# TheCacophonyProject/classifier-pipeline

Measured on AMD Instinct MI355X. Metric: CPTV frames/s end-to-end (track+classify) at 160x120, higher is better.
Workload: dtype u16/i32 track stage (f32 normalise, f64 gates); f32 crop/tile; f32 CNN (stride-1 3x3 convs of stages 2-4 (+ the stride-2 one): two fp16 planes per operand rounded to nearest (11 + 11 significand bits), power-of-two range scaling, 3 fp16 MFMAs per K step, device-side rerun in the exact split if an ac

## Files before the change

classifier-pipeline_amd/cpx/_lib.py:

```python

import ctypes as C
import os

import numpy as np

_HERE = os.path.dirname(os.path.abspath(__file__))
LIB_PATH = os.environ.get("CPX_LIB") or os.path.join(_HERE, "libcpx_hip.so")

CPX_OK = 0
STATUS = {
    0: "CPX_OK",
    -1: "CPX_ERR_INVALID",
    -2: "CPX_ERR_UNSUPPORTED",
    -3: "CPX_ERR_NO_DEVICE",
    -4: "CPX_ERR_HIP",
    -5: "CPX_ERR_OVERFLOW",
    -6: "CPX_ERR_NOMEM",
}


class CpxError(RuntimeError):
    def __init__(self, code, what=""):
        self.code = code
        super().__init__("%s (%d) %s" % (STATUS.get(code, "CPX_ERR"), code, what))


class Config(C.Structure):
    _fields_ = [
        ("width", C.c_int32),
        ("height", C.c_int32),
        ("edge_pixels", C.c_int32),
        ("window", C.c_int32),
        ("background_thresh", C.c_double),
        ("weight_add", C.c_double),
        ("max_components", C.c_int32),
        ("max_frames", C.c_int32),
        ("denoise", C.c_int32),
        ("reserved", C.c_int32),
    ]


FRAME_META_DTYPE = np.dtype(
    [("time_on_ms", "<i8"), ("last_ffc_ms", "<i8"), ("background_frame", "<i4"), ("has_times", "<i4")]
)
COMPONENT_DTYPE = np.dtype(
    [("x", "<i4"), ("y", "<i4"), ("width", "<i4"), ("height", "<i4"), ("area", "<i4"),
     ("sum_x", "<i4"), ("sum_y", "<i4"), ("pixel_variance", "<f4")]
)
FRAME_INFO_DTYPE = np.dtype(
    [("frame_number", "<i4"), ("n_components", "<i4"), ("status", "<i4"), ("ffc_affected", "<i4"),
     ("avg_change", "<i4"), ("norm_min", "<i4"), ("norm_max", "<i4"), ("threshold", "<f4"),
     ("filt_min", "<i4"), ("filt_max", "<i4"), ("thermal_min", "<i4"), ("thermal_max", "<i4"),
     ("thermal_sum", "<u4"), ("thermal_median", "<f4"), ("filtered_abs_sum", "<u8"),
     ("background_average", "<f8"), ("background_changed", "<i4"), ("reserved", "<i4")]
)
REGION_REF_DTYPE = np.dtype([("frame", "<i4"), ("x", "<i4"), ("y", "<i4"), ("width", "<i4"), ("height", "<i4"),
                             ("in_segment", "<i4")])
TRACK_LIMITS_DTYPE = np.dtype([("filt_min", "<f4"), ("filt_max", "<f4"), ("clip_at_zero", "<i4"), ("flags", "<i4"),
                               ("therm_min", "<f4"), ("therm_max", "<f4"), ("reserved", "<i4", (2,))])
CROP_REQ_DTYPE = np.dtype([("frame", "<i4"), ("x", "<i4"), ("y", "<i4"), ("width", "<i4"), ("height", "<i4"),
                           ("track", "<i4"), ("sample", "<i4"), ("tile", "<i4")])
THUMB_STAT_DTYPE = np.dtype([("contours", "<i4"), ("status", "<i4"), ("median_diff", "<f8")])
CONV_TIMING_DTYPE = np.dtype([("key", "<i4"), ("launches", "<i4"), ("total_ms", "<f8"), ("flops", "<f8")])
CPTV_FILE_DTYPE = np.dtype([("in_offset", "<i8"), ("in_bytes", "<i8"), ("out_offset", "<i8"), ("out_capacity", "<i8"),
                            ("slot_offset", "<i8"), ("slot_capacity", "<i4"), ("reserved", "<i4")])
CPTV_RESULT_DTYPE = np.dtype([("status", "<i4"), ("n_frames", "<i4"), ("out_bytes", "<i8"), ("in_consumed", "<i8"),
                              ("header_bytes", "<i4"), ("width", "<i4"), ("height", "<i4"), ("reserved", "<i4")])
CPTV_SLOT_DTYPE = np.dtype([("offset", "<i8"), ("bit_width", "<i4"), ("time_on_ms", "<u4"), ("last_ffc_ms", "<u4"),
                            ("temp_c", "<f4"), ("last_ffc_temp_c", "<f4"), ("flags", "<u4")])
CPTV_HEADER_BYTES = 1024
CPTV_BACKGROUND_FRAME, CPTV_HAS_TIME_ON, CPTV_HAS_LAST_FFC = 1, 2, 4
CPTV_STATUS = {1: "deflate: reserved block type", 2: "deflate: stored block length", 3: "deflate: block header",
               4: "deflate: code lengths", 5: "deflate: invalid symbol", 6: "deflate: distance too far back",
               7: "inflated data larger than the gzip trailer says", 8: "deflate: input exhausted (truncated file)",
               9: "deflate: no end-of-block code", 10: "not a gzip member", 11: "gzip trailer / further member", 12: "gzip CRC-32 mismatch",
               20: "not a CPTV file", 21: "unsupported CPTV version", 22: "CPTV header section", 23: "expected frame section",
               24: "truncated CPTV frame", 25: "malformed CPTV frame section", 26: "more frames than slots",
               27: "CPTV file has no frames"}
assert CPTV_FILE_DTYPE.itemsize == 48 and CPTV_RESULT_DTYPE.itemsize == 40 and CPTV_SLOT_DTYPE.itemsize == 32
assert REGION_REF_DTYPE.itemsize == 24 and TRACK_LIMITS_DTYPE.itemsize == 32 and CROP_REQ_DTYPE.itemsize == 32
assert FRAME_META_DTYPE.itemsize == 24 and COMPONENT_DTYPE.itemsize == 32 and FRAME_INFO_DTYPE.itemsize == 80

class WRResNetBlock(C.Structure):
    _fields_ = [(k, C.c_void_p) for k in ("in_scale", "in_shift", "wa", "a_scale", "a_shift", "wb", "bb")]


class WRResNetParams(C.Structure):
    _fields_ = [("n_labels", C.c_int32), ("blocks_per_stage", C.c_int32), ("groups", C.c_int32),
                ("in_channels", C.c_int32), ("filters", C.c_int32 * 4),
                ("conv1_w", C.c_void_p), ("conv1_b", C.c_void_p),
                ("block", (WRResNetBlock * 8) * 3),
                ("shortcut_w", C.c_void_p * 3), ("shortcut_b", C.c_void_p * 3),
                ("final_scale", C.c_void_p), ("final_shift", C.c_void_p),
                ("dense_w", C.c_void_p), ("dense_b", C.c_void_p),
                ("n_hidden", C.c_int32), ("activation", C.c_int32), ("hidden_sizes", C.c_int32 * 4),
                ("hidden_w", C.c_void_p * 4), ("hidden_b", C.c_void_p * 4)]


class HeadDesc(C.Structure):
    _fields_ = [("N", C.c_int32), ("HW", C.c_int32), ("C", C.c_int32), ("L", C.c_int32),
                ("n_hidden", C.c_int32), ("activation", C.c_int32), ("hidden_sizes", C.c_int32 * 4),
                ("in_dev", C.c_void_p), ("bn_scale_dev", C.c_void_p), ("bn_shift_dev", C.c_void_p),
                ("hidden_w_dev", C.c_void_p * 4), ("hidden_b_dev", C.c_void_p * 4),
                ("dense_w_dev", C.c_void_p), ("dense_b_dev", C.c_void_p),
                ("logits_dev", C.c_void_p), ("probs_dev", C.c_void_p)]


class GraphTensor(C.Structure):
    _fields_ = [("H", C.c_int32), ("W", C.c_int32), ("C", C.c_int32), ("c_offset", C.c_int32), ("c_stride", C.c_int32),
                ("reserved", C.c_int32), ("arena_offset", C.c_int64)]


class GraphOp(C.Structure):
    _fields_ = [("kind", C.c_int32), ("in0", C.c_int32), ("in1", C.c_int32), ("out", C.c_int32),
                ("kh", C.c_int32), ("kw", C.c_int32), ("stride_h", C.c_int32), ("stride_w", C.c_int32),
                ("pad_top", C.c_int32), ("pad_left", C.c_int32), ("pad_bottom", C.c_int32), ("pad_right", C.c_int32),
                ("activation", C.c_int32), ("out_c_offset", C.c_int32), ("out_c_stride", C.c_int32),
                ("n_map", C.c_int32), ("channel_map", C.c_int32 * 4), ("param", C.c_float),
                ("weights", C.c_void_p), ("scale", C.c_void_p), ("shift", C.c_void_p)]


assert C.sizeof(WRResNetParams) == 1560
assert C.sizeof(GraphTensor) == 32 and C.sizeof(GraphOp) == 112
GRAPH_CONV, GRAPH_MAX_POOL, GRAPH_AVG_POOL, GRAPH_ADD, GRAPH_AFFINE, GRAPH_MEAN, GRAPH_FC, GRAPH_LOGISTIC, GRAPH_SOFTMAX, \
    GRAPH_PAD, GRAPH_CHANNEL_MAP, GRAPH_CONV_Q8, GRAPH_FC_Q8, GRAPH_QUANT_PARAMS, GRAPH_DWCONV, GRAPH_DWCONV_Q8, GRAPH_MUL, \
    GRAPH_INPUT, GRAPH_CONV_PRE, GRAPH_SLICE, GRAPH_DWCONV_PRE = range(1, 22)
GRAPH_ACT_SWISH, GRAPH_ACT_LOGISTIC = 16, 17
GRAPH_MEAN_WIDE_PIXELS = 256
GRAPH_CONV_KC, GRAPH_CONV_CO = 16, 32
GRAPH_CONV_Q8_KC = 32
HEAD_SIGMOID, HEAD_SOFTMAX = 0, 1


EXPORTS = [
    "cpx_abi_version", "cpx_create", "cpx_destroy", "cpx_last_error", "cpx_stream", "cpx_synchronize", "cpx_join_medians", "cpx_release_memory",
    "cpx_track_batch", "cpx_track_workspace_bytes", "cpx_last_kernel_timing", "cpx_associate_batch",
    "cpx_track_limits_batch", "cpx_crop_tile", "cpx_conv2d", "cpx_cnn_head",
    "cpx_finalize_tracks", "cpx_counts_prefix", "cpx_plan_segments", "cpx_aggregate_predictions",
    "cpx_conv_timing_enable", "cpx_conv_timing_report", "cpx_cptv_unpack", "cpx_thumb_stats", "cpx_trackless_thumb",
    "cpx_trackless_thumb_batch", "cpx_thumb_stats_ex",
    "cpx_track_frame", "cpx_associate_frame", "cpx_cnn_create", "cpx_cnn_destroy", "cpx_cnn_forward", "cpx_ir_detect", "cpx_set_cnn_math", "cpx_get_cnn_math",
    "cpx_mog2_create", "cpx_mog2_apply", "cpx_mog2_background", "cpx_mog2_destroy",
    "cpx_track_batch_ex", "cpx_track_frame_ex", "cpx_set_background", "cpx_get_background", "cpx_track_limits_batch_ex",
    "cpx_cnn_head_ex", "cpx_ir_delta_variance", "cpx_cptv_inflate", "cpx_cptv_gather_index", "cpx_format_regions", "cpx_json_indent", "cpx_ir_merge", "cpx_ir_resize_area",
    "cpx_ir_frame_statistics", "cpx_cnn_last_overflow", "cpx_cnn_set_activation_bounds", "cpx_cnn_overflow_forwards", "cpx_cnn_forward_taps",
    "cpx_graph_create", "cpx_graph_forward", "cpx_graph_arena_bytes", "cpx_graph_arena_allocated", "cpx_graph_destroy",
    "cpx_cnn_set_residual_bounds", "cpx_cnn_shortcut_scale",
]

IR_FRAME_STATS_DTYPE = np.dtype([("min", "<i4"), ("max", "<i4"), ("sum", "<i8"), ("median_x2", "<i4"), ("reserved", "<i4"),
                                 ("filtered_sum", "<i8")])
assert IR_FRAME_STATS_DTYPE.itemsize == 32

TRACK_KEEP_BACKGROUND, TRACK_FREEZE_ON_FFC, TRACK_FREEZE_BACKGROUND, TRACK_DEFER_MEDIANS = 1, 2, 4, 8
LIMITS_POST_PROCESS, LIMITS_THERMAL_DIFF_NORM, LIMITS_NO_DIFF_NORM, LIMITS_ALWAYS_CLIP, LIMITS_SWAP_CHANNELS = 1, 2, 4, 8, 16
LIMITS_TF_SCALING = 32

_lib = None


def load():
    global _lib
    if _lib is not None:
        return _lib
    if not os.path.exists(LIB_PATH):
        raise ImportError(
            "libcpx_hip.so not built: run `python __graft_entry__.py` (or make -C classifier-pipeline_amd/csrc)")
    try:
        import torch
    except ImportError:
        pass
    lib = C.CDLL(LIB_PATH)
    vp, i32p = C.c_void_p, C.POINTER(C.c_int32)
    lib.cpx_abi_version.restype = C.c_int
    lib.cpx_create.argtypes = [C.c_int, C.POINTER(Config), C.POINTER(vp)]
    lib.cpx_create.restype = C.c_int
    lib.cpx_destroy.argtypes = [vp]
    lib.cpx_destroy.restype = None
    lib.cpx_last_error.argtypes = [vp]
    lib.cpx_last_error.restype = C.c_char_p
    lib.cpx_stream.argtypes = [vp]
    lib.cpx_stream.restype = vp
    lib.cpx_synchronize.argtypes = [vp]
    lib.cpx_synchronize.restype = C.c_int
    lib.cpx_join_medians.argtypes = [vp]
    lib.cpx_join_medians.restype = C.c_int
    lib.cpx_release_memory.argtypes = [vp]
    lib.cpx_release_memory.restype = C.c_int
    lib.cpx_track_batch.argtypes = [vp, vp, i32p, vp, C.c_int, vp, vp, vp, vp, vp]
    lib.cpx_track_batch.restype = C.c_int
    lib.cpx_associate_batch.argtypes = [vp, vp, i32p, vp, C.c_int, vp, vp, vp, vp, vp, vp, vp, vp]
    lib.cpx_associate_batch.restype = C.c_int
    lib.cpx_track_limits_batch.argtypes = [vp, vp, vp, vp, vp, vp, C.c_int, vp]
    lib.cpx_track_limits_batch.restype = C.c_int
    lib.cpx_crop_tile.argtypes = [vp, vp, vp, vp, vp, C.c_int, vp, C.c_int, C.c_int, vp]
    lib.cpx_crop_tile.restype = C.c_int
    lib.cpx_conv2d.argtypes = [vp, vp]
    lib.cpx_conv2d.restype = C.c_int
    lib.cpx_cnn_head.argtypes = [vp, vp, C.c_int, C.c_int, C.c_int, vp, vp, vp, vp, C.c_int, vp, vp]
    lib.cpx_cnn_head.restype = C.c_int
    lib.cpx_cnn_head_ex.argtypes = [vp, C.POINTER(HeadDesc)]
    lib.cpx_cnn_head_ex.restype = C.c_int
    lib.cpx_finalize_tracks.argtypes = [vp, vp, i32p, vp, C.c_int, vp, vp, vp, vp, vp]
    lib.cpx_finalize_tracks.restype = C.c_int
    lib.cpx_plan_segments.argtypes = [vp, vp, i32p, vp, C.c_int, vp, vp, vp, vp, C.c_int, vp, vp, vp, vp, vp]
    lib.cpx_plan_segments.restype = C.c_int
    lib.cpx_counts_prefix.argtypes = [vp, vp, C.c_int, vp]
    lib.cpx_counts_prefix.restype = C.c_int
    lib.cpx_aggregate_predictions.argtypes = [vp, vp, vp, C.c_int, vp, C.c_int, C.c_int, C.c_int, C.c_int, vp, vp]
    lib.cpx_aggregate_predictions.restype = C.c_int
    lib.cpx_conv_timing_enable.argtypes = [vp, C.c_int]
    lib.cpx_conv_timing_enable.restype = C.c_int
    lib.cpx_conv_timing_report.argtypes = [vp, vp, C.c_int, C.POINTER(C.c_int)]
    lib.cpx_conv_timing_report.restype = C.c_int
    lib.cpx_set_cnn_math.argtypes = [vp, C.c_int]
    lib.cpx_set_cnn_math.restype = C.c_int
    lib.cpx_get_cnn_math.argtypes = [vp]
    lib.cpx_get_cnn_math.restype = C.c_int
    lib.cpx_cnn_last_overflow.argtypes = [vp, C.POINTER(C.c_int)]
    lib.cpx_cnn_last_overflow.restype = C.c_int
    lib.cpx_cnn_overflow_forwards.argtypes = [vp, C.POINTER(C.c_int), C.c_int]
    lib.cpx_cnn_overflow_forwards.restype = C.c_int
    lib.cpx_cnn_set_activation_bounds.argtypes = [vp, C.POINTER(C.c_float), C.c_int]
    lib.cpx_cnn_set_activation_bounds.restype = C.c_int
    lib.cpx_cnn_set_residual_bounds.argtypes = [vp, C.POINTER(C.c_float), C.c_int]
    lib.cpx_cnn_set_residual_bounds.restype = C.c_int
    lib.cpx_cnn_shortcut_scale.argtypes = [C.c_float, C.c_float, C.POINTER(C.c_float)]
    lib.cpx_cnn_shortcut_scale.restype = C.c_int
    lib.cpx_mog2_create.argtypes = [vp, C.c_int, C.c_int, C.c_int, C.c_int, C.c_float, C.POINTER(vp)]
    lib.cpx_mog2_create.restype = C.c_int
    lib.cpx_mog2_apply.argtypes = [vp, vp, C.c_double, vp]
    lib.cpx_mog2_apply.restype = C.c_int
    lib.cpx_mog2_background.argtypes = [vp, vp]
    lib.cpx_mog2_background.restype = C.c_int
    lib.cpx_mog2_destroy.argtypes = [vp]
    lib.cpx_mog2_destroy.restype = None
    lib.cpx_ir_detect.argtypes = [vp, vp, C.c_int, C.c_int, C.c_int, C.c_int, C.c_int, vp, vp, vp, vp]
    lib.cpx_ir_detect.restype = C.c_int
    lib.cpx_ir_delta_variance.argtypes = [vp, vp, vp, C.c_int, C.c_int, vp, C.c_int, vp]
    lib.cpx_ir_delta_variance.restype = C.c_int
    lib.cpx_ir_merge.argtypes = [vp, vp, vp, C.c_int, C.c_int, C.c_int, vp, vp, C.c_int, C.c_int, C.c_int, C.c_int, vp, vp, vp]
    lib.cpx_ir_merge.restype = C.c_int
    lib.cpx_ir_resize_area.argtypes = [vp, vp, C.c_int, C.c_int, C.c_int, C.c_int, vp]
    lib.cpx_ir_resize_area.restype = C.c_int
    lib.cpx_ir_frame_statistics.argtypes = [vp, vp, vp, C.c_int, C.c_int, vp, vp]
    lib.cpx_ir_frame_statistics.restype = C.c_int
    lib.cpx_cnn_create.argtypes = [vp, C.POINTER(WRResNetParams), C.POINTER(vp)]
    lib.cpx_cnn_create.restype = C.c_int
    lib.cpx_cnn_destroy.argtypes = [vp]
    lib.cpx_cnn_destroy.restype = None
    lib.cpx_graph_create.argtypes = [vp, C.POINTER(GraphOp), C.c_int, C.POINTER(GraphTensor), C.c_int, C.c_int, C.c_int,
                                     C.POINTER(vp)]
    lib.cpx_graph_create.restype = C.c_int
    lib.cpx_graph_forward.argtypes = [vp, vp, C.c_int, vp]
    lib.cpx_graph_forward.restype = C.c_int
    lib.cpx_graph_arena_bytes.argtypes = [vp, C.c_int, C.POINTER(C.c_size_t)]
    lib.cpx_graph_arena_bytes.restype = C.c_int
    lib.cpx_graph_arena_allocated.argtypes = [vp, C.POINTER(C.c_size_t)]
    lib.cpx_graph_arena_allocated.restype = C.c_int
    lib.cpx_graph_destroy.argtypes = [vp]
    lib.cpx_graph_destroy.restype = None
    lib.cpx_cnn_forward.argtypes = [vp, vp, C.c_int, C.c_int, C.c_int, vp, vp]
    lib.cpx_cnn_forward.restype = C.c_int
    lib.cpx_cnn_forward_taps.argtypes = [vp, vp, C.c_int, C.c_int, C.c_int, vp, vp, C.POINTER(vp), C.c_int, vp]
    lib.cpx_cnn_forward_taps.restype = C.c_int
    lib.cpx_track_frame.argtypes = [vp, vp, vp, C.c_int, C.c_int, vp, vp, vp, vp, vp]
    lib.cpx_track_frame.restype = C.c_int
    lib.cpx_track_batch_ex.argtypes = [vp, vp, i32p, vp, C.c_int, vp, vp, vp, vp, vp, C.c_int]
    lib.cpx_track_batch_ex.restype = C.c_int
    lib.cpx_track_frame_ex.argtypes = [vp, vp, vp, C.c_int, C.c_int, vp, vp, vp, vp, vp, C.c_int]
    lib.cpx_track_frame_ex.restype = C.c_int
    lib.cpx_set_background.argtypes = [vp, C.c_int, vp, vp, C.c_double]
    lib.cpx_set_background.restype = C.c_int
    lib.cpx_get_background.argtypes = [vp, C.c_int, vp, vp, C.POINTER(C.c_double)]
    lib.cpx_get_background.restype = C.c_int
    lib.cpx_track_limits_batch_ex.argtypes = [vp, vp, vp, vp, vp, vp, C.c_int, vp, C.c_int]
    lib.cpx_track_limits_batch_ex.restype = C.c_int
    lib.cpx_associate_frame.argtypes = [vp, vp, vp, C.c_int, C.c_int, vp, vp, vp, vp, vp, vp, vp, vp]
    lib.cpx_associate_frame.restype = C.c_int
    lib.cpx_thumb_stats.argtypes = [vp, vp, vp, vp, vp, C.c_int, vp]
    lib.cpx_thumb_stats.restype = C.c_int
    lib.cpx_thumb_stats_ex.argtypes = [vp, vp, vp, vp, vp, C.c_int, vp, C.c_int, C.c_int, C.c_int]
    lib.cpx_thumb_stats_ex.restype = C.c_int
    lib.cpx_trackless_thumb.argtypes = [vp, vp, C.c_int, C.c_int, vp]
    lib.cpx_trackless_thumb.restype = C.c_int
    lib.cpx_trackless_thumb_batch.argtypes = [vp, vp, vp, C.c_int, vp]
    lib.cpx_trackless_thumb_batch.restype = C.c_int
    lib.cpx_cptv_unpack.argtypes = [vp, vp, vp, vp, vp, C.c_int, vp]
    lib.cpx_cptv_unpack.restype = C.c_int
    lib.cpx_cptv_inflate.argtypes = [vp, vp, vp, C.c_int, vp, vp, vp, vp]
    lib.cpx_cptv_inflate.restype = C.c_int
    lib.cpx_cptv_gather_index.argtypes = [vp, vp, vp, vp, C.c_int, vp, vp, vp]
    lib.cpx_cptv_gather_index.restype = C.c_int
    lib.cpx_format_regions.argtypes = [vp, C.c_int, C.c_long, C.c_int, C.c_int, C.c_int, vp, C.c_long]
    lib.cpx_format_regions.restype = C.c_long
    lib.cpx_json_indent.argtypes = [C.c_char_p, C.c_long, C.c_int, C.c_int, vp, C.c_long]
    lib.cpx_json_indent.restype = C.c_long
    lib.cpx_track_workspace_bytes.argtypes = [vp, C.c_int, C.c_int]
    lib.cpx_track_workspace_bytes.restype = C.c_size_t
    lib.cpx_last_kernel_timing.argtypes = [vp, C.POINTER(C.c_float), C.POINTER(C.c_int)]
    lib.cpx_last_kernel_timing.restype = C.c_int
    if lib.cpx_abi_version() != 3:
        raise ImportError("libcpx_hip.so ABI version mismatch")
    _lib = lib
    return lib
```

classifier-pipeline_amd/cpx/engine.py:

```python

import ctypes as C

import numpy as np

from . import _lib
from ._lib import (COMPONENT_DTYPE, CROP_REQ_DTYPE, FRAME_INFO_DTYPE, FRAME_META_DTYPE, REGION_REF_DTYPE,
                   THUMB_STAT_DTYPE, TRACK_LIMITS_DTYPE, CpxError)
from .tracking import REGION_DTYPE, TRACK_RECORD_DTYPE, make_track_params, track_regions


def thresholds_for_model(model):
    if model == "lepton3.5":
        return 50.0, 1.0
    return 20.0, 0.1


class TrackBatchResult:

    def __init__(self, engine, total, cap, comps, info, labels, filtered, background):
        self.engine, self.total, self.cap = engine, total, cap
        self.comps_dev, self.info_dev = comps, info
        self.labels_dev, self.filtered_dev, self.background_dev = labels, filtered, background
        self._info = self._comps = None
        engine._retain(self)
# ... 108 lines not shown
        self.filtered = t.zeros((n, H, W), dtype=t.float32, device=dev)
        self.background = t.zeros((1, H, W), dtype=t.float32, device=dev)
        ma, mt = params.max_active_tracks, params.max_tracks
        self.pool = t.zeros(n * ma * 14, dtype=t.int32, device=dev)
        self.tracks = t.zeros(mt * 8, dtype=t.int32, device=dev)
        self.ntracks = t.zeros(1, dtype=t.int32, device=dev)
        self.status = t.zeros(1, dtype=t.int32, device=dev)
        self.regions = t.zeros(n * cap * 14, dtype=t.int32, device=dev)
        self.rcounts = t.zeros(n, dtype=t.int32, device=dev)
        self.meta = np.zeros(n, dtype=FRAME_META_DTYPE)
        self.n = 0
        self.n_tracked = 0
        self.result = TrackBatchResult(engine, n, cap, self.comps, self.info, self.labels, self.filtered,
                                       self.background)

    def _p(self, tensor):
        return C.c_void_p(tensor.data_ptr() if tensor is not None else None)

    def append(self, pix, time_on=None, last_ffc=None, init_only=False, associate=True, flags=0):
        eng, t = self.engine, self.engine.torch
        if self.n >= self.cap_frames:
            raise CpxError(-1, "stream is full (%d frames): open the extractor with a larger max_frames"
                           % self.cap_frames)
        f = self.n
        a = np.ascontiguousarray(pix, dtype=np.uint16)
        self.frames_dev[f].copy_(t.from_numpy(a.view(np.int16)))
        m = self.meta[f]
        m["background_frame"] = 1 if init_only else 0
        if time_on is not None and last_ffc is not None:
            m["time_on_ms"], m["last_ffc_ms"], m["has_times"] = time_on, last_ffc, 1
        self.n = f + 1
        if init_only and f == 0:
            return f
        eng.sync_inputs()
        eng.track_calls = getattr(eng, "track_calls", 0) + 1
        mp = C.c_void_p(self.meta.ctypes.data)
        rc = eng.lib.cpx_track_frame_ex(eng.h, self._p(self.frames_dev), mp, self.n_tracked, self.n,
                                        self._p(self.comps), self._p(self.info), self._p(self.labels),
                                        self._p(self.filtered), self._p(self.background), int(flags))
        if rc != 0:
            raise CpxError(rc, eng._err())
        n_prev = self.n_tracked
        self.n_tracked = self.n
        if associate and not init_only:
            rc = eng.lib.cpx_associate_frame(eng.h, C.byref(self.params), mp, n_prev, self.n, self._p(self.comps),
                                             self._p(self.info), self._p(self.pool), self._p(self.tracks),
                                             self._p(self.ntracks), self._p(self.status), self._p(self.regions),
                                             self._p(self.rcounts))
            if rc != 0:
                raise CpxError(rc, eng._err())
        eng.synchronize()
        return f

    def replay(self, old, flags=0, associate=True):
        eng, n = self.engine, old.n
        if n > self.cap_frames:
            raise CpxError(-1, "replay of %d frames into a stream of %d" % (n, self.cap_frames))
        self.frames_dev[:n].copy_(old.frames_dev[:n])
        self.meta[:n] = old.meta[:n]
        self.n = n
        if n == 0 or (n == 1 and self.meta[0]["background_frame"]):
            return
        eng.torch.cuda.current_stream(eng.device).synchronize()
        eng.track_calls = getattr(eng, "track_calls", 0) + 1
        mp = C.c_void_p(self.meta.ctypes.data)
        rc = eng.lib.cpx_track_frame_ex(eng.h, self._p(self.frames_dev), mp, 0, n, self._p(self.comps), self._p(self.info),
                                        self._p(self.labels), self._p(self.filtered), self._p(self.background), int(flags))
        if rc != 0:
            raise CpxError(rc, eng._err())
        self.n_tracked = n
        if associate:
            rc = eng.lib.cpx_associate_frame(eng.h, C.byref(self.params), mp, 0, n, self._p(self.comps), self._p(self.info),
                                             self._p(self.pool), self._p(self.tracks), self._p(self.ntracks),
                                             self._p(self.status), self._p(self.regions), self._p(self.rcounts))
            if rc != 0:
                raise CpxError(rc, eng._err())
        eng.synchronize()

    def overflow(self):
        info = self.info[: self.n * 20].cpu().numpy().view(FRAME_INFO_DTYPE)
        bad = (info["frame_number"] >= 0) & (info["status"] != 0)
        need = int(info["n_components"][bad].max()) if bad.any() else 0
        return need, int(self.status.item()) != 0

    def frame_info(self, f):
        return self.info[f * 20:(f + 1) * 20].cpu().numpy().view(FRAME_INFO_DTYPE)[0]

    def frame_regions(self, f):
        n = int(self.rcounts[f].item())
        cap = self.engine.cap
        return self.regions[f * cap * 14:(f * cap + n) * 14].cpu().numpy().view(REGION_DTYPE)

    def track_records(self):
        n = int(self.ntracks.item())
        st = int(self.status.item())
        if st != 0:
            raise CpxError(st, "track capacity exceeded")
        return self.tracks[: n * 8].cpu().numpy().view(TRACK_RECORD_DTYPE)

    def pool_row(self, q):
        ma = self.params.max_active_tracks
        return self.pool[q * ma * 14:(q + 1) * ma * 14].cpu().numpy().view(REGION_DTYPE)


class ComponentStream:

    def __init__(self, engine, capacity, params):
        t = engine.torch
        self.engine, self.cap_frames, self.params = engine, int(capacity), params
        if self.cap_frames > engine.cfg.max_frames:
            raise ValueError("stream capacity %d exceeds the engine's max_frames %d" % (capacity, engine.cfg.max_frames))
        dev, cap, n = engine.device, engine.cap, self.cap_frames
        ma, mt = params.max_active_tracks, params.max_tracks
        self.comps = t.zeros(n * cap * 8, dtype=t.int32, device=dev)
        self.info = t.zeros(n * 20, dtype=t.int32, device=dev)
        self.pool = t.zeros(n * ma * 14, dtype=t.int32, device=dev)
        self.tracks = t.zeros(mt * 8, dtype=t.int32, device=dev)
        self.ntracks = t.zeros(1, dtype=t.int32, device=dev)
        self.status = t.zeros(1, dtype=t.int32, device=dev)
        self.regions = t.zeros(n * cap * 14, dtype=t.int32, device=dev)
        self.rcounts = t.zeros(n, dtype=t.int32, device=dev)
        self.meta = np.zeros(n, dtype=FRAME_META_DTYPE)
        self.n = 0

    def append(self, components, ffc_affected=False):
        eng, t = self.engine, self.engine.torch
        if self.n >= self.cap_frames:
            raise CpxError(-1, "stream is full (%d frames)" % self.cap_frames)
        comps = np.ascontiguousarray(components, dtype=COMPONENT_DTYPE)
        if len(comps) > eng.cap:
            raise CpxError(-5, "%d components exceed the engine's max_components %d" % (len(comps), eng.cap))
        f = self.n
        if len(comps):
            self.comps[f * eng.cap * 8:(f * eng.cap + len(comps)) * 8] = t.from_numpy(comps.view(np.int32).reshape(-1).copy()).to(eng.device)
        fi = np.zeros(1, FRAME_INFO_DTYPE)
        fi["frame_number"], fi["n_components"], fi["ffc_affected"] = f, len(comps), 1 if ffc_affected else 0
        self.info[f * 20:(f + 1) * 20] = t.from_numpy(fi.view(np.int32).copy()).to(eng.device)
        if ffc_affected:
            self.meta[f]["time_on_ms"], self.meta[f]["last_ffc_ms"], self.meta[f]["has_times"] = 100, 100, 1
        self.n = f + 1
        eng.sync_inputs()
        p = lambda x: C.c_void_p(x.data_ptr())
        rc = eng.lib.cpx_associate_frame(eng.h, C.byref(self.params), C.c_void_p(self.meta.ctypes.data), f, self.n,
                                         p(self.comps), p(self.info), p(self.pool), p(self.tracks), p(self.ntracks),
                                         p(self.status), p(self.regions), p(self.rcounts))
        if rc != 0:
            raise CpxError(rc, eng._err())
        eng.synchronize()
        return f

    frame_regions = TrackStream.frame_regions
    track_records = TrackStream.track_records
    pool_row = TrackStream.pool_row


class TrackEngine:
    def __init__(self, width=160, height=120, model="lepton3", device=0, edge_pixels=1, window=45,
                 max_components=64, max_frames=4096, background_thresh=None, weight_add=None, denoise=False):
        import torch

        self.torch = torch
        self.lib = _lib.load()
        if not torch.cuda.is_available():
            raise RuntimeError("cpx.TrackEngine needs a HIP device (no CPU fallback)")
        bt, wa = thresholds_for_model(model)
        self.cfg = _lib.Config(width, height, edge_pixels, window,
                               float(bt if background_thresh is None else background_thresh),
                               float(wa if weight_add is None else weight_add),
                               max_components, max_frames, 1 if denoise else 0, 0)
        self.device = torch.device("cuda", device)
        self.h = C.c_void_p()
        rc = self.lib.cpx_create(device, C.byref(self.cfg), C.byref(self.h))
        if rc != 0:
            raise CpxError(rc, "cpx_create")
        self.width, self.height, self.cap = width, height, max_components
        self._ctor = dict(width=width, height=height, model=model, device=device, edge_pixels=edge_pixels,
                          background_thresh=self.cfg.background_thresh, weight_add=self.cfg.weight_add,
                          max_frames=max_frames, denoise=denoise)
        self._grown = {}
        self._live_results = 0
        self._close_deferred = False

    def close(self):
        for eng in getattr(self, "_grown", {}).values():
            eng.close()
        self._grown = {}
        if getattr(self, "_live_results", 0) > 0:
            self._close_deferred = True
            if self.h:
                self.lib.cpx_release_memory(self.h)
            return
        self._destroy()

    def _destroy(self):
        if self.h:
            self.lib.cpx_destroy(self.h)
            self.h = C.c_void_p()
        self._torch_stream = None

    def _retain(self, result):
        import weakref

        self._live_results += 1
        weakref.finalize(result, self._release).atexit = False

    def _release(self):
        self._live_results -= 1
        if self.h:
            self.lib.cpx_join_medians(self.h)
        if self._live_results == 0 and self._close_deferred:
            self._close_deferred = False
            try:
                self._destroy()
            except Exception:
                pass

    def _own_stream(self):
        self.sync_inputs()
        return self.torch.cuda.stream(self.torch_stream())

    def MAX_COMPONENTS_EVER(self):
        return ((self.height + 1) // 2) * ((self.width + 1) // 2)

    def grown(self, max_components, max_frames=None):
        cap = self.grown_capacity(max_components)
        eng = self._grown.get(cap)
        if eng is None or (max_frames and eng.cfg.max_frames < max_frames):
            if eng is not None:
                eng.close()
            eng = self.sibling(cap, max_frames)
            self._grown[cap] = eng
        return eng

    def grown_capacity(self, max_components):
        cap = 128
        while cap < max_components:
            cap *= 2
        return max(min(cap, self.MAX_COMPONENTS_EVER()), int(max_components))

    def sibling(self, max_components, max_frames=None):
        args = dict(self._ctor)
        if max_frames:
            args["max_frames"] = max(int(max_frames), args["max_frames"])
        return TrackEngine(max_components=int(max_components), **args)

    def track_clip_grown(self, frames_dev, meta, params=None, need_components=0, want_labels=False, want_filtered=True,
                         want_background=False, flags=0, want_regions=True, associate=True):
        from .tracking import TrackParams

        n = int(frames_dev.shape[0])
        offs = np.array([0, n], np.int32)
        need = max(int(need_components), self.cap)
        params = params or make_track_params(self.width, self.height, self.cfg.edge_pixels)
        while True:
            eng = self if need <= self.cap else self.grown(need, max_frames=n)
            res = eng.track_batch(frames_dev, offs, meta, want_labels=want_labels, want_filtered=want_filtered,
                                  want_background=want_background, flags=flags)
            over = res.overflowed(offs)
            if over:
                if over[0] <= eng.cap:
                    raise CpxError(-5, "a frame reports %d components and still does not fit %d" % (over[0], eng.cap))
                need = over[0]
                continue
            if not associate:
                return eng, res, None, params
            while True:
                assoc = eng.associate_batch(res, offs, meta, params=params, want_regions=want_regions)
                if not assoc.overflowed():
                    return eng, res, assoc, params
                if params.max_active_tracks >= 65536:
                    raise CpxError(-5, "track capacity exceeded at 65536 simultaneous tracks")
                grown = TrackParams.from_buffer_copy(params)
                grown.max_active_tracks = params.max_active_tracks * 2
                grown.max_tracks = params.max_tracks * 2
                params = grown

    def __del__(self):
        try:
            self.close()
        except Exception:
            pass

    def _err(self):
        return (self.lib.cpx_last_error(self.h) or b"").decode()

    def torch_stream(self):
        if getattr(self, "_torch_stream", None) is None:
            self._torch_stream = self.torch.cuda.ExternalStream(int(self.lib.cpx_stream(self.h)), device=self.device)
        return self._torch_stream

    def synchronize(self):
        rc = self.lib.cpx_synchronize(self.h)
        if rc != 0:
            raise CpxError(rc, self._err())

    def sync_inputs(self):
        cur = self.torch.cuda.current_stream(self.device)
        if int(cur.cuda_stream) != int(self.lib.cpx_stream(self.h) or 0):
            cur.synchronize()

    def upload_frames(self, frames):
        t = self.torch
        a = np.ascontiguousarray(frames, dtype=np.uint16)
        return t.from_numpy(a.view(np.int16)).to(self.device)

    def cptv_unpack(self, payload, frame_offsets, bit_widths, clip_offsets):
# ... 60 lines not shown
            res = sub_out.cpu().numpy().view(THUMB_STAT_DTYPE)
            got[take] = res
            done = take[res["status"] == 0] if side is not None else take
            pending = np.setdiff1d(pending, done, assume_unique=True)
        bad = np.nonzero(got["status"] != 0)[0]
        if bad.size:
            raise CpxError(int(got["status"][bad[0]]), "region %d: contour longer than the kernel's chain capacity"
                           % int(bad[0]))
        return got

    THUMB_TIERS = ((46, 2304), (80, 4608))

    CNN_MATH = {"f32": 0, "bf16x3": 1, "bf16x2": 2, "fp16x2": 3}
    DEFAULT_CNN_MATH = "fp16x2"

    def set_cnn_math(self, mode):
        rc = self.lib.cpx_set_cnn_math(self.h, self.CNN_MATH[mode])
        if rc != 0:
            raise CpxError(rc, self._err())

    def cnn_last_overflow(self):
        out = C.c_int(0)
        rc = self.lib.cpx_cnn_last_overflow(self.h, C.byref(out))
        if rc != 0:
            raise CpxError(rc, self._err())
        return bool(out.value)

    def cnn_overflow_forwards(self, reset=False):
        out = C.c_int(0)
        rc = self.lib.cpx_cnn_overflow_forwards(self.h, C.byref(out), 1 if reset else 0)
        if rc != 0:
            raise CpxError(rc, self._err())
        return int(out.value)

    def get_cnn_math(self):
        return {v: k for k, v in self.CNN_MATH.items()}[self.lib.cpx_get_cnn_math(self.h)]

    def ir_detect(self, images_dev, threshold=0, max_components=1024, want_labels=False):
        t = self.torch
        if images_dev.dtype != t.uint8 or images_dev.dim() != 3 or not images_dev.is_contiguous():
            raise ValueError("ir_detect wants a contiguous uint8 [n, H, W] device tensor")
        n, H, W = (int(v) for v in images_dev.shape)
        with self._own_stream():
            comps = t.empty((n, max_components, COMPONENT_DTYPE.itemsize // 4), dtype=t.int32, device=self.device)
            counts = t.zeros(n, dtype=t.int32, device=self.device)
            status = t.zeros(n, dtype=t.int32, device=self.device)
            labels = t.empty((n, H, W), dtype=t.int32, device=self.device) if want_labels else None
        rc = self.lib.cpx_ir_detect(self.h, C.c_void_p(images_dev.data_ptr()), n, W, H, int(threshold),
                                    int(max_components), C.c_void_p(comps.data_ptr()), C.c_void_p(counts.data_ptr()),
                                    C.c_void_p(status.data_ptr()),
                                    C.c_void_p(labels.data_ptr()) if want_labels else None)
        if rc != 0:
            raise CpxError(rc, self._err())
        self.synchronize()
        st = status.cpu().numpy()
        cnt = counts.cpu().numpy()
        bad = np.nonzero(st != 0)[0]
        if bad.size:
            raise CpxError(int(st[bad[0]]), "frame %d has %d components, max_components is %d"
                           % (int(bad[0]), int(cnt[bad[0]]), max_components))
        used = max(1, int(cnt.max()))
        host = comps[:, :used].contiguous().cpu().numpy().view(COMPONENT_DTYPE).reshape(n, used)
        return cnt, host, labels

    def ir_resize_area(self, images_dev, factor, pad_width_to=1):
        t = self.torch
        single = images_dev.dim() == 2
        src = (images_dev[None] if single else images_dev).contiguous()
        n, H, W = (int(v) for v in src.shape)
        with self._own_stream():
            out = t.empty((n, H // factor, W // factor), dtype=t.uint8, device=self.device)
        rc = self.lib.cpx_ir_resize_area(self.h, C.c_void_p(src.data_ptr()), n, W, H, int(factor), C.c_void_p(out.data_ptr()))
        if rc != 0:
            raise CpxError(rc, self._err())
        wo = W // factor
        if pad_width_to > 1 and wo % pad_width_to:
            with t.cuda.stream(self.torch_stream()):
                wide = t.zeros((n, H // factor, (wo + pad_width_to - 1) // pad_width_to * pad_width_to), dtype=t.uint8,
                               device=self.device)
                wide[:, :, :wo] = out
            out = wide
        return out[0] if single else out

    def ir_delta_variance(self, cur_dev, prev_dev, rects):
        t = self.torch
        rects = np.ascontiguousarray(rects, dtype=np.int32).reshape(-1, 4)
        n = len(rects)
        if n == 0:
            return np.zeros(0, np.float64)
        H, W = (int(v) for v in cur_dev.shape)
        r_dev = t.from_numpy(rects).to(self.device)
        out = t.empty(n, dtype=t.float64, device=self.device)
        self.sync_inputs()
        rc = self.lib.cpx_ir_delta_variance(self.h, C.c_void_p(cur_dev.data_ptr()), C.c_void_p(prev_dev.data_ptr()), W, H,
                                            C.c_void_p(r_dev.data_ptr()), n, C.c_void_p(out.data_ptr()))
        if rc != 0:
            raise CpxError(rc, self._err())
        self.synchronize()
        return out.cpu().numpy()

    def trackless_thumb(self, frames_dev, frame, background):
        t = self.torch
        out = t.zeros(2, dtype=t.int32, device=self.device)
        self.sync_inputs()
        rc = self.lib.cpx_trackless_thumb(self.h, C.c_void_p(frames_dev.data_ptr()), int(frame), int(background),
                                          C.c_void_p(out.data_ptr()))
        if rc != 0:
            raise CpxError(rc, self._err())
        self.synchronize()
        x, y = out.cpu().numpy()
        return int(x), int(y)

    @staticmethod
    def make_meta(n, time_on=None, last_ffc=None, background=None):
        m = np.zeros(n, dtype=FRAME_META_DTYPE)
        if time_on is not None:
            for i in range(n):
                if time_on[i] is not None and last_ffc[i] is not None:
                    m["time_on_ms"][i] = time_on[i]
                    m["last_ffc_ms"][i] = last_ffc[i]
                    m["has_times"][i] = 1
        if background is not None:
            m["background_frame"] = np.asarray(background, dtype=np.int32)
        return m

    def set_background(self, clip, background, weights=None, average=None):
        bg = np.ascontiguousarray(background, dtype=np.float32)
        if bg.shape != (self.height, self.width):
            raise ValueError("background must be [%d, %d]" % (self.height, self.width))
        e = self.cfg.edge_pixels
        w = None
        if weights is not None:
            w = np.ascontiguousarray(weights, dtype=np.float64)
            if w.shape != (self.height - 2 * e, self.width - 2 * e):
                raise ValueError("weights must cover the cropped interior")
        if average is None:
            average = float(np.average(bg[e:self.height - e, e:self.width - e]))
        rc = self.lib.cpx_set_background(self.h, int(clip), C.c_void_p(bg.ctypes.data),
                                         C.c_void_p(w.ctypes.data if w is not None else None), float(average))
        if rc != 0:
            raise CpxError(rc, self._err())

    def get_background(self, clip=0):
        e = self.cfg.edge_pixels
        bg = np.empty((self.height, self.width), np.float32)
        w = np.empty((self.height - 2 * e, self.width - 2 * e), np.float64)
        avg = C.c_double()
        rc = self.lib.cpx_get_background(self.h, int(clip), C.c_void_p(bg.ctypes.data), C.c_void_p(w.ctypes.data),
                                         C.byref(avg))
        if rc != 0:
            raise CpxError(rc, self._err())
        return bg, w, float(avg.value)

    def track_batch(self, frames_dev, clip_offsets, meta, want_labels=False, want_filtered=False,
                    want_background=False, outputs=None, flags=0):
        t = self.torch
        offs = np.ascontiguousarray(clip_offsets, dtype=np.int32)
        B = offs.size - 1
        total = int(offs[-1])
        meta = np.ascontiguousarray(meta, dtype=FRAME_META_DTYPE)
        assert meta.size == total and frames_dev.shape[0] >= total
        if outputs is None:
            with self._own_stream():
                comps = t.empty(total * self.cap * 8, dtype=t.int32, device=self.device)
                info = t.empty(total * 20, dtype=t.int32, device=self.device)
                labels = t.empty((total, self.height, self.width), dtype=t.int32, device=self.device) if want_labels else None
                filt = t.empty((total, self.height, self.width), dtype=t.float32, device=self.device) if want_filtered else None
                bgo = t.empty((B, self.height, self.width), dtype=t.float32, device=self.device) if want_background else None
        else:
            comps, info, labels, filt, bgo = outputs
            self.sync_inputs()
        self.track_calls = getattr(self, "track_calls", 0) + 1
        rc = self.lib.cpx_track_batch_ex(
            self.h, C.c_void_p(frames_dev.data_ptr()), offs.ctypes.data_as(C.POINTER(C.c_int32)),
            C.c_void_p(meta.ctypes.data), B, C.c_void_p(comps.data_ptr()), C.c_void_p(info.data_ptr()),
            C.c_void_p(labels.data_ptr() if labels is not None else None),
            C.c_void_p(filt.data_ptr() if filt is not None else None),
            C.c_void_p(bgo.data_ptr() if bgo is not None else None), int(flags))
        if rc != 0:
            raise CpxError(rc, self._err())
        return TrackBatchResult(self, total, self.cap, comps, info, labels, filt, bgo)

    def associate_batch(self, track_result, clip_offsets, meta, params=None, want_regions=True):
        t = self.torch
        offs = np.ascontiguousarray(clip_offsets, dtype=np.int32)
        B = offs.size - 1
        total = int(offs[-1])
        meta = np.ascontiguousarray(meta, dtype=FRAME_META_DTYPE)
        params = params or make_track_params(self.width, self.height, self.cfg.edge_pixels)
        ma, mt = params.max_active_tracks, params.max_tracks
        with self._own_stream():
            pool = t.zeros(total * ma * 14, dtype=t.int32, device=self.device)
            tracks = t.zeros(B * mt * 8, dtype=t.int32, device=self.device)
            ntr = t.zeros(B, dtype=t.int32, device=self.device)
            status = t.zeros(B, dtype=t.int32, device=self.device)
            regions = t.zeros(total * self.cap * 14, dtype=t.int32, device=self.device) if want_regions else None
            rcounts = t.zeros(total, dtype=t.int32, device=self.device) if want_regions else None
        rc = self.lib.cpx_associate_batch(
            self.h, C.byref(params), offs.ctypes.data_as(C.POINTER(C.c_int32)), C.c_void_p(meta.ctypes.data), B,
            C.c_void_p(track_result.comps_dev.data_ptr()), C.c_void_p(track_result.info_dev.data_ptr()),
            C.c_void_p(pool.data_ptr()), C.c_void_p(tracks.data_ptr()), C.c_void_p(ntr.data_ptr()),
            C.c_void_p(status.data_ptr()),
            C.c_void_p(regions.data_ptr() if regions is not None else None),
            C.c_void_p(rcounts.data_ptr() if rcounts is not None else None))
        if rc != 0:
            raise CpxError(rc, self._err())
        return AssocBatchResult(self, offs, params, pool, tracks, ntr, status, regions, rcounts)

    def _to_dev(self, arr):
        a = np.ascontiguousarray(arr)
        return self.torch.from_numpy(a.view(np.int32).reshape(-1).copy()).to(self.device)

    def preprocess_segments(self, frames_dev, track_result, refs, track_offsets, reqs, n_samples, frame_size=32,
                            square_width=5, out=None, limits_flags=0):
        t = self.torch
        if track_result.filtered_dev is None:
            raise ValueError("preprocess_segments needs the filtered frames (track_batch(want_filtered=True))")
        refs = np.ascontiguousarray(refs, dtype=REGION_REF_DTYPE)
        reqs = np.ascontiguousarray(reqs, dtype=CROP_REQ_DTYPE)
        offs = np.ascontiguousarray(track_offsets, dtype=np.int32)
        n_tracks = offs.size - 1
        n_frames, H, W = (int(v) for v in frames_dev.shape[-3:])
        n_frames = min(n_frames, int(track_result.filtered_dev.shape[0]))
        if n_tracks < 0 or offs[0] != 0 or np.any(np.diff(offs) < 0) or offs[-1] > refs.size:
            raise ValueError("preprocess_segments: track_offsets must rise from 0 to at most len(refs)")
        for name, a in (("refs", refs), ("reqs", reqs)):
            empty = (a["width"] <= 0) | (a["height"] <= 0)
            bad = ((a["frame"] < 0) | (a["frame"] >= n_frames) | (a["x"] < 0) | (a["y"] < 0)
                   | (a["x"].astype(np.int64) + a["width"] > W) | (a["y"].astype(np.int64) + a["height"] > H))
            if name == "refs":
                bad &= ~empty
            else:
                bad |= (empty | (a["track"] < 0) | (a["track"] >= n_tracks) | (a["sample"] < 0)
                        | (a["sample"] >= n_samples) | (a["tile"] < 0) | (a["tile"] >= square_width ** 2))
            if np.any(bad):
                raise ValueError("preprocess_segments: %s[%d] = %s lies outside %d frames of %d x %d, %d tracks, "
                                 "%d samples of %d tiles" % (name, int(np.flatnonzero(bad)[0]), a[bad][0], n_frames,
                                                             W, H, n_tracks, n_samples, square_width ** 2))
        refs_dev = self._to_dev(refs) if refs.size else t.zeros(6, dtype=t.int32, device=self.device)
        offs_dev = t.from_numpy(offs).to(self.device)
        reqs_dev = self._to_dev(reqs) if reqs.size else t.zeros(8, dtype=t.int32, device=self.device)
        limits_dev = t.zeros(max(n_tracks, 1) * 8, dtype=t.int32, device=self.device)
        side = square_width * frame_size
        if out is None:
            out = t.empty((n_samples, side, side, 2), dtype=t.float32, device=self.device)
        self.sync_inputs()
        rc = self.lib.cpx_track_limits_batch_ex(
            self.h, C.c_void_p(frames_dev.data_ptr()), C.c_void_p(track_result.filtered_dev.data_ptr()),
            C.c_void_p(track_result.info_dev.data_ptr()), C.c_void_p(refs_dev.data_ptr()),
            C.c_void_p(offs_dev.data_ptr()), n_tracks, C.c_void_p(limits_dev.data_ptr()), int(limits_flags))
        if rc != 0:
            raise CpxError(rc, self._err())
        if reqs.size:
            rc = self.lib.cpx_crop_tile(
                self.h, C.c_void_p(frames_dev.data_ptr()), C.c_void_p(track_result.filtered_dev.data_ptr()),
                C.c_void_p(track_result.info_dev.data_ptr()), C.c_void_p(reqs_dev.data_ptr()), int(reqs.size),
                C.c_void_p(limits_dev.data_ptr()), frame_size, square_width, C.c_void_p(out.data_ptr()))
            if rc != 0:
                raise CpxError(rc, self._err())
        self.synchronize()
        limits = limits_dev.cpu().numpy().view(TRACK_LIMITS_DTYPE).reshape(-1)[:n_tracks]
        return out, limits

    def conv_timing(self, enable=None):
        from ._lib import CONV_TIMING_DTYPE

        if enable is not None:
            rc = self.lib.cpx_conv_timing_enable(self.h, 1 if enable else 0)
            if rc != 0:
                raise CpxError(rc, self._err())
            return None
        out = np.zeros(32, CONV_TIMING_DTYPE)
        n = C.c_int(0)
        rc = self.lib.cpx_conv_timing_report(self.h, C.c_void_p(out.ctypes.data), 32, C.byref(n))
        if rc != 0:
            raise CpxError(rc, self._err())
        return {int(r["key"]): (int(r["launches"]), float(r["total_ms"]), float(r["flops"])) for r in out[: n.value]}

    def last_kernel_timing(self):
        ms = C.c_float()
        n = C.c_int()
        rc = self.lib.cpx_last_kernel_timing(self.h, C.byref(ms), C.byref(n))
        if rc != 0:
            raise CpxError(rc, self._err())
        return float(ms.value), int(n.value)
```

classifier-pipeline_amd/cpx/pipeline.py:

```python

import ctypes as C
import os

import numpy as np

from ._lib import CROP_REQ_DTYPE, REGION_REF_DTYPE, TRACK_DEFER_MEDIANS, CpxError
from .tracking import TRACK_SUMMARY_DTYPE, make_filter_params, make_track_params


class BatchResult:
    def __init__(self):
        self.track = None
        self.assoc = None
        self.summaries_dev = None
        self.counts = None
        self.n_tracks = 0
        self.n_samples = 0
        self.track_clip = None
        self.scores = None
        self.best = None
        self.samples_dev = None
        self.reqs_dev = None
        self.sample_track_dev = None
        self.limits_dev = None
        self.probs = None
        self.parts = None
        self.overflowed = []
        self.regrown = []
        self.clip0 = 0
        self.track_timing = (0.0, 0)

    def summaries(self, max_tracks):
        return self.summaries_dev.cpu().numpy().view(TRACK_SUMMARY_DTYPE).reshape(-1, max_tracks)


class BatchPipeline:
    def __init__(self, engine, network=None, n_labels=17, fp_index=-1, frame_size=32, square_width=5,
                 track_params=None, filter_params=None, cnn_chunk=512, want_regions=False, limits_flags=0,
                 network_bytes=None):
        self.want_regions = want_regions
        self.limits_flags = limits_flags
        self.eng = engine
        self.net = network
        self.n_labels = n_labels
        self.fp_index = fp_index
        self.fs, self.sq = frame_size, square_width
        self.tp = track_params or make_track_params(engine.width, engine.height, engine.cfg.edge_pixels)
        self.fp = filter_params or make_filter_params(max_active_tracks=self.tp.max_active_tracks,
                                                      max_tracks_per_clip=self.tp.max_tracks)
        self.cnn_chunk = cnn_chunk
        self.network_bytes = network_bytes
        self._sample_buf = None

    def _check(self, rc):
        if rc != 0:
            raise CpxError(rc, self.eng._err())

    def sample_chunk(self):
        chunk = max(1, int(self.cnn_chunk))
        per = getattr(self.net, "arena_bytes_per_sample", 0)
        if self.network_bytes is not None and per:
            chunk = max(1, min(chunk, int(self.network_bytes) // int(per)))
        return chunk

    def run(self, frames_dev, clip_offsets, meta, outputs=None, classify=True, keep_samples=False, sub_batches=1):
        if sub_batches > 1 and classify and self.net is not None and not keep_samples:
            if not getattr(self.net, "has_logits", True):
                raise NotImplementedError("sub_batches > 1 (BatchPipeline._run_overlapped) takes the WR-ResNet network only: "
                                          "a TFLite graph network runs through run(sub_batches=1) / classify_front")
            return self._run_overlapped(frames_dev, clip_offsets, meta, outputs, sub_batches)
        eng, t = self.eng, self.eng.torch
        t.cuda.current_stream(eng.device).synchronize()
        with t.cuda.stream(eng.torch_stream()):
            return self._run_on_stream(frames_dev, clip_offsets, meta, outputs, classify, keep_samples)

    def _run_on_stream(self, frames_dev, clip_offsets, meta, outputs, classify, keep_samples):
        eng, t = self.eng, self.eng.torch
        out = self._front(frames_dev, clip_offsets, meta, outputs, classify)
        if not classify or out.n_tracks == 0 or out.n_samples == 0:
            eng.synchronize()
        else:
            out = self.classify_front(out, frames_dev, keep_samples)
        if out.overflowed:
            out = self._regrow(out, frames_dev, clip_offsets, meta, classify, keep_samples)
        return out

    def _regrow(self, out, frames_dev, clip_offsets, meta, classify, keep_samples):
        from .tracking import FilterParams

        eng, t = self.eng, self.eng.torch
        offs = np.ascontiguousarray(clip_offsets, dtype=np.int32)
        meta = np.ascontiguousarray(meta)
        parts = [out]
        for b in out.overflowed:
            f0, f1 = int(offs[b]), int(offs[b + 1])
            fr = frames_dev[f0:f1]
            eng_k, res_k, assoc_k, tp_k = eng.track_clip_grown(fr, meta[f0:f1], params=self.tp, want_filtered=True,
                                                               want_regions=self.want_regions)
            fp_k = FilterParams.from_buffer_copy(self.fp)
            fp_k.max_active_tracks, fp_k.max_tracks_per_clip = tp_k.max_active_tracks, tp_k.max_tracks
            sub = BatchPipeline(eng_k, self.net, n_labels=self.n_labels, fp_index=self.fp_index, frame_size=self.fs,
                                square_width=self.sq, track_params=tp_k, filter_params=fp_k, cnn_chunk=self.cnn_chunk,
                                want_regions=self.want_regions, limits_flags=self.limits_flags,
                                network_bytes=self.network_bytes)
            with t.cuda.stream(eng_k.torch_stream()):
                part = sub._front(fr, np.array([0, f1 - f0], np.int32), meta[f0:f1], None, classify, pre=(res_k, assoc_k))
                if classify and part.n_tracks and part.n_samples:
                    part = sub.classify_front(part, fr, keep_samples)
                else:
                    eng_k.synchronize()
            part.clip0 = b
            out.regrown.append((b, eng_k.cap, tp_k.max_active_tracks, tp_k.max_tracks))
            parts.append(part)
        live = [p for p in parts if p.n_tracks and p.track_clip is not None]
        out.parts = parts
        out.n_tracks = sum(p.n_tracks for p in parts)
        out.n_samples = sum(p.n_samples for p in parts)
        if live:
            tcs = []
            for p in live:
                tc = p.track_clip.clone()
                tc[:, 0] += p.clip0
                tcs.append(tc)
            out.track_clip = t.cat(tcs)
            for name in ("scores", "best", "probs", "logits"):
                vals = [getattr(p, name, None) for p in live]
                if all(v is not None for v in vals):
                    setattr(out, name, t.cat(vals))
        return out

    def classify_front(self, out, frames_dev, keep_samples=False):
        eng, t = self.eng, self.eng.torch
        lib, h = eng.lib, eng.h
        dev = eng.device
        n_tracks, n_samples = out.n_tracks, out.n_samples
        reqs, limits, per = out.reqs_dev, out.limits_dev, self.sq * self.sq
        side = self.sq * self.fs
        probs = t.empty((n_samples, self.n_labels), dtype=t.float32, device=dev)
        has_logits = getattr(self.net, "has_logits", True)
        logits = t.empty((n_samples, self.n_labels), dtype=t.float32, device=dev) if has_logits else None
        n_chunks = -(-n_samples // self.sample_chunk())
        chunk = -(-n_samples // n_chunks)
        if keep_samples:
            out.samples_dev = t.empty((n_samples, side, side, 2), dtype=t.float32, device=dev)
        elif self._sample_buf is None or self._sample_buf.shape[0] < chunk or self._sample_buf.shape[1] != side:
            self._sample_buf = t.empty((chunk, side, side, 2), dtype=t.float32, device=dev)
        sample_bytes = side * side * 2 * 4
        two_streams = self.net is not None and self.net.eng is not eng
        s_eng = eng.torch_stream()
        s_net = self.net.eng.torch_stream() if two_streams else None
        for s0 in range(0, n_samples, chunk):
            s1 = min(s0 + chunk, n_samples)
            buf = out.samples_dev[s0:s1] if keep_samples else self._sample_buf[: s1 - s0]
            self._check(lib.cpx_crop_tile(
                h, C.c_void_p(frames_dev.data_ptr()), C.c_void_p(out.track.filtered_dev.data_ptr()),
                C.c_void_p(out.track.info_dev.data_ptr()), C.c_void_p(reqs.data_ptr() + s0 * per * 32), (s1 - s0) * per,
                C.c_void_p(limits.data_ptr()), self.fs, self.sq, C.c_void_p(buf.data_ptr() - s0 * sample_bytes)))
            if self.net is not None:
                if two_streams:
                    ev = t.cuda.Event()
                    ev.record(s_eng)
                    s_net.wait_event(ev)
                self.net.forward_async(buf, logits[s0:s1] if has_logits else None, probs[s0:s1])
                if has_logits and os.environ.get("CPX_CNN_DEBUG_OVF") and self.net.eng.cnn_last_overflow():
                    per = buf.reshape(buf.shape[0], -1)
                    mx = per.abs().amax(dim=1)
                    print("overflow forward: samples %d..%d, input max %.1f min %.1f nan %d; per-sample max: top %s; "
                          "logits max %.2f" % (s0, s1, float(mx.max()), float(per.min()), int(t.isnan(per).sum()),
                                               [round(float(v), 1) for v in mx.topk(min(5, mx.numel())).values],
                                               float(logits[s0:s1].abs().max())), flush=True)
                if two_streams:
                    ev = t.cuda.Event()
                    ev.record(s_net)
                    s_eng.wait_event(ev)
        if self.net is None:
            eng.synchronize()
            return out
        out.scores = t.empty((n_tracks, self.n_labels), dtype=t.float32, device=dev)
        out.best = t.empty(n_tracks, dtype=t.int32, device=dev)
        self._check(lib.cpx_aggregate_predictions(
            h, C.c_void_p(probs.data_ptr()), C.c_void_p(out.sample_track_dev.data_ptr()), n_samples,
            C.c_void_p(reqs.data_ptr()), n_tracks, self.n_labels, self.fp_index, self.sq,
            C.c_void_p(out.scores.data_ptr()), C.c_void_p(out.best.data_ptr())))
        out.probs = probs
        out.logits = logits
        eng.synchronize()
        if two_streams:
            self.net.eng.synchronize()
        return out

    def _front(self, frames_dev, clip_offsets, meta, outputs, classify=True, pre=None):
        eng, t = self.eng, self.eng.torch
        lib, h = eng.lib, eng.h
        dev = eng.device
        offs = np.ascontiguousarray(clip_offsets, dtype=np.int32)
        meta = np.ascontiguousarray(meta)
        B = offs.size - 1
        out = BatchResult()
        if pre is not None:
            out.track, out.assoc = pre
        else:
            out.track = eng.track_batch(frames_dev, offs, meta, want_filtered=True, outputs=outputs,
                                        flags=TRACK_DEFER_MEDIANS)
            out.assoc = eng.associate_batch(out.track, offs, meta, params=self.tp, want_regions=self.want_regions)
        mt = self.tp.max_tracks
        summ = t.zeros(B * mt * 30, dtype=t.int32, device=dev)
        counts = t.zeros((B, 4), dtype=t.int32, device=dev)
        offs_p = offs.ctypes.data_as(C.POINTER(C.c_int32))
        eng.sync_inputs()
        self._check(lib.cpx_finalize_tracks(
            h, C.byref(self.fp), offs_p, C.c_void_p(meta.ctypes.data), B, C.c_void_p(out.assoc.pool_dev.data_ptr()),
            C.c_void_p(out.assoc.tracks_dev.data_ptr()), C.c_void_p(out.assoc.ntracks_dev.data_ptr()),
            C.c_void_p(summ.data_ptr()), C.c_void_p(counts.data_ptr())))
        out.summaries_dev = summ
        on_stream = int(t.cuda.current_stream(dev).cuda_stream) == int(lib.cpx_stream(h) or 0)
        if not on_stream:
            eng.synchronize()
        prefix = t.empty((B + 1, 4), dtype=t.int32, device=dev)
        self._check(lib.cpx_counts_prefix(h, C.c_void_p(counts.data_ptr()), B, C.c_void_p(prefix.data_ptr())))
        if not on_stream:
            eng.synchronize()
        out.counts = counts.cpu().numpy()
        out.overflowed = [int(b) for b in np.nonzero(out.assoc.status_dev.cpu().numpy())[0]]
        totals = out.counts.sum(axis=0)
        out.track_timing = eng.last_kernel_timing()
        n_tracks, n_refs, n_samples = int(totals[0]), int(totals[1]), int(totals[2])
        out.n_tracks, out.n_samples = n_tracks, n_samples
        if not classify or n_tracks == 0 or n_samples == 0:
            return out
        per = self.sq * self.sq
        refs = t.empty(max(n_refs, 1) * 6, dtype=t.int32, device=dev)
        toffs = t.empty(n_tracks + 1, dtype=t.int32, device=dev)
        reqs = t.empty(n_samples * per * 8, dtype=t.int32, device=dev)
        sample_track = t.empty(n_samples, dtype=t.int32, device=dev)
        track_clip = t.empty((n_tracks, 2), dtype=t.int32, device=dev)
        eng.sync_inputs()
        self._check(lib.cpx_plan_segments(
            h, C.byref(self.fp), offs_p, C.c_void_p(meta.ctypes.data), B, C.c_void_p(out.assoc.pool_dev.data_ptr()),
            C.c_void_p(summ.data_ptr()), C.c_void_p(out.assoc.ntracks_dev.data_ptr()), C.c_void_p(prefix.data_ptr()),
            self.sq, C.c_void_p(refs.data_ptr()), C.c_void_p(toffs.data_ptr()), C.c_void_p(reqs.data_ptr()),
            C.c_void_p(sample_track.data_ptr()), C.c_void_p(track_clip.data_ptr())))
        if not on_stream:
            eng.synchronize()
        out.track_clip, out.reqs_dev, out.sample_track_dev = track_clip, reqs, sample_track
        limits = t.zeros(n_tracks * 8, dtype=t.int32, device=dev)
        eng.sync_inputs()
        self._check(lib.cpx_track_limits_batch_ex(
            h, C.c_void_p(frames_dev.data_ptr()), C.c_void_p(out.track.filtered_dev.data_ptr()),
            C.c_void_p(out.track.info_dev.data_ptr()), C.c_void_p(refs.data_ptr()), C.c_void_p(toffs.data_ptr()),
            n_tracks, C.c_void_p(limits.data_ptr()), int(self.limits_flags)))
        out.limits_dev = limits
        out._keep = (refs, toffs, prefix)
        return out

    def _run_overlapped(self, frames_dev, clip_offsets, meta, outputs, n_sub):
        eng, ceng, t = self.eng, self.net.eng, self.eng.torch
        lib, dev = eng.lib, eng.device
        offs = np.ascontiguousarray(clip_offsets, dtype=np.int32)
        meta = np.ascontiguousarray(meta)
        B = offs.size - 1
        n_sub = max(1, min(n_sub, B))
        bounds = [int(round(B * k / n_sub)) for k in range(n_sub + 1)]
        s_track, s_cnn = eng.torch_stream(), ceng.torch_stream()
        per, side, cap = self.sq * self.sq, self.sq * self.fs, eng.cap
        parts = []
        for k in range(n_sub):
            b0, b1 = bounds[k], bounds[k + 1]
            if b1 <= b0:
                continue
            f0, f1 = int(offs[b0]), int(offs[b1])
            sub_out = None
            if outputs is not None:
                comps, info, labels, filt, bgo = outputs
                sub_out = (comps[f0 * cap * 8:f1 * cap * 8], info[f0 * 20:f1 * 20],
                           None if labels is None else labels[f0:f1], None if filt is None else filt[f0:f1],
                           None if bgo is None else bgo[b0:b1])
            fr = frames_dev[f0:f1]
            part = self._front(fr, offs[b0:b1 + 1] - f0, meta[f0:f1], sub_out)
            part.clip0 = b0
            parts.append(part)
            if part.n_tracks == 0 or part.n_samples == 0:
                continue
            ns, nt = part.n_samples, part.n_tracks
            samples = t.empty((ns, side, side, 2), dtype=t.float32, device=dev)
            part.probs = t.empty((ns, self.n_labels), dtype=t.float32, device=dev)
            logits = t.empty((ns, self.n_labels), dtype=t.float32, device=dev)
            part.scores = t.empty((nt, self.n_labels), dtype=t.float32, device=dev)
            part.best = t.empty(nt, dtype=t.int32, device=dev)
            eng.sync_inputs()
            self._check(lib.cpx_crop_tile(
                eng.h, C.c_void_p(fr.data_ptr()), C.c_void_p(part.track.filtered_dev.data_ptr()),
                C.c_void_p(part.track.info_dev.data_ptr()), C.c_void_p(part.reqs_dev.data_ptr()), ns * per,
                C.c_void_p(part.limits_dev.data_ptr()), self.fs, self.sq, C.c_void_p(samples.data_ptr())))
            ev = t.cuda.Event()
            ev.record(s_track)
            s_cnn.wait_event(ev)
            n_chunks = -(-ns // max(1, self.cnn_chunk))
            chunk = -(-ns // n_chunks)
            for s0 in range(0, ns, chunk):
                s1 = min(s0 + chunk, ns)
                self.net.forward_async(samples[s0:s1], logits[s0:s1], part.probs[s0:s1])
            rc = lib.cpx_aggregate_predictions(
                ceng.h, C.c_void_p(part.probs.data_ptr()), C.c_void_p(part.sample_track_dev.data_ptr()), ns,
                C.c_void_p(part.reqs_dev.data_ptr()), nt, self.n_labels, self.fp_index, self.sq,
                C.c_void_p(part.scores.data_ptr()), C.c_void_p(part.best.data_ptr()))
            if rc != 0:
                raise CpxError(rc, ceng._err())
            part._keep2 = (samples, logits, ev)
        eng.synchronize()
        ceng.synchronize()
        out = BatchResult()
        out.parts = parts
        out.track = parts[0].track if len(parts) == 1 else _MergedCheck([p.track for p in parts])
        out.assoc = parts[0].assoc if len(parts) == 1 else _MergedCheck([p.assoc for p in parts])
        out.counts = np.concatenate([p.counts for p in parts])
        out.track_timing = (sum(p.track_timing[0] for p in parts), sum(p.track_timing[1] for p in parts))
        out.n_tracks = sum(p.n_tracks for p in parts)
        out.n_samples = sum(p.n_samples for p in parts)
        live = [p for p in parts if p.n_tracks and p.n_samples]
        if live:
            tcs = []
            for p in live:
                tc = p.track_clip.clone()
                tc[:, 0] += p.clip0
                tcs.append(tc)
            out.track_clip = t.cat(tcs)
            out.scores = t.cat([p.scores for p in live])
            out.best = t.cat([p.best for p in live])
            out.probs = t.cat([p.probs for p in live])
        out.overflowed = sorted(p.clip0 + b for p in parts for b in p.overflowed)
        if out.overflowed:
            with t.cuda.stream(eng.torch_stream()):
                out = self._regrow(out, frames_dev, clip_offsets, meta, True, False)
        return out


class _MergedCheck:

    def __init__(self, items):
        self.items = items

    def check(self):
        for it in self.items:
            it.check()
```

classifier-pipeline_amd/cpx/track/bulk.py:

```python

import ctypes as C
import json
import logging
import os
import threading
import time
from concurrent.futures import ThreadPoolExecutor
from datetime import datetime, timedelta

import numpy as np

from .._lib import (CPTV_BACKGROUND_FRAME, CPTV_FILE_DTYPE, CPTV_HAS_LAST_FFC, CPTV_HAS_TIME_ON, CPTV_HEADER_BYTES,
                    CPTV_RESULT_DTYPE, CPTV_SLOT_DTYPE, CPTV_STATUS, FRAME_INFO_DTYPE, FRAME_META_DTYPE,
                    REGION_REF_DTYPE, THUMB_STAT_DTYPE, CpxError)
from ..ml_tools import tools
from ..tracking import (REGION_DTYPE, TRACK_SUMMARY_DTYPE, make_filter_params, make_track_params)
from .clip import Clip

THUMBNAIL_SIZE = 64


class StagedFiles:

    def __init__(self, paths, stage, in_off, sizes, isize, errors):
# ... 214 lines not shown
        try:
            h = parse_header_bytes(hdr[i].tobytes())
        except Exception as e:
            out.errors[i] = "%s: %s" % (staged.paths[i], e)
            continue
        headers[i] = h
        groups.setdefault((int(res["width"][i]), int(res["height"][i]), h.model if h.model else None), []).append(i)
    for key, members in groups.items():
        try:
            out.groups.append(_unpack_group(eng, unpack_engine, key, members, headers, res, slot_off, slots_dev, out_dev))
        except Exception as e:
            if isinstance(e, t.cuda.OutOfMemoryError):
                t.cuda.empty_cache()
            for i in members:
                out.errors[i] = "%s: %s: %s" % (staged.paths[i], type(e).__name__, str(e).splitlines()[0] if str(e) else "")
    return out


def _unpack_group(eng, unpack_engine, key, members, headers, res, slot_off, slots_dev, out_dev):
    from .cliptrackextractor import get_engine

    t, dev = eng.torch, eng.device
    p = lambda x: C.c_void_p(x.data_ptr())
    W, H, _ = key
    ok = np.asarray(members)
    offs = np.zeros(len(ok) + 1, np.int32)
    np.cumsum(res["n_frames"][ok], out=offs[1:])
    total = int(offs[-1])
    base = unpack_engine or eng
    ueng = base if (base.width, base.height) == (W, H) else get_engine(W, H, 20.0, 0.1, device=dev.index or 0)
    offs_dev = t.from_numpy(offs).to(dev)
    so_dev = t.from_numpy(np.ascontiguousarray(slot_off[:-1][ok])).to(dev)
    fo_dev = t.empty(total, dtype=t.int64, device=dev)
    bw_dev = t.empty(total, dtype=t.int32, device=dev)
    dense_dev = t.empty(total * 8, dtype=t.int32, device=dev)
    frames_dev = t.empty((total, H, W), dtype=t.int16, device=dev)
    ueng.sync_inputs()
    rc = ueng.lib.cpx_cptv_gather_index(ueng.h, p(slots_dev), p(so_dev), p(offs_dev), len(ok), p(fo_dev), p(bw_dev),
                                        p(dense_dev))
    if rc == 0:
        rc = ueng.lib.cpx_cptv_unpack(ueng.h, p(out_dev), p(fo_dev), p(bw_dev), p(offs_dev), len(ok), p(frames_dev))
    if rc != 0:
        raise CpxError(rc, ueng._err())
    ueng.synchronize()
    slots = dense_dev.cpu().numpy().view(CPTV_SLOT_DTYPE).reshape(-1)
    return DecodedGroup(key, members, [headers[i] for i in members], offs, slots, frames_dev)


def frame_meta_from_slots(slots, process_background=False):
    m = np.zeros(len(slots), FRAME_META_DTYPE)
    fl = slots["flags"]
    has = ((fl & CPTV_HAS_TIME_ON) != 0) & ((fl & CPTV_HAS_LAST_FFC) != 0)
    m["time_on_ms"] = np.where(has, slots["time_on_ms"], 0)
    m["last_ffc_ms"] = np.where(has, slots["last_ffc_ms"], 0)
    m["has_times"] = has
    if not process_background:
        m["background_frame"] = (fl & CPTV_BACKGROUND_FRAME) != 0
    return m


NETWORK_BYTES = 4 << 30


def has_device_network(interp):
    if interp.run_over_network or not callable(getattr(interp, "_network", None)):
        return False
    return getattr(interp, "_weights", True) is not None


def require_device_network(interp):
    if not has_device_network(interp):
        raise NotImplementedError("only the WR-ResNet network runs in the batched forward: a TFLite graph model "
                                  "(LiteInterpreter) or a model served over the network is classified by the "
                                  "one-file path (ClipClassifier.process_file / process_files)")


class BulkTracker:

    def __init__(self, config, device=0):
        from .cliptrackextractor import ClipTrackExtractor

        self.config = config
        self.device = device
        self.extractor = ClipTrackExtractor(config.tracking, config.use_opt_flow, False, verbose=config.verbose,
                                            device=device)
        self.tcfg = self.extractor.config
        self.lib = None
        self.decode_engine = None
        self.cnn_chunk = 2048
        self.network_bytes = NETWORK_BYTES
        self._algorithm_text = {}
        self.timings = {"decode_s": 0.0, "device_s": 0.0, "host_s": 0.0, "write_s": 0.0, "files": 0, "frames": 0}

    def track_group(self, group, clips, classifiers=(), lane=0):
        from ..pipeline import BatchPipeline
        from .cliptrackextractor import get_engine

        cfg = self.tcfg
        c0 = clips[0]
        W, H, _ = group.key
        weight_add = (1 if c0.camera_model == "lepton3.5" else 0.1) / self.extractor.weighting_percent
        longest = int(np.diff(group.offs).max())
        eng = get_engine(W, H, c0.background_thresh, weight_add, cfg.edge_pixels, self.device, max_frames=longest,
                         denoise=bool(cfg.denoise), lane=lane)
        with eng.torch.cuda.stream(eng.torch_stream()):
            return self._track_group(eng, group, clips, classifiers, cfg, c0, W, H)

    def _track_group(self, eng, group, clips, classifiers, cfg, c0, W, H):
        from ..pipeline import BatchPipeline

        t, dev = eng.torch, eng.device
        self.lib = eng.lib
        offs = group.offs
        B = len(offs) - 1
        total = int(offs[-1])
        meta = frame_meta_from_slots(group.slots)
        tp = make_track_params(c0.res_x, c0.res_y, cfg.edge_pixels, cfg.frame_padding, self.extractor.min_dimension,
                               cfg.cropped_regions_strategy, cfg.filter_regions_pre_match, cfg.aoi_min_mass,
                               cfg.aoi_pixel_variance, cfg.params, c0.frames_per_second)
        fp = make_filter_params(cfg.min_duration_secs, cfg.track_min_offset, cfg.track_min_mass, c0.track_min_delta,
                                c0.track_max_delta, cfg.min_moving_frames, cfg.max_blank_percent, cfg.max_jitter,
                                c0.frames_per_second, cfg.max_tracks, tp.max_active_tracks, tp.max_tracks)
        mt, ma = tp.max_tracks, tp.max_active_tracks
        sq = classifiers[0][1].params.square_width if classifiers else 5
        comps = t.empty(total * eng.cap * 8, dtype=t.int32, device=dev)
        info_dev = t.empty(total * 20, dtype=t.int32, device=dev)
        labels = t.empty((total, H, W), dtype=t.int32, device=dev)
        filt = t.empty((total, H, W), dtype=t.float32, device=dev) if classifiers else None
        lflags = classifiers[0][1].limits_flags() if classifiers else 0
        for _, interp in classifiers:
            if interp.params.square_width == 1:
                raise NotImplementedError("single-frame models go through ClipClassifier.process_files")
            if interp.limits_flags() != lflags:
                raise NotImplementedError("models with different normalisation variants in one run")
        pipe = BatchPipeline(eng, None, square_width=sq, track_params=tp, filter_params=fp, want_regions=True,
                             limits_flags=lflags)
        model_out = []
        prof = self.timings.setdefault("device_split_s", {}) if os.environ.get("CPX_BULK_PROFILE") else None
        tick = [time.time()]

        def lap(name):
            if prof is not None:
                eng.synchronize()
                t.cuda.synchronize(dev)
                now = time.time()
                prof[name] = prof.get(name, 0.0) + now - tick[0]
                tick[0] = now

        t.cuda.current_stream(dev).synchronize()
        lap("alloc")
        with t.cuda.stream(eng.torch_stream()):
            front = pipe._front(group.frames_dev, offs, meta, (comps, info_dev, labels, filt, None),
                                classify=bool(classifiers))
            lap("track_assoc_finalize_plan")
            for model, interp in classifiers:
                if interp.params.square_width != sq:
                    raise NotImplementedError("models with different square_width in one run")
                require_device_network(interp)
                fpi = interp.labels.index("false-positive") if "false-positive" in interp.labels else -1
                mp = BatchPipeline(eng, interp._network(eng), n_labels=len(interp.labels), fp_index=fpi,
                                   frame_size=interp.params.frame_size, square_width=sq, track_params=tp,
                                   filter_params=fp, cnn_chunk=self.cnn_chunk, network_bytes=self.network_bytes)
                t0 = time.time()
                probs = None
                if front.n_tracks and front.n_samples:
                    mp.classify_front(front, group.frames_dev)
                    probs = front.probs.cpu().numpy()
                model_out.append(dict(model=model, interp=interp, probs=probs, seconds=time.time() - t0))
            eng.synchronize()
        lap("crop_network")
        res, assoc = front.track, front.assoc
        info = info_dev.cpu().numpy().view(FRAME_INFO_DTYPE).reshape(-1)
        bad = np.nonzero((info["frame_number"] >= 0) & (info["status"] != 0))[0]
        ntr = assoc.ntracks_dev.cpu().numpy()
        astatus = assoc.status_dev.cpu().numpy()
        summ = front.summaries(mt)
        failed = {}
        clip_of_frame = np.repeat(np.arange(B), np.diff(offs))
        for f in bad:
            failed[int(clip_of_frame[f])] = "frame %d: more than %d components" % (int(f - offs[clip_of_frame[f]]), eng.cap)
        for b in np.nonzero(astatus != 0)[0]:
            failed[int(b)] = "track capacity exceeded"
        proc_mask = info["frame_number"] >= 0
        kept = []
        kept_pipe = []
        prefix = np.concatenate([[0], np.cumsum(front.counts[:, 0])])
        for b in range(B):
            s = summ[b, : int(ntr[b])]
            k = np.nonzero(s["reject"] == 0)[0]
            if len(k) and b not in failed:
                k = k[np.argsort(s["rank"][k], kind="stable")]
                kept.extend((b, int(j)) for j in k)
                kept_pipe.extend(int(prefix[b]) + q for q in range(len(k)))
        rows = []
        tr_off = [0]
        for b, j in kept:
            s = summ[b, j]
            n = int(s["n_frames"])
            rows.append((int(offs[b]) + int(s["start_frame"]) + np.arange(n, dtype=np.int64)) * ma + int(s["slot"]))
            tr_off.append(tr_off[-1] + n)
        regions = np.zeros(0, REGION_DTYPE)
        if rows:
            idx = t.from_numpy(np.concatenate(rows)).to(dev)
            pool = assoc.pool_dev.view(-1, 14)
            regions = pool[idx].cpu().numpy().view(REGION_DTYPE).reshape(-1)
        lap("summaries_and_region_gather")
        proc_idx = [np.nonzero(proc_mask[offs[b]:offs[b + 1]])[0] + int(offs[b]) for b in range(B)]
        tr_off = np.asarray(tr_off, np.int64)
        stats = np.zeros(0, THUMB_STAT_DTYPE)
        usable = np.zeros(0, np.int64)
        if len(regions):
            clip_of_reg = np.repeat(np.array([b for b, _ in kept], np.int64), np.diff(tr_off))
            usable = np.nonzero(((regions["flags"] & 1) == 0) & (regions["mass"] != 0))[0]
            if len(usable):
                refs = np.zeros(len(usable), REGION_REF_DTYPE)
                r = regions[usable]
                fidx = np.empty(len(usable), np.int64)
                cb = clip_of_reg[usable]
                for b in np.unique(cb):
                    sel = cb == b
                    fidx[sel] = proc_idx[b][r["frame_number"][sel]]
                refs["frame"], refs["x"], refs["y"], refs["width"], refs["height"] = fidx, r["x"], r["y"], r["width"], r["height"]
                stats = eng.thumb_stats(group.frames_dev, res, refs)
        lap("thumbnail_kernel")
        kept_clips = set(b for b, _ in kept)
        trackless = [b for b in range(B) if b not in kept_clips and b not in failed]
        best_region = {}
        if trackless:
            best_region = self._trackless(eng, group, res, assoc, info, offs, trackless, proc_idx)
        lap("trackless")
        samples = None
        if classifiers and front.n_samples:
            from .._lib import CROP_REQ_DTYPE

            per = sq * sq
            reqs = front.reqs_dev.cpu().numpy().view(CROP_REQ_DTYPE).reshape(-1, per)
            samples = dict(sample_track=front.sample_track_dev.cpu().numpy(), frames=reqs["frame"])
        return dict(info=info, summ=summ, ntr=ntr, kept=kept, kept_pipe=kept_pipe, tr_off=tr_off, regions=regions,
                    usable=usable, stats=stats, failed=failed, best_region=best_region, proc_idx=proc_idx,
                    model_out=model_out, samples=samples)

    def _trackless(self, eng, group, res, assoc, info, offs, clips, proc_idx):
        t, dev = eng.torch, eng.device
        cap = eng.cap
        out = {}
        regs = assoc.regions_dev.view(-1, cap, 14)
        rc_dev = assoc.rcounts_dev
        ffc = res.info_dev.view(-1, 20)[:, 3]
        valid = (t.arange(cap, device=dev)[None, :] < rc_dev[:, None]) & (ffc[:, None] == 0)
        mass = t.where(valid, regs[:, :, 4], t.full((), -1, dtype=t.int32, device=dev))
        fmax, farg = mass.max(dim=1)
        tmax = int(max(offs[b + 1] - offs[b] for b in clips))
        pad_idx = np.full((len(clips), tmax), -1, np.int64)
        for k, b in enumerate(clips):
            pad_idx[k, : offs[b + 1] - offs[b]] = np.arange(offs[b], offs[b + 1])
        pi = t.from_numpy(pad_idx).to(dev)
        m = t.where(pi >= 0, fmax[pi.clamp(min=0)], t.full((), -1, dtype=fmax.dtype, device=dev))
        best_f = m.argmax(dim=1)
        best_m = m.gather(1, best_f[:, None])[:, 0]
        frame_abs = pi.gather(1, best_f[:, None])[:, 0]
        rsel = regs[frame_abs, farg[frame_abs]]
        best_m_h = best_m.cpu().numpy()
        rsel_h = rsel.cpu().numpy().view(REGION_DTYPE).reshape(-1)
        search = []
        for k, b in enumerate(clips):
            if best_m_h[k] >= 0:
                out[b] = ("region", rsel_h[k])
            else:
                search.append(b)
        if search:
            P = eng.width * eng.height
            pairs, rows = [], []
            for b in search:
                pf = proc_idx[b]
                if len(pf) == 0:
                    out[b] = ("none", None)
                    continue
                q = int(np.argmax(info["thermal_sum"][pf] / P))
                pairs.append((int(pf[q]), int(offs[b])))
                rows.append((b, q))
            if pairs:
                pairs_dev = t.from_numpy(np.asarray(pairs, np.int32)).to(dev)
                xy = t.zeros((len(pairs), 2), dtype=t.int32, device=dev)
                eng.sync_inputs()
                rc = eng.lib.cpx_trackless_thumb_batch(eng.h, C.c_void_p(group.frames_dev.data_ptr()),
                                                       C.c_void_p(pairs_dev.data_ptr()), len(pairs), C.c_void_p(xy.data_ptr()))
                if rc != 0:
                    raise CpxError(rc, eng._err())
                eng.synchronize()
                xy_h = xy.cpu().numpy()
                for k, (b, q) in enumerate(rows):
                    out[b] = ("window", (q, int(xy_h[k, 0]), int(xy_h[k, 1])))
        return out

    def _fmt_regions(self, regs, indent, depth, as_list=True):
        n = len(regs)
        cap = 512 + 420 * max(n, 1)
        buf = C.create_string_buffer(cap)
        got = self.lib.cpx_format_regions(C.c_void_p(regs.ctypes.data), n, REGION_DTYPE.itemsize, indent, depth,
                                          1 if as_list else 0, buf, cap)
        if got < 0:
            buf = C.create_string_buffer(-got + 16)
            got = self.lib.cpx_format_regions(C.c_void_p(regs.ctypes.data), n, REGION_DTYPE.itemsize, indent, depth,
                                              1 if as_list else 0, buf, -got + 16)
        return buf.raw[:got].decode("ascii")

# ... 622 lines not shown
```

classifier-pipeline_amd/csrc/cpx_api.cpp:

```cpp
#include <hip/hip_runtime.h>

#include <algorithm>
#include <cmath>
#include <cstdio>
#include <cstdlib>
#include <cstring>
#include <new>
#include <string>
#include <vector>

#include "cpx_internal.h"
#include "cpx_schedule_core.h"

static_assert(sizeof(cpx_component) == 32, "cpx_component layout is part of the ABI");
static_assert(sizeof(cpx_frame_info) == 80, "cpx_frame_info layout is part of the ABI");
static_assert(sizeof(cpx_frame_meta) == 24, "cpx_frame_meta layout is part of the ABI");
static_assert(sizeof(cpx_config) == 48, "cpx_config layout is part of the ABI");
static_assert(sizeof(cpx_region_ref) == 24 && sizeof(cpx_track_limits) == 32 && sizeof(cpx_crop_req) == 32,
              "classification request layouts are part of the ABI");
static_assert(sizeof(cpx_filter_params) == 72 && sizeof(cpx_track_summary) == 120,
              "end-of-clip layouts are part of the ABI");
static_assert(sizeof(cpx_region) == 56, "cpx_region layout is part of the ABI");
static_assert(sizeof(cpx_track_record) == 32, "cpx_track_record layout is part of the ABI");
static_assert(sizeof(cpx_track_params) == 120, "cpx_track_params layout is part of the ABI");

namespace {

struct WsLayout {
  size_t bg, wsum, kcnt, filt, cstate, u8, carry, bgavg, big, total;
};

WsLayout ws_layout(const cpx_config& c, int B, bool need_filt_state) {
  const size_t P = (size_t)c.width * c.height;
  WsLayout l{};
  size_t off = 0;
  l.bg = off;
  off = align_up(off + (size_t)B * 2 * P * sizeof(uint16_t), 256);
  l.wsum = off;
  off = align_up(off + (size_t)B * P * sizeof(uint32_t), 256);
  l.kcnt = off;
  off = align_up(off + (size_t)B * P * sizeof(uint16_t), 256);
  l.filt = off;
  if (need_filt_state) off = align_up(off + (size_t)B * 2 * P * sizeof(float), 256);
  l.cstate = off;
  off = align_up(off + (size_t)B * sizeof(cpx::ClipState), 256);
  l.u8 = off;
  off = align_up(off + (size_t)B * 2 * P, 256);
  l.carry = off;
  off = align_up(off + (size_t)B * 2 * sizeof(cpx::FrameCarry), 256);
  l.bgavg = off;
  off = align_up(off + (size_t)B * sizeof(double), 256);
  l.big = off;
  if (c.max_components > cpx::track_lds_components())
    off = align_up(off + (size_t)B * 9 * c.max_components * sizeof(uint32_t), 256);
  l.total = off;
  return l;
}

int build_schedule(cpx_handle* h, const int32_t* clip_offsets, const cpx_frame_meta* meta, int B, cpx::Schedule* sc) {
  switch (cpx::schedule_build(clip_offsets, meta, B, h->cfg.max_frames, sc)) {
    case cpx::SchedError::EmptyClip: return fail(h, CPX_ERR_INVALID, "empty clip in batch");
    case cpx::SchedError::TooLong: return fail(h, CPX_ERR_INVALID, "clip longer than max_frames");
    case cpx::SchedError::Ok: break;
  }
  return CPX_OK;
}

int upload_schedule(cpx_handle* h, const cpx::Schedule& sc, int B, cpx::SchedLayout* sl) {
  const std::vector<int> flat = cpx::schedule_flatten(sc, B);
  *sl = cpx::SchedLayout::of(B, (int)sc.proc_idx.size());
  if (int rc = h->sched.grow(h, flat.size() * sizeof(int), "schedule hipMalloc")) return rc;
  CPX_HIP(h, hipMemcpyAsync(h->sched.p, flat.data(), flat.size() * sizeof(int), hipMemcpyHostToDevice, h->stream));
  CPX_HIP(h, hipStreamSynchronize(h->stream));
  return CPX_OK;
}

}

extern "C" {

int cpx_abi_version(void) { return CPX_ABI_VERSION; }

int cpx_create(int device_id, const cpx_config* cfg, cpx_handle** out) {
  if (!cfg || !out) return CPX_ERR_INVALID;
  *out = nullptr;
  int ndev = 0;
  if (hipGetDeviceCount(&ndev) != hipSuccess || ndev <= 0) return CPX_ERR_NO_DEVICE;
  if (device_id < 0 || device_id >= ndev) return CPX_ERR_INVALID;
  const int W = cfg->width, H = cfg->height;
  if (W <= 0 || H <= 0 || (W % 8) != 0 || W >= 192 || W * H > cpx::track_max_pixels() || H < 5 || W < 8)
    return CPX_ERR_UNSUPPORTED;
  if (cfg->edge_pixels < 0 || 2 * cfg->edge_pixels >= std::min(W, H) || cfg->window < 1 ||
      cfg->max_components < 1 || cfg->max_frames < 1 || cfg->max_frames > 65534)
    return CPX_ERR_INVALID;
  cpx_handle* h = new (std::nothrow) cpx_handle();
  if (!h) return CPX_ERR_NOMEM;
  h->device = device_id;
  h->cfg = *cfg;
  if (hipSetDevice(device_id) != hipSuccess || hipStreamCreateWithFlags(&h->stream, hipStreamNonBlocking) != hipSuccess ||
      hipStreamCreateWithFlags(&h->stream2, hipStreamNonBlocking) != hipSuccess ||
      hipEventCreateWithFlags(&h->ev_median, hipEventDisableTiming) != hipSuccess ||
      hipEventCreate(&h->ev0) != hipSuccess || hipEventCreate(&h->ev1) != hipSuccess) {
    cpx_destroy(h);
    return CPX_ERR_HIP;
  }
  h->wtab_len = 65536;
  h->wtab_host.resize(h->wtab_len);
  std::vector<double>& wt = h->wtab_host;
  double w = 0.0;
  for (int k = 0; k < h->wtab_len; ++k) {
    wt[k] = w;
    w = w + cfg->weight_add;
  }
  if (cfg->denoise) {
    if (!cpx::nlm_supported(W, H)) {
      cpx_destroy(h);
      return CPX_ERR_UNSUPPORTED;
    }
    const int fixed_point_mult = (int)(2147483647LL / (21 * 21 * 255));
    std::vector<int> lut(64, 0);
    for (int a2 = 0; a2 < 64; ++a2) {
      const double wv = std::exp(-((double)a2 * (64.0 / 49.0)) / 9.0);
      const double wr = std::nearbyint((double)fixed_point_mult * wv);
      lut[a2] = (wr < 0.001 * fixed_point_mult) ? 0 : (int)wr;
    }
    if (lut[63] != 0 || h->nlm_lut_dev.grow(h, 64 * sizeof(int), "NLM weight table allocation") ||
        hipMemcpy(h->nlm_lut_dev.p, lut.data(), 64 * sizeof(int), hipMemcpyHostToDevice) != hipSuccess) {
      cpx_destroy(h);
      return CPX_ERR_HIP;
    }
  }
  std::vector<uint32_t> thr(h->wtab_len);
  for (int k = 0; k < h->wtab_len; ++k) {
    const double wk = wt[k], m = std::nearbyint(wk);
    const bool exact = (wk == m), near = !exact && std::fabs(wk - m) < 1e-6;
    double hi = near ? m + 1.0 : std::floor(wk) + 1.0;
    if (!(hi >= 0.0)) hi = 0.0;
    if (hi > 536870912.0) hi = 536870912.0;
    thr[k] = 2u * (uint32_t)hi - (near ? 1u : 0u);
  }
  if (h->wthr_dev.grow(h, thr.size() * sizeof(uint32_t), "threshold table allocation") ||
      hipMemcpy(h->wthr_dev.p, thr.data(), thr.size() * sizeof(uint32_t), hipMemcpyHostToDevice) != hipSuccess) {
    cpx_destroy(h);
    return CPX_ERR_HIP;
  }
  if (h->wtab_dev.grow(h, wt.size() * sizeof(double), "weight table allocation") ||
      hipMemcpy(h->wtab_dev.p, wt.data(), wt.size() * sizeof(double), hipMemcpyHostToDevice) != hipSuccess ||
      cpx::frame_kernel_attr_setup() != 0) {
    cpx_destroy(h);
    return CPX_ERR_HIP;
  }
  if (const char* env = std::getenv("CPX_TRACK_PACKED_STATE")) h->packed_state_ok = std::atoi(env) != 0;
  if (const char* env = std::getenv("CPX_CNN_FUSE_CONV1")) h->fuse_conv1 = std::atoi(env) != 0;
  if (const char* env = std::getenv("CPX_TRACK_PER_STEP")) h->track_per_step = std::atoi(env) != 0;
  if (const char* env = std::getenv("CPX_CNN_FUSE_SHORTCUT")) h->fuse_shortcut = std::atoi(env) != 0;
  if (const char* env = std::getenv("CPX_CNN_SHORTCUT_FP16")) h->shortcut_fp16 = std::atoi(env) != 0;
  if (const char* env = std::getenv("CPX_CNN_BLOCK_FUSION")) h->block_fusion = std::min(std::max(std::atoi(env), 0), 2);
  if (const char* env = std::getenv("CPX_CNN_MATH")) {
    if (!std::strcmp(env, "f32")) h->cnn_math = CPX_CNN_MATH_F32;
    else if (!std::strcmp(env, "bf16x3")) h->cnn_math = CPX_CNN_MATH_BF16X3;
    else if (!std::strcmp(env, "bf16x2")) h->cnn_math = CPX_CNN_MATH_BF16X2;
    else if (!std::strcmp(env, "fp16x2")) h->cnn_math = CPX_CNN_MATH_FP16X2;
  }
  *out = h;
  return CPX_OK;
}

static void release_buffers(cpx_handle* h, bool all) {
  for (DeviceBuffer* b : {&h->ws, &h->ws_assoc, &h->bf3_scratch, &h->cnn_arena, &h->graph_arena, &h->ir_scratch}) b->release();
  if (!all) return;
  for (DeviceBuffer* b : {&h->sched, &h->wtab_dev, &h->wthr_dev, &h->nlm_lut_dev, &h->cnn_ovf, &h->ir_bitmap}) b->release();
}

void cpx_destroy(cpx_handle* h) {
  if (!h) return;
  hipSetDevice(h->device);
  if (h->stream) hipStreamSynchronize(h->stream);
  for (cpx_cnn* c : h->cnns) cnn_free(c);
  h->cnns.clear();
  for (cpx_mog2* m : h->mog2s) mog2_free(m);
  h->mog2s.clear();
  for (cpx_graph* g : h->graphs) graph_free(g);
  h->graphs.clear();
  release_buffers(h, true);
  for (auto& e : h->conv_events) {
    hipEventDestroy(e.e0);
    hipEventDestroy(e.e1);
  }
  if (h->stream2) {
    hipStreamSynchronize(h->stream2);
    hipStreamDestroy(h->stream2);
  }
  if (h->ev_median) hipEventDestroy(h->ev_median);
  if (h->ev0) hipEventDestroy(h->ev0);
  if (h->ev1) hipEventDestroy(h->ev1);
  if (h->stream) hipStreamDestroy(h->stream);
  delete h;
}

const char* cpx_last_error(const cpx_handle* h) { return h ? h->err.c_str() : "null handle"; }

void* cpx_stream(cpx_handle* h) { return h ? (void*)h->stream : nullptr; }

static int join_medians(cpx_handle* h) {
  if (h->medians_pending) {
    h->medians_pending = false;
    CPX_HIP(h, hipStreamWaitEvent(h->stream, h->ev_median, 0));
  }
  return CPX_OK;
}

int cpx_join_medians(cpx_handle* h) {
  if (!h) return CPX_ERR_INVALID;
  return join_medians(h);
}

int cpx_release_memory(cpx_handle* h) {
  if (!h) return CPX_ERR_INVALID;
  CPX_ENTER(h);
  if (int rc = join_medians(h)) return rc;
  CPX_HIP(h, hipStreamSynchronize(h->stream));
  CPX_HIP(h, hipStreamSynchronize(h->stream2));
  release_buffers(h, false);
  h->last_B = 0;
  h->state_packed = false;
  return CPX_OK;
}

int cpx_synchronize(cpx_handle* h) {
  if (!h) return CPX_ERR_INVALID;
  if (int rc = join_medians(h)) return rc;
  CPX_HIP(h, hipStreamSynchronize(h->stream));
  return CPX_OK;
}

size_t cpx_track_workspace_bytes(const cpx_handle* h, int B, int total_frames) {
  if (!h || B <= 0) return 0;
  (void)total_frames;
  return ws_layout(h->cfg, B, true).total;
}

static int unpack_state(cpx_handle* h) {
  if (h->state_packed && h->ws.p && h->last_B > 0) {
    const WsLayout lp = ws_layout(h->cfg, h->last_B, h->stream_filt_state);
    char* base = h->ws.as<char>();
    cpx::launch_unpack_state((uint32_t*)(base + lp.wsum), (uint16_t*)(base + lp.kcnt),
                             (size_t)h->last_B * h->cfg.width * h->cfg.height, h->stream);
    CPX_HIP(h, hipGetLastError());
  }
  h->state_packed = false;
  return CPX_OK;
}

static int track_run(cpx_handle* h, const uint16_t* frames_dev, const int32_t* clip_offsets,
                     const cpx_frame_meta* meta, int B, int n_prev, cpx_component* comps_dev,
                     cpx_frame_info* info_dev, int32_t* labels_dev, float* filtered_dev,
                     float* background_dev, int flags) {
  CPX_ENTER(h);
  if (flags & ~(CPX_TRACK_KEEP_BACKGROUND | CPX_TRACK_FREEZE_ON_FFC | CPX_TRACK_FREEZE_BACKGROUND | CPX_TRACK_DEFER_MEDIANS))
    return fail(h, CPX_ERR_INVALID, "track: unknown flag");
  if (int jrc = join_medians(h)) return jrc;
  const bool defer_medians = (flags & CPX_TRACK_DEFER_MEDIANS) != 0;
  const cpx_config& c = h->cfg;
  cpx::Schedule sc;
  int rc = build_schedule(h, clip_offsets, meta, B, &sc);
  if (rc != CPX_OK) return rc;
  const int total = sc.total, max_proc = sc.max_proc;
  const bool resume = n_prev > 0;
  const int t_begin = cpx::processed_before(meta, n_prev);
  const bool need_filt = (filtered_dev == nullptr);
  const WsLayout l = ws_layout(c, B, need_filt);
  if (resume && (l.total > h->ws.bytes || need_filt != h->stream_filt_state))
    return fail(h, CPX_ERR_INVALID, "cpx_track_frame: the stream's workspace is gone (optional outputs changed?)");
  const bool keep = !resume && (flags & CPX_TRACK_KEEP_BACKGROUND);
  if (keep) {
    const bool have_prev = h->ws.p && h->last_B == B && need_filt == h->stream_filt_state && l.total <= h->ws.bytes;
    for (int b = 0; b < B && !have_prev; ++b)
      if (!h->staged_bg.count(b)) {
        h->staged_bg.clear();
        return fail(h, CPX_ERR_INVALID, "CPX_TRACK_KEEP_BACKGROUND: no background state for a clip (previous call had another batch size, and nothing staged; staged states dropped)");
      }
  }
  for (const auto& kv : h->staged_bg)
    if (kv.first >= B) {
      h->staged_bg.clear();
      return fail(h, CPX_ERR_INVALID, "cpx_set_background: staged clip index outside the batch (staged states dropped)");
    }
  if (resume || keep) {
    if (int urc = unpack_state(h)) return urc;
  }
  h->state_packed = false;
  h->stream_filt_state = need_filt;
  h->last_B = B;
  struct StateGuard {
    cpx_handle* h;
    bool armed = true;
    ~StateGuard() {
      if (armed) {
        h->last_B = 0;
        h->state_packed = false;
      }
    }
  } guard{h};
  if ((rc = h->ws.grow(h, l.total, "workspace hipMalloc"))) return rc;
  cpx::SchedLayout sl;
  rc = upload_schedule(h, sc, B, &sl);
  if (rc != CPX_OK) return rc;

  cpx::TrackArgs a{};
  a.W = c.width;
  a.H = c.height;
  a.edge = c.edge_pixels;
  a.window = c.window;
  a.cap_out = c.max_components;
  a.flags = flags;
  a.background_thresh = c.background_thresh;
  a.weight_add = c.weight_add;
  a.frames = frames_dev;
  cpx::schedule_point(a, h->sched.as<int>(), sl);
  a.order = h->sched.as<int>() + sl.order;
  a.wtab = h->wtab_dev.as<double>();
  a.wtab_len = h->wtab_len;
  a.wthr = h->wthr_dev.as<uint32_t>();
  char* base = h->ws.as<char>();
  a.bg = (uint16_t*)(base + l.bg);
  a.wsum = (uint32_t*)(base + l.wsum);
  a.kcnt = (uint16_t*)(base + l.kcnt);
  a.packed_state = (h->packed_state_ok && !resume && !keep && h->staged_bg.empty() && max_proc <= 1023 && c.window <= 64) ? 1 : 0;
  a.filt_state = need_filt ? (float*)(base + l.filt) : nullptr;
  a.cstate = (cpx::ClipState*)(base + l.cstate);
  a.u8_state = (unsigned char*)(base + l.u8);
  a.carry = (cpx::FrameCarry*)(base + l.carry);
  a.bgavg = (double*)(base + l.bgavg);
  a.big_stat = c.max_components > cpx::track_lds_components() ? (uint32_t*)(base + l.big) : nullptr;
  a.nlm_flip = c.denoise ? 1 : 0;
  a.nlm_lut = h->nlm_lut_dev.as<int>();
  a.comps_out = comps_dev;
  a.info_out = info_dev;
  a.labels_out = labels_dev;
  a.filtered_out = filtered_dev;

  const int f_new = resume ? n_prev : 0;
  CPX_HIP(h, hipMemsetAsync(info_dev + f_new, 0xFF, (size_t)(total - f_new) * sizeof(cpx_frame_info), h->stream));
  if (!resume) cpx::launch_init(a, B, keep ? 1 : 0, h->stream);
  if (!h->staged_bg.empty()) {
    const size_t P = (size_t)c.width * c.height;
    for (const auto& kv : h->staged_bg) {
      const int b = kv.first;
      const auto& sb = kv.second;
      for (int slot = 0; slot < 2; ++slot)
        CPX_HIP(h, hipMemcpyAsync(a.bg + ((size_t)b * 2 + slot) * P, sb.bg.data(), P * sizeof(uint16_t),
                                  hipMemcpyHostToDevice, h->stream));
      CPX_HIP(h, hipMemcpyAsync(a.kcnt + (size_t)b * P, sb.kcnt.data(), P * sizeof(uint16_t), hipMemcpyHostToDevice,
                                h->stream));
      CPX_HIP(h, hipMemcpyAsync(&a.cstate[b].bg_average, &sb.average, sizeof(double), hipMemcpyHostToDevice, h->stream));
      CPX_HIP(h, hipMemcpyAsync(a.bgavg + b, &sb.average, sizeof(double), hipMemcpyHostToDevice, h->stream));
    }
    CPX_HIP(h, hipStreamSynchronize(h->stream));
    h->staged_bg.clear();
  }
  if ((long long)B * (max_proc - t_begin) > 2147483647LL) return fail(h, CPX_ERR_INVALID, "batch too large for one launch");
  if (!defer_medians) cpx::launch_median(a, B, t_begin, max_proc, h->stream);
  CPX_HIP(h, hipEventRecord(h->ev0, h->stream));
  int launches = 0;
  if (!c.denoise && !h->track_per_step) {
    cpx::launch_frame(a, B, t_begin, max_proc, 0, h->stream);
    launches = 1;
  } else {
    for (int t = t_begin; t < max_proc; ++t) {
      if (!c.denoise) {
        cpx::launch_frame(a, B, t, t + 1, 0, h->stream);
      } else {
        cpx::launch_frame(a, B, t, t + 1, 1, h->stream);
        cpx::launch_nlm(a, B, t, h->stream);
        cpx::launch_frame(a, B, t, t + 1, 2, h->stream);
      }
      ++launches;
    }
  }
  CPX_HIP(h, hipEventRecord(h->ev1, h->stream));
  if (defer_medians) {
    CPX_HIP(h, hipStreamWaitEvent(h->stream2, h->ev1, 0));
    cpx::launch_median(a, B, t_begin, max_proc, h->stream2);
    CPX_HIP(h, hipEventRecord(h->ev_median, h->stream2));
    h->medians_pending = true;
  }
  h->state_packed = a.packed_state != 0;
  h->last_launches = launches;
  h->timing_valid = true;
  if (background_dev) cpx::launch_export_background(a, B, background_dev, h->stream);
  CPX_HIP(h, hipGetLastError());
  guard.armed = false;
  return CPX_OK;
}

int cpx_track_batch_ex(cpx_handle* h, const uint16_t* frames_dev, const int32_t* clip_offsets,
                       const cpx_frame_meta* meta, int B, cpx_component* comps_dev, cpx_frame_info* info_dev,
                       int32_t* labels_dev, float* filtered_dev, float* background_dev, int flags) {
  if (!h) return CPX_ERR_INVALID;
  if (!frames_dev || !clip_offsets || !meta || B <= 0 || !comps_dev || !info_dev)
    return fail(h, CPX_ERR_INVALID, "cpx_track_batch: null argument");
  h->stream_frames = -1;
  return track_run(h, frames_dev, clip_offsets, meta, B, -1, comps_dev, info_dev, labels_dev, filtered_dev,
                   background_dev, flags);
}

int cpx_track_batch(cpx_handle* h, const uint16_t* frames_dev, const int32_t* clip_offsets,
                    const cpx_frame_meta* meta, int B, cpx_component* comps_dev,
                    cpx_frame_info* info_dev, int32_t* labels_dev, float* filtered_dev,
                    float* background_dev) {
  return cpx_track_batch_ex(h, frames_dev, clip_offsets, meta, B, comps_dev, info_dev, labels_dev, filtered_dev,
                            background_dev, 0);
}

int cpx_track_frame_ex(cpx_handle* h, const uint16_t* frames_dev, const cpx_frame_meta* meta, int n_prev, int n_frames,
                       cpx_component* comps_dev, cpx_frame_info* info_dev, int32_t* labels_dev, float* filtered_dev,
                       float* background_dev, int flags) {
  if (!h) return CPX_ERR_INVALID;
  if (!frames_dev || !meta || !comps_dev || !info_dev || n_prev < 0 || n_frames <= n_prev)
    return fail(h, CPX_ERR_INVALID, "cpx_track_frame: bad argument");
  if (n_prev > 0 && h->stream_frames != n_prev)
    return fail(h, CPX_ERR_INVALID, "cpx_track_frame: n_prev does not match the frames this handle has consumed");
  const int32_t offs[2] = {0, n_frames};
  h->stream_frames = -1;
  if (n_prev == 0) h->stream_assoc_frames = -1;
  const int rc = track_run(h, frames_dev, offs, meta, 1, n_prev, comps_dev, info_dev, labels_dev, filtered_dev,
                           background_dev, flags);
  if (rc == CPX_OK) h->stream_frames = n_frames;
  return rc;
}

int cpx_track_frame(cpx_handle* h, const uint16_t* frames_dev, const cpx_frame_meta* meta, int n_prev, int n_frames,
                    cpx_component* comps_dev, cpx_frame_info* info_dev, int32_t* labels_dev, float* filtered_dev,
                    float* background_dev) {
  return cpx_track_frame_ex(h, frames_dev, meta, n_prev, n_frames, comps_dev, info_dev, labels_dev, filtered_dev,
                            background_dev, 0);
}

int cpx_set_background(cpx_handle* h, int clip, const float* background, const double* weights, double average) {
  if (!h) return CPX_ERR_INVALID;
  if (clip < 0 || !background) return fail(h, CPX_ERR_INVALID, "cpx_set_background: bad argument");
  const cpx_config& c = h->cfg;
  const int W = c.width, H = c.height, e = c.edge_pixels;
  const size_t P = (size_t)W * H;
  cpx_handle::StagedBackground sb;
  sb.bg.resize(P);
  sb.kcnt.assign(P, 0);
  sb.average = average;
  for (size_t p = 0; p < P; ++p) {
    const float v = background[p];
    if (!(v >= 0.0f && v <= 65535.0f) || v != std::floor(v))
      return fail(h, CPX_ERR_UNSUPPORTED, "cpx_set_background: the background must be integer-valued in [0, 65535]");
    sb.bg[p] = (uint16_t)v;
  }
  if (weights) {
    const std::vector<double>& wt = h->wtab_host;
    const int iw = W - 2 * e, ih = H - 2 * e;
    for (int y = 0; y < ih; ++y)
      for (int x = 0; x < iw; ++x) {
        const double wv = weights[(size_t)y * iw + x];
        long k = c.weight_add > 0 ? std::lround(wv / c.weight_add) : 0;
        bool ok = false;
        for (long kk = std::max(0L, k - 1); kk <= k + 1 && kk < h->wtab_len; ++kk)
          if (wt[kk] == wv) {
            k = kk;
            ok = true;
            break;
          }
        if (!ok) return fail(h, CPX_ERR_UNSUPPORTED, "cpx_set_background: a weight is not an accumulation of weight_add");
        sb.kcnt[(size_t)(y + e) * W + (x + e)] = (uint16_t)k;
      }
  }
  h->staged_bg[clip] = std::move(sb);
  return CPX_OK;
}

int cpx_get_background(cpx_handle* h, int clip, float* background, double* weights, double* average) {
  if (!h) return CPX_ERR_INVALID;
  if (clip < 0 || clip >= h->last_B || !h->ws.p) return fail(h, CPX_ERR_INVALID, "cpx_get_background: no such clip in the last track call");
  CPX_ENTER(h);
  const cpx_config& c = h->cfg;
  const int W = c.width, H = c.height, e = c.edge_pixels;
  const size_t P = (size_t)W * H;
  const WsLayout l = ws_layout(c, h->last_B, h->stream_filt_state);
  char* base = h->ws.as<char>();
  if (int urc = unpack_state(h)) return urc;
  CPX_HIP(h, hipStreamSynchronize(h->stream));
  cpx::ClipState st;
  CPX_HIP(h, hipMemcpy(&st, base + l.cstate + (size_t)clip * sizeof(cpx::ClipState), sizeof(st), hipMemcpyDeviceToHost));
  if (average) *average = st.bg_average;
  if (background) {
    std::vector<uint16_t> bg(P);
    CPX_HIP(h, hipMemcpy(bg.data(), base + l.bg + ((size_t)clip * 2 + (st.n_done & 1)) * P * sizeof(uint16_t),
                         P * sizeof(uint16_t), hipMemcpyDeviceToHost));
    for (int y = 0; y < H; ++y)
      for (int x = 0; x < W; ++x) {
        const int cy = std::min(std::max(y, e), H - 1 - e), cx = std::min(std::max(x, e), W - 1 - e);
        background[(size_t)y * W + x] = (float)bg[(size_t)cy * W + cx];
      }
  }
  if (weights) {
    std::vector<uint16_t> kc(P);
    CPX_HIP(h, hipMemcpy(kc.data(), base + l.kcnt + (size_t)clip * P * sizeof(uint16_t), P * sizeof(uint16_t),
                         hipMemcpyDeviceToHost));
    const std::vector<double>& wt = h->wtab_host;
    const int iw = W - 2 * e, ih = H - 2 * e;
    for (int y = 0; y < ih; ++y)
      for (int x = 0; x < iw; ++x) {
        const int k = kc[(size_t)(y + e) * W + (x + e)];
        weights[(size_t)y * iw + x] = k < h->wtab_len ? wt[k] : (double)k * c.weight_add;
      }
  }
  return CPX_OK;
}

static int assoc_run(cpx_handle* h, const cpx_track_params* params, const int32_t* clip_offsets,
                     const cpx_frame_meta* meta, int B, int n_prev, bool fresh, const cpx_component* comps_dev,
                     const cpx_frame_info* info_dev, cpx_region* pool_dev,
                     cpx_track_record* tracks_dev, int32_t* n_tracks_dev, int32_t* status_dev,
                     cpx_region* regions_dev, int32_t* region_counts_dev) {
  if (params->max_active_tracks < 1 || params->max_tracks < 1)
    return fail(h, CPX_ERR_INVALID, "association: capacities must be positive");
  CPX_ENTER(h);
  const bool resume = n_prev > 0 && !fresh;
  const int t_begin = cpx::processed_before(meta, n_prev);
  cpx::Schedule sc;
  cpx::SchedLayout sl;
  int rc = build_schedule(h, clip_offsets, meta, B, &sc);
  if (rc != CPX_OK) return rc;
  rc = upload_schedule(h, sc, B, &sl);
  if (rc != CPX_OK) return rc;
  const int cap = h->cfg.max_components, ma = params->max_active_tracks;
  size_t off = 0;
  const size_t o_active = off;
  off = align_up(off + (size_t)B * ma * cpx::assoc_active_bytes(), 256);
  const size_t o_regs = off;
  off = align_up(off + (size_t)B * cap * sizeof(cpx_region), 256);
  const size_t o_scores = off;
  off = align_up(off + (size_t)B * cap * ma * cpx::assoc_score_bytes(), 256);
  const size_t o_used = off;
  off = align_up(off + (size_t)B * cap, 256);
  const size_t o_resume = off;
  off = align_up(off + (size_t)B * sizeof(cpx::AssocResume), 256);
  if (resume && off > h->ws_assoc.bytes)
    return fail(h, CPX_ERR_INVALID, "cpx_associate_frame: the stream's association state is gone");
  if ((rc = h->ws_assoc.grow(h, off, "association workspace hipMalloc"))) return rc;
  char* base = h->ws_assoc.as<char>();
  cpx::AssocArgs a{};
  a.B = B;
  a.cap = cap;
  a.params = *params;
  cpx::schedule_point(a, h->sched.as<int>(), sl);
  a.comps = comps_dev;
  a.info = info_dev;
  a.pool = pool_dev;
  a.tracks = tracks_dev;
  a.n_tracks = n_tracks_dev;
  a.status = status_dev;
  a.regions_out = regions_dev;
  a.region_counts = region_counts_dev;
  a.active = (cpx::ActiveTrack*)(base + o_active);
  a.regs = (cpx_region*)(base + o_regs);
  a.scores = (cpx::ScoreRec*)(base + o_scores);
  a.used = (unsigned char*)(base + o_used);
  a.resume = (cpx::AssocResume*)(base + o_resume);
  a.t_begin = t_begin;
  a.fresh = resume ? 0 : 1;
  cpx::launch_assoc(a, h->stream);
  CPX_HIP(h, hipGetLastError());
  return CPX_OK;
}

int cpx_associate_batch(cpx_handle* h, const cpx_track_params* params, const int32_t* clip_offsets,
                        const cpx_frame_meta* meta, int B, const cpx_component* comps_dev,
                        const cpx_frame_info* info_dev, cpx_region* pool_dev,
                        cpx_track_record* tracks_dev, int32_t* n_tracks_dev, int32_t* status_dev,
                        cpx_region* regions_dev, int32_t* region_counts_dev) {
  if (!h) return CPX_ERR_INVALID;
  if (!params || !clip_offsets || !meta || B <= 0 || !comps_dev || !info_dev || !pool_dev || !tracks_dev ||
      !n_tracks_dev || !status_dev)
    return fail(h, CPX_ERR_INVALID, "cpx_associate_batch: null argument");
  h->stream_assoc_frames = -1;
  return assoc_run(h, params, clip_offsets, meta, B, -1, true, comps_dev, info_dev, pool_dev, tracks_dev, n_tracks_dev,
                   status_dev, regions_dev, region_counts_dev);
}

int cpx_associate_frame(cpx_handle* h, const cpx_track_params* params, const cpx_frame_meta* meta, int n_prev,
                        int n_frames, const cpx_component* comps_dev, const cpx_frame_info* info_dev,
                        cpx_region* pool_dev, cpx_track_record* tracks_dev, int32_t* n_tracks_dev,
                        int32_t* status_dev, cpx_region* regions_dev, int32_t* region_counts_dev) {
  if (!h) return CPX_ERR_INVALID;
  if (!params || !meta || !comps_dev || !info_dev || !pool_dev || !tracks_dev || !n_tracks_dev || !status_dev ||
      n_prev < 0 || n_frames <= n_prev)
    return fail(h, CPX_ERR_INVALID, "cpx_associate_frame: bad argument");
  const bool fresh = h->stream_assoc_frames < 0;
  if (!fresh && h->stream_assoc_frames > n_prev)
    return fail(h, CPX_ERR_INVALID, "cpx_associate_frame: n_prev is behind the frames this handle has consumed");
  const int32_t offs[2] = {0, n_frames};
  h->stream_assoc_frames = -1;
  const int rc = assoc_run(h, params, offs, meta, 1, n_prev, fresh, comps_dev, info_dev, pool_dev, tracks_dev, n_tracks_dev,
                           status_dev, regions_dev, region_counts_dev);
  if (rc == CPX_OK) h->stream_assoc_frames = n_frames;
  return rc;
}

static cpx::ClassifyArgs classify_args(const cpx_handle* h) {
  cpx::ClassifyArgs a{};
  const cpx_config& c = h->cfg;
  a.W = c.width;
  a.H = c.height;
  a.crop_x = c.edge_pixels;
  a.crop_y = c.edge_pixels;
  a.crop_w = c.width - 2 * c.edge_pixels;
  a.crop_h = c.height - 2 * c.edge_pixels;
  return a;
}

int cpx_track_limits_batch(cpx_handle* h, const uint16_t* frames_dev, const float* filtered_dev,
                           const cpx_frame_info* info_dev, const cpx_region_ref* refs_dev,
                           const int32_t* track_offsets_dev, int n_tracks, cpx_track_limits* limits_dev) {
  return cpx_track_limits_batch_ex(h, frames_dev, filtered_dev, info_dev, refs_dev, track_offsets_dev, n_tracks,
                                   limits_dev, 0);
}

int cpx_track_limits_batch_ex(cpx_handle* h, const uint16_t* frames_dev, const float* filtered_dev,
                              const cpx_frame_info* info_dev, const cpx_region_ref* refs_dev,
                              const int32_t* track_offsets_dev, int n_tracks, cpx_track_limits* limits_dev, int flags) {
  if (!h) return CPX_ERR_INVALID;
  if (!frames_dev || !filtered_dev || !info_dev || !refs_dev || !track_offsets_dev || !limits_dev || n_tracks < 0 ||
      (flags & ~(CPX_LIMITS_POST_PROCESS | CPX_LIMITS_THERMAL_DIFF_NORM | CPX_LIMITS_NO_DIFF_NORM | CPX_LIMITS_ALWAYS_CLIP |
                 CPX_LIMITS_SWAP_CHANNELS | CPX_LIMITS_TF_SCALING)))
    return fail(h, CPX_ERR_INVALID, "cpx_track_limits_batch: bad argument");
  if (n_tracks == 0) return CPX_OK;
  CPX_ENTER(h);
  if (int jrc = join_medians(h)) return jrc;
  cpx::ClassifyArgs a = classify_args(h);
  a.limits_flags = flags;
  a.frames = frames_dev;
  a.filtered = filtered_dev;
  a.info = info_dev;
  a.refs = refs_dev;
  a.track_offsets = track_offsets_dev;
  a.limits = limits_dev;
  cpx::launch_limits(a, n_tracks, h->stream);
  CPX_HIP(h, hipGetLastError());
  return CPX_OK;
}

int cpx_crop_tile(cpx_handle* h, const uint16_t* frames_dev, const float* filtered_dev,
                  const cpx_frame_info* info_dev, const cpx_crop_req* reqs_dev, int n_reqs,
                  const cpx_track_limits* limits_dev, int frame_size, int square_width, float* out_dev) {
  if (!h) return CPX_ERR_INVALID;
  if (!frames_dev || !filtered_dev || !info_dev || !reqs_dev || !limits_dev || !out_dev || n_reqs < 0)
    return fail(h, CPX_ERR_INVALID, "cpx_crop_tile: null argument");
  if (frame_size < 1 || frame_size > 128 || square_width < 1 || square_width > 16)
    return fail(h, CPX_ERR_UNSUPPORTED, "cpx_crop_tile: frame_size must be 1..128, square_width 1..16");
  if (n_reqs == 0) return CPX_OK;
  CPX_ENTER(h);
  if (int jrc = join_medians(h)) return jrc;
  cpx::ClassifyArgs a = classify_args(h);
  a.frames = frames_dev;
  a.filtered = filtered_dev;
  a.info = info_dev;
  a.limits = const_cast<cpx_track_limits*>(limits_dev);
  a.reqs = reqs_dev;
  a.out = out_dev;
  a.frame_size = frame_size;
  a.square_width = square_width;
  if (cpx::launch_crop(a, n_reqs, h->stream) != 0) return fail(h, CPX_ERR_HIP, "cpx_crop_tile: kernel configuration failed");
  CPX_HIP(h, hipGetLastError());
  return CPX_OK;
}

static int final_args(cpx_handle* h, const cpx_filter_params* params, const int32_t* clip_offsets,
                      const cpx_frame_meta* meta, int B, cpx::FinalArgs* a) {
  if (params->max_active_tracks < 1 || params->max_tracks_per_clip < 1)
    return fail(h, CPX_ERR_INVALID, "filter params: capacities must be positive");
  CPX_ENTER(h);
  cpx::Schedule sc;
  cpx::SchedLayout sl;
  int rc = build_schedule(h, clip_offsets, meta, B, &sc);
  if (rc != CPX_OK) return rc;
  rc = upload_schedule(h, sc, B, &sl);
  if (rc != CPX_OK) return rc;
  a->B = B;
  a->params = *params;
  a->max_frames = h->cfg.max_frames;
  cpx::schedule_point(*a, h->sched.as<int>(), sl);
  const size_t doubles = (size_t)B * h->cfg.max_frames * 2 * sizeof(double);
  rc = h->ws_assoc.grow(h, doubles + (size_t)B * h->cfg.max_frames * sizeof(float) + 512, "finalize workspace hipMalloc");
  if (rc != CPX_OK) return rc;
  a->scratch_d = h->ws_assoc.as<double>();
  a->scratch_f = (float*)(h->ws_assoc.as<char>() + align_up(doubles, 256));
  return CPX_OK;
}

int cpx_finalize_tracks(cpx_handle* h, const cpx_filter_params* params, const int32_t* clip_offsets,
                        const cpx_frame_meta* meta, int B, const cpx_region* pool_dev,
                        const cpx_track_record* tracks_dev, const int32_t* n_tracks_dev,
                        cpx_track_summary* summaries_dev, int32_t* counts_dev) {
  if (!h) return CPX_ERR_INVALID;
  if (!params || !clip_offsets || !meta || B <= 0 || !pool_dev || !tracks_dev || !n_tracks_dev || !summaries_dev ||
      !counts_dev)
    return fail(h, CPX_ERR_INVALID, "cpx_finalize_tracks: null argument");
  cpx::FinalArgs a{};
  const int rc = final_args(h, params, clip_offsets, meta, B, &a);
  if (rc != CPX_OK) return rc;
  a.square_width = 5;
  a.pool = pool_dev;
  a.tracks = tracks_dev;
  a.n_tracks = n_tracks_dev;
  a.summaries = summaries_dev;
  a.counts = counts_dev;
  cpx::launch_finalize(a, h->stream);
  CPX_HIP(h, hipGetLastError());
  return CPX_OK;
}

int cpx_plan_segments(cpx_handle* h, const cpx_filter_params* params, const int32_t* clip_offsets,
                      const cpx_frame_meta* meta, int B, const cpx_region* pool_dev,
                      const cpx_track_summary* summaries_dev, const int32_t* n_tracks_dev,
                      const int32_t* prefix_dev, int square_width, cpx_region_ref* refs_dev,
                      int32_t* track_offsets_dev, cpx_crop_req* reqs_dev, int32_t* sample_track_dev,
                      int32_t* track_clip_dev) {
  if (!h) return CPX_ERR_INVALID;
  if (!params || !clip_offsets || !meta || B <= 0 || !pool_dev || !summaries_dev || !n_tracks_dev || !prefix_dev ||
      !refs_dev || !track_offsets_dev || !reqs_dev || !sample_track_dev || !track_clip_dev)
    return fail(h, CPX_ERR_INVALID, "cpx_plan_segments: null argument");
  if (square_width != 5) return fail(h, CPX_ERR_UNSUPPORTED, "cpx_plan_segments: square_width must be 5");
  cpx::FinalArgs a{};
  const int rc = final_args(h, params, clip_offsets, meta, B, &a);
  if (rc != CPX_OK) return rc;
  a.square_width = square_width;
  a.pool = pool_dev;
  a.summaries = const_cast<cpx_track_summary*>(summaries_dev);
  a.n_tracks = n_tracks_dev;
  a.prefix = prefix_dev;
  a.refs = refs_dev;
  a.track_offsets = track_offsets_dev;
  a.reqs = reqs_dev;
  a.sample_track = sample_track_dev;
  a.track_clip = track_clip_dev;
  cpx::launch_plan(a, h->stream);
  CPX_HIP(h, hipGetLastError());
  return CPX_OK;
}

int cpx_counts_prefix(cpx_handle* h, const int32_t* counts_dev, int B, int32_t* prefix_dev) {
  if (!h) return CPX_ERR_INVALID;
  if (!counts_dev || !prefix_dev || B <= 0) return fail(h, CPX_ERR_INVALID, "cpx_counts_prefix: bad argument");
  CPX_ENTER(h);
  cpx::launch_counts_prefix(counts_dev, B, prefix_dev, h->stream);
  CPX_HIP(h, hipGetLastError());
  return CPX_OK;
}

int cpx_aggregate_predictions(cpx_handle* h, const float* probs_dev, const int32_t* sample_track_dev,
                              int n_samples, const cpx_crop_req* reqs_dev, int n_tracks, int n_labels,
                              int false_positive_index, int square_width, float* scores_dev, int32_t* best_dev) {
  if (!h) return CPX_ERR_INVALID;
  if (n_tracks == 0) return CPX_OK;
  if (!probs_dev || !sample_track_dev || !reqs_dev || !scores_dev || !best_dev || n_samples < 0 || n_tracks < 0 ||
      n_labels < 1)
    return fail(h, CPX_ERR_INVALID, "cpx_aggregate_predictions: bad argument");
  CPX_ENTER(h);
  cpx::AggregateArgs a{};
  a.n_samples = n_samples; a.n_tracks = n_tracks; a.n_labels = n_labels; a.fp_index = false_positive_index;
  a.square_width = square_width;
  a.probs = probs_dev; a.sample_track = sample_track_dev; a.reqs = reqs_dev; a.scores = scores_dev; a.best = best_dev;
  cpx::launch_aggregate(a, h->stream);
  CPX_HIP(h, hipGetLastError());
  return CPX_OK;
}

int cpx_cptv_unpack(cpx_handle* h, const uint8_t* payload_dev, const int64_t* frame_offsets_dev,
                    const int32_t* bit_widths_dev, const int32_t* clip_offsets_dev, int B,
                    uint16_t* frames_out_dev) {
  if (!h) return CPX_ERR_INVALID;
  if (!payload_dev || !frame_offsets_dev || !bit_widths_dev || !clip_offsets_dev || !frames_out_dev || B < 1)
    return fail(h, CPX_ERR_INVALID, "cpx_cptv_unpack: bad argument");
  CPX_ENTER(h);
  cpx::CptvArgs a{};
  a.W = h->cfg.width;
  a.H = h->cfg.height;
  a.payload = payload_dev;
  a.frame_offsets = (const long long*)frame_offsets_dev;
  a.bit_widths = bit_widths_dev;
  a.clip_offsets = clip_offsets_dev;
  a.frames_out = frames_out_dev;
  const int rc = cpx::launch_cptv_unpack(a, B, h->stream);
  if (rc == -2) return fail(h, CPX_ERR_UNSUPPORTED, "cpx_cptv_unpack: resolution too large for the unpack kernel");
  if (rc != 0) return fail(h, CPX_ERR_HIP, "cpx_cptv_unpack: kernel configuration failed");
  CPX_HIP(h, hipGetLastError());
  return CPX_OK;
}

int cpx_cptv_inflate(cpx_handle* h, const uint8_t* in_dev, const cpx_cptv_file* files_dev, int B, uint8_t* out_dev,
                     cpx_cptv_frame_slot* slots_dev, uint8_t* header_dev, cpx_cptv_file_result* results_dev) {
  if (!h) return CPX_ERR_INVALID;
  if (!in_dev || !files_dev || !out_dev || !slots_dev || !results_dev || B < 1)
    return fail(h, CPX_ERR_INVALID, "cpx_cptv_inflate: bad argument");
  CPX_ENTER(h);
  cpx::CptvInflateArgs a{};
  a.B = B;
  a.in = in_dev;
  a.files = files_dev;
  a.out = out_dev;
  a.slots = slots_dev;
  a.header = header_dev;
  a.results = results_dev;
  cpx::launch_cptv_inflate(a, h->stream);
  CPX_HIP(h, hipGetLastError());
  return CPX_OK;
}

int cpx_cptv_gather_index(cpx_handle* h, const cpx_cptv_frame_slot* slots_dev, const int64_t* slot_offsets_dev,
                          const int32_t* clip_offsets_dev, int B, int64_t* frame_offsets_dev, int32_t* bit_widths_dev,
                          cpx_cptv_frame_slot* slots_out_dev) {
  if (!h) return CPX_ERR_INVALID;
  if (!slots_dev || !slot_offsets_dev || !clip_offsets_dev || !frame_offsets_dev || !bit_widths_dev || B < 1)
    return fail(h, CPX_ERR_INVALID, "cpx_cptv_gather_index: bad argument");
  CPX_ENTER(h);
  cpx::CptvGatherArgs a{};
  a.slots = slots_dev;
  a.slot_offsets = (const long long*)slot_offsets_dev;
  a.clip_offsets = clip_offsets_dev;
  a.frame_offsets = (long long*)frame_offsets_dev;
  a.bit_widths = bit_widths_dev;
  a.slots_out = slots_out_dev;
  cpx::launch_cptv_gather(a, B, h->stream);
  CPX_HIP(h, hipGetLastError());
  return CPX_OK;
}

int cpx_thumb_stats_ex(cpx_handle* h, const uint16_t* frames_dev, const int32_t* labels_dev,
                       const cpx_frame_info* info_dev, const cpx_region_ref* refs_dev, int n_refs,
                       cpx_thumb_stat* out_dev, int max_width, int max_height, int chain_capacity) {
  if (!h) return CPX_ERR_INVALID;
  if (!frames_dev || !labels_dev || !info_dev || !refs_dev || !out_dev || n_refs < 0 || max_width < 1 || max_height < 1 ||
      chain_capacity < 16 || chain_capacity > 32000)
    return fail(h, CPX_ERR_INVALID, "cpx_thumb_stats: bad argument");
  if (n_refs == 0) return CPX_OK;
  CPX_ENTER(h);
  if (int jrc = join_medians(h)) return jrc;
  cpx::ThumbArgs a{};
  a.W = h->cfg.width;
  a.H = h->cfg.height;
  a.chain_cap = chain_capacity;
  a.max_w = max_width < a.W ? max_width : a.W;
  a.max_h = max_height < a.H ? max_height : a.H;
  a.frames = frames_dev;
  a.labels = labels_dev;
  a.info = info_dev;
  a.refs = refs_dev;
  a.out = out_dev;
  const int rc = cpx::launch_thumb(a, n_refs, h->stream);
  if (rc == -2) return fail(h, CPX_ERR_UNSUPPORTED, "cpx_thumb_stats: resolution too large for the contour kernel");
  if (rc != 0) return fail(h, CPX_ERR_HIP, "cpx_thumb_stats: kernel configuration failed");
  CPX_HIP(h, hipGetLastError());
  return CPX_OK;
}

int cpx_thumb_stats(cpx_handle* h, const uint16_t* frames_dev, const int32_t* labels_dev,
                    const cpx_frame_info* info_dev, const cpx_region_ref* refs_dev, int n_refs,
                    cpx_thumb_stat* out_dev) {
  if (!h) return CPX_ERR_INVALID;
  return cpx_thumb_stats_ex(h, frames_dev, labels_dev, info_dev, refs_dev, n_refs, out_dev, h->cfg.width, h->cfg.height,
                            8192);
}

int cpx_trackless_thumb(cpx_handle* h, const uint16_t* frames_dev, int frame, int background, int32_t* out_dev) {
  if (!h) return CPX_ERR_INVALID;
  if (!frames_dev || !out_dev || frame < 0 || background < 0)
    return fail(h, CPX_ERR_INVALID, "cpx_trackless_thumb: bad argument");
  CPX_ENTER(h);
  cpx::TracklessArgs a{};
  a.W = h->cfg.width;
  a.H = h->cfg.height;
  a.frame = frame;
  a.background = background;
  a.frames = frames_dev;
  a.out = out_dev;
  const int rc = cpx::launch_trackless(a, h->stream);
  if (rc == -2) return fail(h, CPX_ERR_UNSUPPORTED, "cpx_trackless_thumb: resolution outside the kernel's envelope");
// ... 36 lines not shown
```

classifier-pipeline_amd/csrc/cpx_internal.h:

```cpp
#pragma once
#include <hip/hip_runtime.h>

#include <map>
#include <string>
#include <vector>

#include "cpx.h"
#include "cpx_kernels.h"

struct cpx_cnn;
struct cpx_mog2;
struct cpx_graph;
void cnn_free(cpx_cnn* c);
void graph_free(cpx_graph* g);
void mog2_free(cpx_mog2* m);

struct DeviceBuffer {
  void* p = nullptr;
  size_t bytes = 0;
  DeviceBuffer() = default;
  DeviceBuffer(const DeviceBuffer&) = delete;
  DeviceBuffer& operator=(const DeviceBuffer&) = delete;
  int grow(cpx_handle* h, size_t need, const char* what);
  void release() {
    if (p) hipFree(p);
    p = nullptr;
    bytes = 0;
  }
  template <class T>
  T* as() const { return static_cast<T*>(p); }
};

struct cpx_handle {
  int device = 0;
  cpx_config cfg{};
  hipStream_t stream = nullptr;
  std::string err;
  DeviceBuffer ws;
  DeviceBuffer wtab_dev, wthr_dev;
  int wtab_len = 0;
  std::vector<double> wtab_host;
  DeviceBuffer nlm_lut_dev;
  DeviceBuffer sched;
  struct ConvEv { int key; double flops; hipEvent_t e0, e1; };
  std::vector<ConvEv> conv_events;
  bool conv_timing = false;
  DeviceBuffer ws_assoc;
  hipEvent_t ev0 = nullptr, ev1 = nullptr;
  int last_launches = 0;
  bool timing_valid = false;
  hipStream_t stream2 = nullptr;
  bool state_packed = false;
  bool packed_state_ok = true;
  bool fuse_conv1 = true;
  bool medians_pending = false;
  hipEvent_t ev_median = nullptr;
  bool track_per_step = false;
  std::vector<struct cpx_cnn*> cnns;
  std::vector<struct cpx_mog2*> mog2s;
  std::vector<struct cpx_graph*> graphs;
  DeviceBuffer graph_arena;
  int stream_frames = -1;
  int stream_assoc_frames = -1;
  bool stream_filt_state = false;
  int last_B = 0;
  struct StagedBackground { std::vector<uint16_t> bg, kcnt; double average; };
  std::map<int, StagedBackground> staged_bg;
  int cnn_math = CPX_CNN_MATH_FP16X2;
  bool fuse_shortcut = true;
  bool shortcut_fp16 = true;
  DeviceBuffer bf3_scratch;
  DeviceBuffer cnn_arena;
  DeviceBuffer cnn_ovf;
  int block_fusion = 2;
  DeviceBuffer ir_scratch;
  DeviceBuffer ir_bitmap;
};

inline int fail(cpx_handle* h, int code, const char* what, hipError_t e = hipSuccess) {
  if (h) {
    h->err = what;
    if (e != hipSuccess) {
      h->err += ": ";
      h->err += hipGetErrorString(e);
    }
  }
  return code;
}

#define CPX_HIP(h, call)                                            \
  do {                                                              \
    hipError_t _e = (call);                                         \
    if (_e != hipSuccess) return fail((h), CPX_ERR_HIP, #call, _e); \
  } while (0)

#define CPX_ENTER(h)                           \
  do {                                         \
    CPX_HIP((h), hipSetDevice((h)->device));   \
    (void)hipGetLastError();                   \
  } while (0)

inline int DeviceBuffer::grow(cpx_handle* h, size_t need, const char* what) {
  if (need <= bytes) return CPX_OK;
  if (p) CPX_HIP(h, hipStreamSynchronize(h->stream));
  release();
  const hipError_t e = hipMalloc(&p, need);
  if (e != hipSuccess) {
    p = nullptr;
    (void)hipGetLastError();
    return fail(h, CPX_ERR_NOMEM, what, e);
  }
  bytes = need;
  return CPX_OK;
}

inline size_t align_up(size_t v, size_t a) { return (v + a - 1) / a * a; }
```

classifier-pipeline_amd/csrc/cpx_schedule_core.h:

```cpp
#pragma once
#include <stddef.h>
#include <stdint.h>

#include <algorithm>
#include <vector>

#include "cpx.h"

namespace cpx {

struct Schedule {
  std::vector<int> clip_first, proc_off, proc_idx, proc_ffc, order;
  int total = 0, max_proc = 0;
};

enum class SchedError { Ok, EmptyClip, TooLong };

inline SchedError schedule_build(const int32_t* clip_offsets, const cpx_frame_meta* meta, int B, int max_frames,
                                 Schedule* sc) {
  sc->total = clip_offsets[B];
  sc->clip_first.resize(B);
  sc->proc_off.assign(B + 1, 0);
  sc->proc_idx.reserve(sc->total);
  sc->proc_ffc.reserve(sc->total);
  for (int b = 0; b < B; ++b) {
    const int f0 = clip_offsets[b], f1 = clip_offsets[b + 1];
    if (f1 <= f0) return SchedError::EmptyClip;
    sc->clip_first[b] = f0;
    for (int f = f0; f < f1; ++f) {
      if (meta[f].background_frame) continue;
      sc->proc_idx.push_back(f);
      int ffc = 0;
      if (meta[f].has_times) ffc = (meta[f].time_on_ms - meta[f].last_ffc_ms) < 9 ? 1 : 0;
      sc->proc_ffc.push_back(ffc);
    }
    sc->proc_off[b + 1] = (int)sc->proc_idx.size();
    const int np = sc->proc_off[b + 1] - sc->proc_off[b];
    if (np > max_frames) return SchedError::TooLong;
    sc->max_proc = std::max(sc->max_proc, np);
  }
  sc->order.resize(B);
  for (int b = 0; b < B; ++b) sc->order[b] = b;
  std::stable_sort(sc->order.begin(), sc->order.end(), [&](int x, int y) {
    return sc->proc_off[x + 1] - sc->proc_off[x] > sc->proc_off[y + 1] - sc->proc_off[y];
  });
  return SchedError::Ok;
}

struct SchedLayout {
  size_t clip_first, proc_off, proc_idx, proc_ffc, order, ints;
  static SchedLayout of(int B, int nproc) {
    const size_t n = (size_t)std::max(nproc, 1);
    SchedLayout l{};
    l.clip_first = 0;
    l.proc_off = l.clip_first + (size_t)B;
    l.proc_idx = l.proc_off + (size_t)B + 1;
    l.proc_ffc = l.proc_idx + n;
    l.order = l.proc_ffc + n;
    l.ints = l.order + (size_t)B;
    return l;
  }
};

inline std::vector<int> schedule_flatten(const Schedule& sc, int B) {
  const SchedLayout l = SchedLayout::of(B, (int)sc.proc_idx.size());
  std::vector<int> flat(l.ints, 0);
  std::copy(sc.clip_first.begin(), sc.clip_first.end(), flat.begin() + l.clip_first);
  std::copy(sc.proc_off.begin(), sc.proc_off.end(), flat.begin() + l.proc_off);
  std::copy(sc.proc_idx.begin(), sc.proc_idx.end(), flat.begin() + l.proc_idx);
  std::copy(sc.proc_ffc.begin(), sc.proc_ffc.end(), flat.begin() + l.proc_ffc);
  std::copy(sc.order.begin(), sc.order.end(), flat.begin() + l.order);
  return flat;
}

template <class Args>
void schedule_point(Args& a, const int* base, const SchedLayout& l) {
  a.clip_first = base + l.clip_first;
  a.proc_off = base + l.proc_off;
  a.proc_idx = base + l.proc_idx;
  a.proc_ffc = base + l.proc_ffc;
}

inline int processed_before(const cpx_frame_meta* meta, int n_prev) {
  int t = 0;
  for (int f = 0; f < n_prev; ++f) t += meta[f].background_frame ? 0 : 1;
  return t;
}

}
```

include/cpx.h:

```cpp
#ifndef CPX_H
#define CPX_H

#include <stddef.h>
#include <stdint.h>

#ifdef __cplusplus
extern "C" {
#endif

#define CPX_ABI_VERSION 3

typedef enum cpx_status {
  CPX_OK = 0,
  CPX_ERR_INVALID = -1,
  CPX_ERR_UNSUPPORTED = -2,
  CPX_ERR_NO_DEVICE = -3,
  CPX_ERR_HIP = -4,
  CPX_ERR_OVERFLOW = -5,
  CPX_ERR_NOMEM = -6
} cpx_status;

typedef struct cpx_handle cpx_handle;

typedef struct cpx_config {
// ... 282 lines not shown
int cpx_mog2_background(cpx_mog2* m, uint8_t* out_dev);
void cpx_mog2_destroy(cpx_mog2* m);

typedef struct cpx_conv_desc {
  int32_t N, H, W, Cin, Cout, groups, ksize, stride, pad_same, relu;
  const float* in_dev;
  float* out_dev;
  const float* weights_dev;
  const float* in_scale_dev;
  const float* in_shift_dev;
  const float* out_scale_dev;
  const float* out_shift_dev;
  const float* residual_dev;
} cpx_conv_desc;
int cpx_conv2d(cpx_handle* h, const cpx_conv_desc* desc);
#define CPX_CNN_MATH_F32 0
#define CPX_CNN_MATH_BF16X3 1
#define CPX_CNN_MATH_BF16X2 2
#define CPX_CNN_MATH_FP16X2 3
int cpx_set_cnn_math(cpx_handle* h, int mode);
int cpx_get_cnn_math(const cpx_handle* h);
int cpx_cnn_last_overflow(cpx_handle* h, int* overflowed);
int cpx_cnn_overflow_forwards(cpx_handle* h, int* count, int reset);
int cpx_cnn_head(cpx_handle* h, const float* in_dev, int N, int HW, int C, const float* bn_scale_dev,
                 const float* bn_shift_dev, const float* dense_w_dev, const float* dense_b_dev, int L,
                 float* logits_dev, float* probs_dev);
#define CPX_HEAD_MAX_HIDDEN 4
#define CPX_HEAD_SIGMOID 0
#define CPX_HEAD_SOFTMAX 1
typedef struct cpx_head_desc {
  int32_t N, HW, C, L;
  int32_t n_hidden, activation;
  int32_t hidden_sizes[CPX_HEAD_MAX_HIDDEN];
  const float* in_dev;
  const float* bn_scale_dev;
  const float* bn_shift_dev;
  const float* hidden_w_dev[CPX_HEAD_MAX_HIDDEN];
  const float* hidden_b_dev[CPX_HEAD_MAX_HIDDEN];
  const float* dense_w_dev;
  const float* dense_b_dev;
  float* logits_dev;
  float* probs_dev;
} cpx_head_desc;
int cpx_cnn_head_ex(cpx_handle* h, const cpx_head_desc* desc);

typedef struct cpx_wrresnet_block {
  const float* in_scale;
  const float* in_shift;
  const float* wa;
  const float* a_scale;
  const float* a_shift;
  const float* wb;
  const float* bb;
} cpx_wrresnet_block;

#define CPX_WRRESNET_MAX_BLOCKS 8
typedef struct cpx_wrresnet_params {
  int32_t n_labels, blocks_per_stage, groups, in_channels;
  int32_t filters[4];
  const float* conv1_w;
  const float* conv1_b;
  cpx_wrresnet_block block[3][CPX_WRRESNET_MAX_BLOCKS];
  const float* shortcut_w[3];
  const float* shortcut_b[3];
  const float* final_scale;
  const float* final_shift;
  const float* dense_w;
  const float* dense_b;
  int32_t n_hidden, activation;
  int32_t hidden_sizes[CPX_HEAD_MAX_HIDDEN];
  const float* hidden_w[CPX_HEAD_MAX_HIDDEN];
  const float* hidden_b[CPX_HEAD_MAX_HIDDEN];
} cpx_wrresnet_params;

typedef struct cpx_cnn cpx_cnn;
int cpx_cnn_create(cpx_handle* h, const cpx_wrresnet_params* params, cpx_cnn** out);
void cpx_cnn_destroy(cpx_cnn* cnn);
int cpx_cnn_set_activation_bounds(cpx_cnn* cnn, const float* bounds, int n);
int cpx_cnn_set_residual_bounds(cpx_cnn* cnn, const float* bounds, int n);
int cpx_cnn_shortcut_scale(float bound, float wmax, float* sx);
int cpx_cnn_forward(cpx_cnn* cnn, const float* in_dev, int N, int H, int W, float* logits_dev, float* probs_dev);
int cpx_cnn_forward_taps(cpx_cnn* cnn, const float* in_dev, int N, int H, int W, float* logits_dev, float* probs_dev,
                         float* const* block_out_dev, int n_blocks, int* block_overflow_dev);

typedef struct cpx_conv_timing {
  int32_t key, launches;
  double total_ms, flops;
} cpx_conv_timing;
int cpx_conv_timing_enable(cpx_handle* h, int enable);
int cpx_conv_timing_report(cpx_handle* h, cpx_conv_timing* out, int cap, int* n_out);

enum {
  CPX_GRAPH_CONV = 1,
  CPX_GRAPH_MAX_POOL = 2,
  CPX_GRAPH_AVG_POOL = 3,
  CPX_GRAPH_ADD = 4,
  CPX_GRAPH_AFFINE = 5,
  CPX_GRAPH_MEAN = 6,
  CPX_GRAPH_FC = 7,
  CPX_GRAPH_LOGISTIC = 8,
  CPX_GRAPH_SOFTMAX = 9,
  CPX_GRAPH_PAD = 10,
  CPX_GRAPH_CHANNEL_MAP = 11,
  CPX_GRAPH_CONV_Q8 = 12,
  CPX_GRAPH_FC_Q8 = 13,
  CPX_GRAPH_QUANT_PARAMS = 14,
  CPX_GRAPH_DWCONV = 15,
  CPX_GRAPH_DWCONV_Q8 = 16,
  CPX_GRAPH_MUL = 17,
  CPX_GRAPH_INPUT = 18,
  CPX_GRAPH_CONV_PRE = 19,
  CPX_GRAPH_SLICE = 20,
  CPX_GRAPH_DWCONV_PRE = 21
};
enum {
  CPX_GRAPH_ACT_NONE = 0, CPX_GRAPH_ACT_RELU = 1, CPX_GRAPH_ACT_RELU6 = 3,
  CPX_GRAPH_ACT_SWISH = 16,
  CPX_GRAPH_ACT_LOGISTIC = 17
};

typedef struct cpx_graph_tensor {
  int32_t H, W, C;
  int32_t c_offset, c_stride;
  int32_t reserved;
  int64_t arena_offset;
} cpx_graph_tensor;

typedef struct cpx_graph_op {
  int32_t kind;
  int32_t in0, in1, out;
  int32_t kh, kw, stride_h, stride_w;
  int32_t pad_top, pad_left, pad_bottom, pad_right;
  int32_t activation;
  int32_t out_c_offset, out_c_stride;
  int32_t n_map, channel_map[4];
  float param;
  const float* weights;
  const float* scale;
  const float* shift;
} cpx_graph_op;

typedef struct cpx_graph cpx_graph;
int cpx_graph_create(cpx_handle* h, const cpx_graph_op* ops, int n_ops, const cpx_graph_tensor* tensors, int n_tensors,
                     int input_tensor, int output_tensor, cpx_graph** out);
int cpx_graph_forward(cpx_graph* g, const float* in_dev, int N, float* out_dev);
int cpx_graph_arena_bytes(const cpx_graph* g, int N, size_t* bytes);
int cpx_graph_arena_allocated(const cpx_handle* h, size_t* bytes);
void cpx_graph_destroy(cpx_graph* g);

size_t cpx_track_workspace_bytes(const cpx_handle* h, int B, int total_frames);

int cpx_last_kernel_timing(cpx_handle* h, float* total_ms, int* launches);

#ifdef __cplusplus
}
#endif
#endif
```

Before: 3.175 million.

## Build frame schedule once per batch and reuse it across tracking stages

Adds a persistent schedule object, built once from clip offsets and frame metadata and uploaded to the device. Track, associate, finalize and plan-segments each take it through new _sched entry points instead of rebuilding and re-uploading the schedule on every call. This is meant to cut repeated host scanning of the metadata and the matching host-to-device copies. In exchange it adds lifetime management (create, destroy, spare buffers, release in finally blocks) and an environment flag to disable it.

```diff
diff --git a/classifier-pipeline_amd/cpx/_lib.py b/classifier-pipeline_amd/cpx/_lib.py
--- a/classifier-pipeline_amd/cpx/_lib.py
+++ b/classifier-pipeline_amd/cpx/_lib.py
@@ -146,6 +146,8 @@
     "cpx_ir_frame_statistics", "cpx_cnn_last_overflow", "cpx_cnn_set_activation_bounds", "cpx_cnn_overflow_forwards", "cpx_cnn_forward_taps",
     "cpx_graph_create", "cpx_graph_forward", "cpx_graph_arena_bytes", "cpx_graph_arena_allocated", "cpx_graph_destroy",
     "cpx_cnn_set_residual_bounds", "cpx_cnn_shortcut_scale",
+    "cpx_schedule_create", "cpx_schedule_destroy", "cpx_track_batch_sched", "cpx_associate_batch_sched",
+    "cpx_finalize_tracks_sched", "cpx_plan_segments_sched",
 ]
 
 IR_FRAME_STATS_DTYPE = np.dtype([("min", "<i4"), ("max", "<i4"), ("sum", "<i8"), ("median_x2", "<i4"), ("reserved", "<i4"),
@@ -300,6 +302,18 @@
     lib.cpx_track_workspace_bytes.restype = C.c_size_t
     lib.cpx_last_kernel_timing.argtypes = [vp, C.POINTER(C.c_float), C.POINTER(C.c_int)]
     lib.cpx_last_kernel_timing.restype = C.c_int
+    lib.cpx_schedule_create.argtypes = [vp, i32p, vp, C.c_int, C.POINTER(vp)]
+    lib.cpx_schedule_create.restype = C.c_int
+    lib.cpx_schedule_destroy.argtypes = [vp]
+    lib.cpx_schedule_destroy.restype = None
+    lib.cpx_track_batch_sched.argtypes = [vp, vp, vp, C.c_int, vp, vp, vp, vp, vp, C.c_int]
+    lib.cpx_track_batch_sched.restype = C.c_int
+    lib.cpx_associate_batch_sched.argtypes = [vp, vp, vp, C.c_int, vp, vp, vp, vp, vp, vp, vp, vp]
+    lib.cpx_associate_batch_sched.restype = C.c_int
+    lib.cpx_finalize_tracks_sched.argtypes = [vp, vp, vp, C.c_int, vp, vp, vp, vp, vp]
+    lib.cpx_finalize_tracks_sched.restype = C.c_int
+    lib.cpx_plan_segments_sched.argtypes = [vp, vp, vp, C.c_int, vp, vp, vp, vp, C.c_int, vp, vp, vp, vp, vp]
+    lib.cpx_plan_segments_sched.restype = C.c_int
     if lib.cpx_abi_version() != 3:
         raise ImportError("libcpx_hip.so ABI version mismatch")
     _lib = lib
diff --git a/classifier-pipeline_amd/cpx/engine.py b/classifier-pipeline_amd/cpx/engine.py
--- a/classifier-pipeline_amd/cpx/engine.py
+++ b/classifier-pipeline_amd/cpx/engine.py
@@ -284,6 +284,23 @@
     frame_regions = TrackStream.frame_regions
     track_records = TrackStream.track_records
     pool_row = TrackStream.pool_row
+
+
+class FrameSchedule:
+
+    def __init__(self, eng, s, B, total):
+        self.eng, self._s, self.B, self.total = eng, s, B, total
+        self._h = eng.h.value
+
+    def ptr(self):
+        if not self._s or self.eng.h.value != self._h:
+            raise ValueError("the schedule is closed (or its engine is)")
+        return self._s
+
+    def close(self):
+        if self._s and self.eng.h.value == self._h:
+            self.eng.lib.cpx_schedule_destroy(self._s)
+        self._s = None
 
 
 class TrackEngine:
@@ -650,8 +667,19 @@
             raise CpxError(rc, self._err())
         return bg, w, float(avg.value)
 
+    def make_schedule(self, clip_offsets, meta):
+        offs = np.ascontiguousarray(clip_offsets, dtype=np.int32)
+        meta = np.ascontiguousarray(meta, dtype=FRAME_META_DTYPE)
+        assert meta.size == int(offs[-1])
+        s = C.c_void_p()
+        rc = self.lib.cpx_schedule_create(self.h, offs.ctypes.data_as(C.POINTER(C.c_int32)), C.c_void_p(meta.ctypes.data),
+                                          offs.size - 1, C.byref(s))
+        if rc != 0:
+            raise CpxError(rc, self._err())
+        return FrameSchedule(self, s, offs.size - 1, int(offs[-1]))
+
     def track_batch(self, frames_dev, clip_offsets, meta, want_labels=False, want_filtered=False,
-                    want_background=False, outputs=None, flags=0):
+                    want_background=False, outputs=None, flags=0, schedule=None):
         t = self.torch
         offs = np.ascontiguousarray(clip_offsets, dtype=np.int32)
         B = offs.size - 1
@@ -669,17 +697,21 @@
             comps, info, labels, filt, bgo = outputs
             self.sync_inputs()
         self.track_calls = getattr(self, "track_calls", 0) + 1
-        rc = self.lib.cpx_track_batch_ex(
-            self.h, C.c_void_p(frames_dev.data_ptr()), offs.ctypes.data_as(C.POINTER(C.c_int32)),
-            C.c_void_p(meta.ctypes.data), B, C.c_void_p(comps.data_ptr()), C.c_void_p(info.data_ptr()),
-            C.c_void_p(labels.data_ptr() if labels is not None else None),
-            C.c_void_p(filt.data_ptr() if filt is not None else None),
-            C.c_void_p(bgo.data_ptr() if bgo is not None else None), int(flags))
+        outs = (C.c_void_p(comps.data_ptr()), C.c_void_p(info.data_ptr()),
+                C.c_void_p(labels.data_ptr() if labels is not None else None),
+                C.c_void_p(filt.data_ptr() if filt is not None else None),
+                C.c_void_p(bgo.data_ptr() if bgo is not None else None), int(flags))
+        if schedule is not None:
+            rc = self.lib.cpx_track_batch_sched(self.h, C.c_void_p(frames_dev.data_ptr()), schedule.ptr(), B, *outs)
+        else:
+            rc = self.lib.cpx_track_batch_ex(
+                self.h, C.c_void_p(frames_dev.data_ptr()), offs.ctypes.data_as(C.POINTER(C.c_int32)),
+                C.c_void_p(meta.ctypes.data), B, *outs)
         if rc != 0:
             raise CpxError(rc, self._err())
         return TrackBatchResult(self, total, self.cap, comps, info, labels, filt, bgo)
 
-    def associate_batch(self, track_result, clip_offsets, meta, params=None, want_regions=True):
+    def associate_batch(self, track_result, clip_offsets, meta, params=None, want_regions=True, schedule=None):
         t = self.torch
         offs = np.ascontiguousarray(clip_offsets, dtype=np.int32)
         B = offs.size - 1
@@ -694,13 +726,16 @@
             status = t.zeros(B, dtype=t.int32, device=self.device)
             regions = t.zeros(total * self.cap * 14, dtype=t.int32, device=self.device) if want_regions else None
             rcounts = t.zeros(total, dtype=t.int32, device=self.device) if want_regions else None
-        rc = self.lib.cpx_associate_batch(
-            self.h, C.byref(params), offs.ctypes.data_as(C.POINTER(C.c_int32)), C.c_void_p(meta.ctypes.data), B,
-            C.c_void_p(track_result.comps_dev.data_ptr()), C.c_void_p(track_result.info_dev.data_ptr()),
-            C.c_void_p(pool.data_ptr()), C.c_void_p(tracks.data_ptr()), C.c_void_p(ntr.data_ptr()),
-            C.c_void_p(status.data_ptr()),
-            C.c_void_p(regions.data_ptr() if regions is not None else None),
-            C.c_void_p(rcounts.data_ptr() if rcounts is not None else None))
+        bufs = (C.c_void_p(track_result.comps_dev.data_ptr()), C.c_void_p(track_result.info_dev.data_ptr()),
+                C.c_void_p(pool.data_ptr()), C.c_void_p(tracks.data_ptr()), C.c_void_p(ntr.data_ptr()),
+                C.c_void_p(status.data_ptr()),
+                C.c_void_p(regions.data_ptr() if regions is not None else None),
+                C.c_void_p(rcounts.data_ptr() if rcounts is not None else None))
+        if schedule is not None:
+            rc = self.lib.cpx_associate_batch_sched(self.h, C.byref(params), schedule.ptr(), B, *bufs)
+        else:
+            rc = self.lib.cpx_associate_batch(
+                self.h, C.byref(params), offs.ctypes.data_as(C.POINTER(C.c_int32)), C.c_void_p(meta.ctypes.data), B, *bufs)
         if rc != 0:
             raise CpxError(rc, self._err())
         return AssocBatchResult(self, offs, params, pool, tracks, ntr, status, regions, rcounts)
diff --git a/classifier-pipeline_amd/cpx/pipeline.py b/classifier-pipeline_amd/cpx/pipeline.py
--- a/classifier-pipeline_amd/cpx/pipeline.py
+++ b/classifier-pipeline_amd/cpx/pipeline.py
@@ -29,6 +29,7 @@
         self.regrown = []
         self.clip0 = 0
         self.track_timing = (0.0, 0)
+        self.schedule = None
 
     def summaries(self, max_tracks):
         return self.summaries_dev.cpu().numpy().view(TRACK_SUMMARY_DTYPE).reshape(-1, max_tracks)
@@ -77,10 +78,13 @@
     def _run_on_stream(self, frames_dev, clip_offsets, meta, outputs, classify, keep_samples):
         eng, t = self.eng, self.eng.torch
         out = self._front(frames_dev, clip_offsets, meta, outputs, classify)
-        if not classify or out.n_tracks == 0 or out.n_samples == 0:
-            eng.synchronize()
-        else:
-            out = self.classify_front(out, frames_dev, keep_samples)
+        try:
+            if not classify or out.n_tracks == 0 or out.n_samples == 0:
+                eng.synchronize()
+            else:
+                out = self.classify_front(out, frames_dev, keep_samples)
+        finally:
+            self.release_schedule(out)
         if out.overflowed:
             out = self._regrow(out, frames_dev, clip_offsets, meta, classify, keep_samples)
         return out
@@ -105,10 +109,13 @@
                                 network_bytes=self.network_bytes)
             with t.cuda.stream(eng_k.torch_stream()):
                 part = sub._front(fr, np.array([0, f1 - f0], np.int32), meta[f0:f1], None, classify, pre=(res_k, assoc_k))
-                if classify and part.n_tracks and part.n_samples:
-                    part = sub.classify_front(part, fr, keep_samples)
-                else:
-                    eng_k.synchronize()
+                try:
+                    if classify and part.n_tracks and part.n_samples:
+                        part = sub.classify_front(part, fr, keep_samples)
+                    else:
+                        eng_k.synchronize()
+                finally:
+                    sub.release_schedule(part)
             part.clip0 = b
             out.regrown.append((b, eng_k.cap, tp_k.max_active_tracks, tp_k.max_tracks))
             parts.append(part)
@@ -190,28 +197,49 @@
         return out
 
     def _front(self, frames_dev, clip_offsets, meta, outputs, classify=True, pre=None):
-        eng, t = self.eng, self.eng.torch
-        lib, h = eng.lib, eng.h
-        dev = eng.device
+        eng = self.eng
         offs = np.ascontiguousarray(clip_offsets, dtype=np.int32)
         meta = np.ascontiguousarray(meta)
         B = offs.size - 1
         out = BatchResult()
+        if os.environ.get("CPX_SCHEDULE_ONCE", "1") != "0":
+            out.schedule = eng.make_schedule(offs, meta)
+        try:
+            return self._front_stages(out, frames_dev, offs, meta, B, outputs, classify, pre)
+        except BaseException:
+            self.release_schedule(out)
+            raise
+
+    @staticmethod
+    def release_schedule(out):
+        for part in [out] + list(out.parts or []):
+            if part.schedule is not None:
+                part.schedule.close()
+                part.schedule = None
+
+    def _front_stages(self, out, frames_dev, offs, meta, B, outputs, classify, pre):
+        eng, t = self.eng, self.eng.torch
+        lib, h = eng.lib, eng.h
+        dev = eng.device
+        sched = out.schedule
         if pre is not None:
             out.track, out.assoc = pre
         else:
             out.track = eng.track_batch(frames_dev, offs, meta, want_filtered=True, outputs=outputs,
-                                        flags=TRACK_DEFER_MEDIANS)
-            out.assoc = eng.associate_batch(out.track, offs, meta, params=self.tp, want_regions=self.want_regions)
+                                        flags=TRACK_DEFER_MEDIANS, schedule=sched)
+            out.assoc = eng.associate_batch(out.track, offs, meta, params=self.tp, want_regions=self.want_regions,
+                                            schedule=sched)
         mt = self.tp.max_tracks
         summ = t.zeros(B * mt * 30, dtype=t.int32, device=dev)
         counts = t.zeros((B, 4), dtype=t.int32, device=dev)
         offs_p = offs.ctypes.data_as(C.POINTER(C.c_int32))
         eng.sync_inputs()
-        self._check(lib.cpx_finalize_tracks(
-            h, C.byref(self.fp), offs_p, C.c_void_p(meta.ctypes.data), B, C.c_void_p(out.assoc.pool_dev.data_ptr()),
-            C.c_void_p(out.assoc.tracks_dev.data_ptr()), C.c_void_p(out.assoc.ntracks_dev.data_ptr()),
-            C.c_void_p(summ.data_ptr()), C.c_void_p(counts.data_ptr())))
+        fin = (C.c_void_p(out.assoc.pool_dev.data_ptr()), C.c_void_p(out.assoc.tracks_dev.data_ptr()),
+               C.c_void_p(out.assoc.ntracks_dev.data_ptr()), C.c_void_p(summ.data_ptr()), C.c_void_p(counts.data_ptr()))
+        if sched is not None:
+            self._check(lib.cpx_finalize_tracks_sched(h, C.byref(self.fp), sched.ptr(), B, *fin))
+        else:
+            self._check(lib.cpx_finalize_tracks(h, C.byref(self.fp), offs_p, C.c_void_p(meta.ctypes.data), B, *fin))
         out.summaries_dev = summ
         on_stream = int(t.cuda.current_stream(dev).cuda_stream) == int(lib.cpx_stream(h) or 0)
         if not on_stream:
@@ -235,11 +263,14 @@
         sample_track = t.empty(n_samples, dtype=t.int32, device=dev)
         track_clip = t.empty((n_tracks, 2), dtype=t.int32, device=dev)
         eng.sync_inputs()
-        self._check(lib.cpx_plan_segments(
-            h, C.byref(self.fp), offs_p, C.c_void_p(meta.ctypes.data), B, C.c_void_p(out.assoc.pool_dev.data_ptr()),
-            C.c_void_p(summ.data_ptr()), C.c_void_p(out.assoc.ntracks_dev.data_ptr()), C.c_void_p(prefix.data_ptr()),
-            self.sq, C.c_void_p(refs.data_ptr()), C.c_void_p(toffs.data_ptr()), C.c_void_p(reqs.data_ptr()),
-            C.c_void_p(sample_track.data_ptr()), C.c_void_p(track_clip.data_ptr())))
+        plan = (C.c_void_p(out.assoc.pool_dev.data_ptr()), C.c_void_p(summ.data_ptr()),
+                C.c_void_p(out.assoc.ntracks_dev.data_ptr()), C.c_void_p(prefix.data_ptr()), self.sq,
+                C.c_void_p(refs.data_ptr()), C.c_void_p(toffs.data_ptr()), C.c_void_p(reqs.data_ptr()),
+                C.c_void_p(sample_track.data_ptr()), C.c_void_p(track_clip.data_ptr()))
+        if sched is not None:
+            self._check(lib.cpx_plan_segments_sched(h, C.byref(self.fp), sched.ptr(), B, *plan))
+        else:
+            self._check(lib.cpx_plan_segments(h, C.byref(self.fp), offs_p, C.c_void_p(meta.ctypes.data), B, *plan))
         if not on_stream:
             eng.synchronize()
         out.track_clip, out.reqs_dev, out.sample_track_dev = track_clip, reqs, sample_track
@@ -254,17 +285,28 @@
         return out
 
     def _run_overlapped(self, frames_dev, clip_offsets, meta, outputs, n_sub):
-        eng, ceng, t = self.eng, self.net.eng, self.eng.torch
-        lib, dev = eng.lib, eng.device
+        eng, ceng = self.eng, self.net.eng
         offs = np.ascontiguousarray(clip_offsets, dtype=np.int32)
         meta = np.ascontiguousarray(meta)
         B = offs.size - 1
         n_sub = max(1, min(n_sub, B))
         bounds = [int(round(B * k / n_sub)) for k in range(n_sub + 1)]
+        parts = []
+        try:
+            self._enqueue_groups(parts, frames_dev, offs, meta, outputs, bounds)
+            eng.synchronize()
+            ceng.synchronize()
+        finally:
+            for part in parts:
+                self.release_schedule(part)
+        return self._merge_groups(parts, frames_dev, clip_offsets, meta)
+
+    def _enqueue_groups(self, parts, frames_dev, offs, meta, outputs, bounds):
+        eng, ceng, t = self.eng, self.net.eng, self.eng.torch
+        lib, dev = eng.lib, eng.device
         s_track, s_cnn = eng.torch_stream(), ceng.torch_stream()
         per, side, cap = self.sq * self.sq, self.sq * self.fs, eng.cap
-        parts = []
-        for k in range(n_sub):
+        for k in range(len(bounds) - 1):
             b0, b1 = bounds[k], bounds[k + 1]
             if b1 <= b0:
                 continue
@@ -307,8 +349,9 @@
             if rc != 0:
                 raise CpxError(rc, ceng._err())
             part._keep2 = (samples, logits, ev)
-        eng.synchronize()
-        ceng.synchronize()
+
+    def _merge_groups(self, parts, frames_dev, clip_offsets, meta):
+        eng, t = self.eng, self.eng.torch
         out = BatchResult()
         out.parts = parts
         out.track = parts[0].track if len(parts) == 1 else _MergedCheck([p.track for p in parts])
diff --git a/classifier-pipeline_amd/cpx/track/bulk.py b/classifier-pipeline_amd/cpx/track/bulk.py
--- a/classifier-pipeline_amd/cpx/track/bulk.py
+++ b/classifier-pipeline_amd/cpx/track/bulk.py
@@ -390,6 +390,7 @@
         with t.cuda.stream(eng.torch_stream()):
             front = pipe._front(group.frames_dev, offs, meta, (comps, info_dev, labels, filt, None),
                                 classify=bool(classifiers))
+            pipe.release_schedule(front)
             lap("track_assoc_finalize_plan")
             for model, interp in classifiers:
                 if interp.params.square_width != sq:
diff --git a/classifier-pipeline_amd/csrc/cpx_api.cpp b/classifier-pipeline_amd/csrc/cpx_api.cpp
--- a/classifier-pipeline_amd/csrc/cpx_api.cpp
+++ b/classifier-pipeline_amd/csrc/cpx_api.cpp
@@ -57,21 +57,129 @@
   return l;
 }
 
-int build_schedule(cpx_handle* h, const int32_t* clip_offsets, const cpx_frame_meta* meta, int B, cpx::Schedule* sc) {
-  switch (cpx::schedule_build(clip_offsets, meta, B, h->cfg.max_frames, sc)) {
+}
+
+struct cpx_schedule {
+  cpx_handle* h = nullptr;
+  int B = 0;
+  cpx::SchedTotals t;
+  cpx::SchedLayout l{};
+  cpx_handle::SchedMem mem{};
+  mutable unsigned median_seq = 0;
+};
+
+namespace {
+
+const size_t kSchedSpares = 4;
+
+void sched_mem_free(cpx_handle::SchedMem* m) {
+  if (m->host) hipHostFree(m->host);
+  if (m->dev) hipFree(m->dev);
+  *m = cpx_handle::SchedMem{};
+}
+
+int sched_mem_take(cpx_handle* h, size_t ints, cpx_handle::SchedMem* m) {
+  std::vector<cpx_handle::SchedMem>& sp = h->sched_spare;
+  int best = -1;
+  for (size_t i = 0; i < sp.size(); ++i)
+    if (sp[i].ints >= ints && (best < 0 || sp[i].ints < sp[best].ints)) best = (int)i;
+  if (best >= 0) {
+    *m = sp[best];
+    sp.erase(sp.begin() + best);
+    return CPX_OK;
+  }
+  *m = cpx_handle::SchedMem{};
+  hipError_t e = hipHostMalloc((void**)&m->host, ints * sizeof(int), hipHostMallocDefault);
+  if (e == hipSuccess) e = hipMalloc((void**)&m->dev, ints * sizeof(int));
+  if (e != hipSuccess) {
+    sched_mem_free(m);
+    (void)hipGetLastError();
+    return fail(h, CPX_ERR_NOMEM, "schedule allocation", e);
+  }
+  m->ints = ints;
+  return CPX_OK;
+}
+
+void drain_streams(cpx_handle* h) {
+  hipSetDevice(h->device);
+  if (h->stream) hipStreamSynchronize(h->stream);
+  if (h->stream2) hipStreamSynchronize(h->stream2);
+  h->medians_pending = false;
+  h->median_joined = h->median_seq;
+}
+
+void schedule_release(cpx_handle* h, cpx_schedule* s) {
+  std::vector<cpx_handle::SchedMem>& sp = h->sched_spare;
+  if (s->mem.host) sp.push_back(s->mem);
+  if (sp.size() > kSchedSpares) {
+    size_t least = 0;
+    for (size_t i = 1; i < sp.size(); ++i)
+      if (sp[i].ints < sp[least].ints) least = i;
+    sched_mem_free(&sp[least]);
+    sp.erase(sp.begin() + least);
+  }
+  delete s;
+}
+
+int schedule_make(cpx_handle* h, const int32_t* clip_offsets, const cpx_frame_meta* meta, int B, cpx_schedule** out) {
+  *out = nullptr;
+  CPX_ENTER(h);
+  cpx::SchedTotals t;
+  switch (cpx::schedule_measure(clip_offsets, meta, B, h->cfg.max_frames, &t)) {
     case cpx::SchedError::EmptyClip: return fail(h, CPX_ERR_INVALID, "empty clip in batch");
     case cpx::SchedError::TooLong: return fail(h, CPX_ERR_INVALID, "clip longer than max_frames");
     case cpx::SchedError::Ok: break;
   }
-  return CPX_OK;
-}
-
-int upload_schedule(cpx_handle* h, const cpx::Schedule& sc, int B, cpx::SchedLayout* sl) {
-  const std::vector<int> flat = cpx::schedule_flatten(sc, B);
-  *sl = cpx::SchedLayout::of(B, (int)sc.proc_idx.size());
-  if (int rc = h->sched.grow(h, flat.size() * sizeof(int), "schedule hipMalloc")) return rc;
-  CPX_HIP(h, hipMemcpyAsync(h->sched.p, flat.data(), flat.size() * sizeof(int), hipMemcpyHostToDevice, h->stream));
-  CPX_HIP(h, hipStreamSynchronize(h->stream));
+  cpx_schedule* s = new (std::nothrow) cpx_schedule();
+  if (!s) return fail(h, CPX_ERR_NOMEM, "schedule allocation");
+  s->h = h;
+  s->B = B;
+  s->t = t;
+  s->l = cpx::SchedLayout::of(B, t.nproc);
+  if (int rc = sched_mem_take(h, s->l.ints, &s->mem)) {
+    delete s;
+    return rc;
+  }
+  cpx::schedule_write(clip_offsets, meta, B, s->l, s->mem.host);
+  const hipError_t e = hipMemcpyAsync(s->mem.dev, s->mem.host, s->l.ints * sizeof(int), hipMemcpyHostToDevice, h->stream);
+  if (e != hipSuccess) {
+    drain_streams(h);
+    schedule_release(h, s);
+    return fail(h, CPX_ERR_HIP, "schedule upload", e);
+  }
+  *out = s;
+  return CPX_OK;
+}
+
+void sweep_retired(cpx_handle* h) {
+  if (h->retired.empty()) return;
+  unsigned done = h->median_joined;
+  if (h->median_seq > done) {
+    if (hipEventQuery(h->ev_median) == hipSuccess) done = h->median_seq;
+    (void)hipGetLastError();
+  }
+  size_t kept = 0;
+  for (cpx_schedule* s : h->retired) {
+    if (s->median_seq > done) h->retired[kept++] = s;
+    else schedule_release(h, s);
+  }
+  h->retired.resize(kept);
+}
+
+int legacy_schedule(cpx_handle* h, const int32_t* clip_offsets, const cpx_frame_meta* meta, int B, const cpx_schedule** out) {
+  cpx_schedule* s = nullptr;
+  if (int rc = schedule_make(h, clip_offsets, meta, B, &s)) return rc;
+  const hipError_t e = hipStreamSynchronize(h->stream);
+  if (e == hipSuccess) sweep_retired(h);
+  h->retired.push_back(s);
+  if (e != hipSuccess) return fail(h, CPX_ERR_HIP, "hipStreamSynchronize(h->stream)", e);
+  *out = s;
+  return CPX_OK;
+}
+
+int check_schedule(cpx_handle* h, const cpx_schedule* s, int B) {
+  if (s->h != h) return fail(h, CPX_ERR_INVALID, "the schedule belongs to another handle");
+  if (s->B != B) return fail(h, CPX_ERR_INVALID, "the schedule was made for another batch size");
   return CPX_OK;
 }
 
@@ -168,14 +276,20 @@
 
 static void release_buffers(cpx_handle* h, bool all) {
   for (DeviceBuffer* b : {&h->ws, &h->ws_assoc, &h->bf3_scratch, &h->cnn_arena, &h->graph_arena, &h->ir_scratch}) b->release();
+  for (cpx_handle::SchedMem& m : h->sched_spare) sched_mem_free(&m);
+  h->sched_spare.clear();
   if (!all) return;
-  for (DeviceBuffer* b : {&h->sched, &h->wtab_dev, &h->wthr_dev, &h->nlm_lut_dev, &h->cnn_ovf, &h->ir_bitmap}) b->release();
+  for (DeviceBuffer* b : {&h->wtab_dev, &h->wthr_dev, &h->nlm_lut_dev, &h->cnn_ovf, &h->ir_bitmap}) b->release();
 }
 
 void cpx_destroy(cpx_handle* h) {
   if (!h) return;
   hipSetDevice(h->device);
-  if (h->stream) hipStreamSynchronize(h->stream);
+  drain_streams(h);
+  for (std::vector<cpx_schedule*>* list : {&h->schedules, &h->retired}) {
+    for (cpx_schedule* s : *list) schedule_release(h, s);
+    list->clear();
+  }
   for (cpx_cnn* c : h->cnns) cnn_free(c);
   h->cnns.clear();
   for (cpx_mog2* m : h->mog2s) mog2_free(m);
@@ -206,6 +320,7 @@
   if (h->medians_pending) {
     h->medians_pending = false;
     CPX_HIP(h, hipStreamWaitEvent(h->stream, h->ev_median, 0));
+    h->median_joined = h->median_seq;
   }
   return CPX_OK;
 }
@@ -221,6 +336,7 @@
   if (int rc = join_medians(h)) return rc;
   CPX_HIP(h, hipStreamSynchronize(h->stream));
   CPX_HIP(h, hipStreamSynchronize(h->stream2));
+  sweep_retired(h);
   release_buffers(h, false);
   h->last_B = 0;
   h->state_packed = false;
@@ -231,7 +347,30 @@
   if (!h) return CPX_ERR_INVALID;
   if (int rc = join_medians(h)) return rc;
   CPX_HIP(h, hipStreamSynchronize(h->stream));
-  return CPX_OK;
+  sweep_retired(h);
+  return CPX_OK;
+}
+
+int cpx_schedule_create(cpx_handle* h, const int32_t* clip_offsets, const cpx_frame_meta* meta, int B,
+                        cpx_schedule** out) {
+  if (!h) return CPX_ERR_INVALID;
+  if (!clip_offsets || !meta || B <= 0 || !out) return fail(h, CPX_ERR_INVALID, "cpx_schedule_create: null argument");
+  cpx_schedule* s = nullptr;
+  if (int rc = schedule_make(h, clip_offsets, meta, B, &s)) {
+    *out = nullptr;
+    return rc;
+  }
+  h->schedules.push_back(s);
+  *out = s;
+  return CPX_OK;
+}
+
+void cpx_schedule_destroy(cpx_schedule* s) {
+  if (!s) return;
+  cpx_handle* h = s->h;
+  drain_streams(h);
+  h->schedules.erase(std::remove(h->schedules.begin(), h->schedules.end(), s), h->schedules.end());
+  schedule_release(h, s);
 }
 
 size_t cpx_track_workspace_bytes(const cpx_handle* h, int B, int total_frames) {
@@ -252,22 +391,23 @@
   return CPX_OK;
 }
 
-static int track_run(cpx_handle* h, const uint16_t* frames_dev, const int32_t* clip_offsets,
-                     const cpx_frame_meta* meta, int B, int n_prev, cpx_component* comps_dev,
-                     cpx_frame_info* info_dev, int32_t* labels_dev, float* filtered_dev,
-                     float* background_dev, int flags) {
-  CPX_ENTER(h);
+static int track_flags_check(cpx_handle* h, int flags) {
   if (flags & ~(CPX_TRACK_KEEP_BACKGROUND | CPX_TRACK_FREEZE_ON_FFC | CPX_TRACK_FREEZE_BACKGROUND | CPX_TRACK_DEFER_MEDIANS))
     return fail(h, CPX_ERR_INVALID, "track: unknown flag");
+  return CPX_OK;
+}
+
+static int track_run(cpx_handle* h, const uint16_t* frames_dev, const cpx_schedule* s, int n_prev, int t_begin,
+                     cpx_component* comps_dev, cpx_frame_info* info_dev, int32_t* labels_dev, float* filtered_dev,
+                     float* background_dev, int flags) {
+  CPX_ENTER(h);
+  if (int frc = track_flags_check(h, flags)) return frc;
   if (int jrc = join_medians(h)) return jrc;
   const bool defer_medians = (flags & CPX_TRACK_DEFER_MEDIANS) != 0;
   const cpx_config& c = h->cfg;
-  cpx::Schedule sc;
-  int rc = build_schedule(h, clip_offsets, meta, B, &sc);
-  if (rc != CPX_OK) return rc;
-  const int total = sc.total, max_proc = sc.max_proc;
+  int rc = CPX_OK;
+  const int B = s->B, total = s->t.total, max_proc = s->t.max_proc;
   const bool resume = n_prev > 0;
-  const int t_begin = cpx::processed_before(meta, n_prev);
   const bool need_filt = (filtered_dev == nullptr);
   const WsLayout l = ws_layout(c, B, need_filt);
   if (resume && (l.total > h->ws.bytes || need_filt != h->stream_filt_state))
@@ -303,9 +443,6 @@
     }
   } guard{h};
   if ((rc = h->ws.grow(h, l.total, "workspace hipMalloc"))) return rc;
-  cpx::SchedLayout sl;
-  rc = upload_schedule(h, sc, B, &sl);
-  if (rc != CPX_OK) return rc;
 
   cpx::TrackArgs a{};
   a.W = c.width;
@@ -317,8 +454,8 @@
   a.background_thresh = c.background_thresh;
   a.weight_add = c.weight_add;
   a.frames = frames_dev;
-  cpx::schedule_point(a, h->sched.as<int>(), sl);
-  a.order = h->sched.as<int>() + sl.order;
+  cpx::schedule_point(a, s->mem.dev, s->l);
+  a.order = s->mem.dev + s->l.order;
   a.wtab = h->wtab_dev.as<double>();
   a.wtab_len = h->wtab_len;
   a.wthr = h->wthr_dev.as<uint32_t>();
@@ -381,6 +518,7 @@
   CPX_HIP(h, hipEventRecord(h->ev1, h->stream));
   if (defer_medians) {
     CPX_HIP(h, hipStreamWaitEvent(h->stream2, h->ev1, 0));
+    s->median_seq = ++h->median_seq;
     cpx::launch_median(a, B, t_begin, max_proc, h->stream2);
     CPX_HIP(h, hipEventRecord(h->ev_median, h->stream2));
     h->medians_pending = true;
@@ -401,8 +539,21 @@
   if (!frames_dev || !clip_offsets || !meta || B <= 0 || !comps_dev || !info_dev)
     return fail(h, CPX_ERR_INVALID, "cpx_track_batch: null argument");
   h->stream_frames = -1;
-  return track_run(h, frames_dev, clip_offsets, meta, B, -1, comps_dev, info_dev, labels_dev, filtered_dev,
-                   background_dev, flags);
+  if (int frc = track_flags_check(h, flags)) return frc;
+  const cpx_schedule* s = nullptr;
+  if (int rc = legacy_schedule(h, clip_offsets, meta, B, &s)) return rc;
+  return track_run(h, frames_dev, s, -1, 0, comps_dev, info_dev, labels_dev, filtered_dev, background_dev, flags);
+}
+
+int cpx_track_batch_sched(cpx_handle* h, const uint16_t* frames_dev, const cpx_schedule* s, int B,
+                          cpx_component* comps_dev, cpx_frame_info* info_dev, int32_t* labels_dev,
+                          float* filtered_dev, float* background_dev, int flags) {
+  if (!h) return CPX_ERR_INVALID;
+  if (!frames_dev || !s || B <= 0 || !comps_dev || !info_dev)
+    return fail(h, CPX_ERR_INVALID, "cpx_track_batch: null argument");
+  if (int rc = check_schedule(h, s, B)) return rc;
+  h->stream_frames = -1;
+  return track_run(h, frames_dev, s, -1, 0, comps_dev, info_dev, labels_dev, filtered_dev, background_dev, flags);
 }
 
 int cpx_track_batch(cpx_handle* h, const uint16_t* frames_dev, const int32_t* clip_offsets,
@@ -424,8 +575,11 @@
   const int32_t offs[2] = {0, n_frames};
   h->stream_frames = -1;
   if (n_prev == 0) h->stream_assoc_frames = -1;
-  const int rc = track_run(h, frames_dev, offs, meta, 1, n_prev, comps_dev, info_dev, labels_dev, filtered_dev,
-                           background_dev, flags);
+  if (int frc = track_flags_check(h, flags)) return frc;
+  const cpx_schedule* s = nullptr;
+  if (int src = legacy_schedule(h, offs, meta, 1, &s)) return src;
+  const int rc = track_run(h, frames_dev, s, n_prev, cpx::processed_before(meta, n_prev), comps_dev, info_dev, labels_dev,
+                           filtered_dev, background_dev, flags);
   if (rc == CPX_OK) h->stream_frames = n_frames;
   return rc;
 }
@@ -514,22 +668,21 @@
   return CPX_OK;
 }
 
-static int assoc_run(cpx_handle* h, const cpx_track_params* params, const int32_t* clip_offsets,
-                     const cpx_frame_meta* meta, int B, int n_prev, bool fresh, const cpx_component* comps_dev,
-                     const cpx_frame_info* info_dev, cpx_region* pool_dev,
+static int assoc_params_check(cpx_handle* h, const cpx_track_params* params) {
+  if (params->max_active_tracks < 1 || params->max_tracks < 1)
+    return fail(h, CPX_ERR_INVALID, "association: capacities must be positive");
+  return CPX_OK;
+}
+
+static int assoc_run(cpx_handle* h, const cpx_track_params* params, const cpx_schedule* s, int n_prev, int t_begin,
+                     bool fresh, const cpx_component* comps_dev, const cpx_frame_info* info_dev, cpx_region* pool_dev,
                      cpx_track_record* tracks_dev, int32_t* n_tracks_dev, int32_t* status_dev,
                      cpx_region* regions_dev, int32_t* region_counts_dev) {
-  if (params->max_active_tracks < 1 || params->max_tracks < 1)
-    return fail(h, CPX_ERR_INVALID, "association: capacities must be positive");
+  if (int prc = assoc_params_check(h, params)) return prc;
   CPX_ENTER(h);
   const bool resume = n_prev > 0 && !fresh;
-  const int t_begin = cpx::processed_before(meta, n_prev);
-  cpx::Schedule sc;
-  cpx::SchedLayout sl;
-  int rc = build_schedule(h, clip_offsets, meta, B, &sc);
-  if (rc != CPX_OK) return rc;
-  rc = upload_schedule(h, sc, B, &sl);
-  if (rc != CPX_OK) return rc;
+  const int B = s->B;
+  int rc = CPX_OK;
   const int cap = h->cfg.max_components, ma = params->max_active_tracks;
   size_t off = 0;
   const size_t o_active = off;
@@ -550,7 +703,7 @@
   a.B = B;
   a.cap = cap;
   a.params = *params;
-  cpx::schedule_point(a, h->sched.as<int>(), sl);
+  cpx::schedule_point(a, s->mem.dev, s->l);
   a.comps = comps_dev;
   a.info = info_dev;
   a.pool = pool_dev;
@@ -581,8 +734,24 @@
       !n_tracks_dev || !status_dev)
     return fail(h, CPX_ERR_INVALID, "cpx_associate_batch: null argument");
   h->stream_assoc_frames = -1;
-  return assoc_run(h, params, clip_offsets, meta, B, -1, true, comps_dev, info_dev, pool_dev, tracks_dev, n_tracks_dev,
-                   status_dev, regions_dev, region_counts_dev);
+  if (int prc = assoc_params_check(h, params)) return prc;
+  const cpx_schedule* s = nullptr;
+  if (int rc = legacy_schedule(h, clip_offsets, meta, B, &s)) return rc;
+  return assoc_run(h, params, s, -1, 0, true, comps_dev, info_dev, pool_dev, tracks_dev, n_tracks_dev, status_dev,
+                   regions_dev, region_counts_dev);
+}
+
+int cpx_associate_batch_sched(cpx_handle* h, const cpx_track_params* params, const cpx_schedule* s, int B,
+                              const cpx_component* comps_dev, const cpx_frame_info* info_dev, cpx_region* pool_dev,
+                              cpx_track_record* tracks_dev, int32_t* n_tracks_dev, int32_t* status_dev,
+                              cpx_region* regions_dev, int32_t* region_counts_dev) {
+  if (!h) return CPX_ERR_INVALID;
+  if (!params || !s || B <= 0 || !comps_dev || !info_dev || !pool_dev || !tracks_dev || !n_tracks_dev || !status_dev)
+    return fail(h, CPX_ERR_INVALID, "cpx_associate_batch: null argument");
+  if (int rc = check_schedule(h, s, B)) return rc;
+  h->stream_assoc_frames = -1;
+  return assoc_run(h, params, s, -1, 0, true, comps_dev, info_dev, pool_dev, tracks_dev, n_tracks_dev, status_dev,
+                   regions_dev, region_counts_dev);
 }
 
 int cpx_associate_frame(cpx_handle* h, const cpx_track_params* params, const cpx_frame_meta* meta, int n_prev,
@@ -598,8 +767,11 @@
     return fail(h, CPX_ERR_INVALID, "cpx_associate_frame: n_prev is behind the frames this handle has consumed");
   const int32_t offs[2] = {0, n_frames};
   h->stream_assoc_frames = -1;
-  const int rc = assoc_run(h, params, offs, meta, 1, n_prev, fresh, comps_dev, info_dev, pool_dev, tracks_dev, n_tracks_dev,
-                           status_dev, regions_dev, region_counts_dev);
+  if (int prc = assoc_params_check(h, params)) return prc;
+  const cpx_schedule* s = nullptr;
+  if (int src = legacy_schedule(h, offs, meta, 1, &s)) return src;
+  const int rc = assoc_run(h, params, s, n_prev, cpx::processed_before(meta, n_prev), fresh, comps_dev, info_dev, pool_dev,
+                           tracks_dev, n_tracks_dev, status_dev, regions_dev, region_counts_dev);
   if (rc == CPX_OK) h->stream_assoc_frames = n_frames;
   return rc;
 }
@@ -672,23 +844,22 @@
   return CPX_OK;
 }
 
-static int final_args(cpx_handle* h, const cpx_filter_params* params, const int32_t* clip_offsets,
-                      const cpx_frame_meta* meta, int B, cpx::FinalArgs* a) {
+static int filter_params_check(cpx_handle* h, const cpx_filter_params* params) {
   if (params->max_active_tracks < 1 || params->max_tracks_per_clip < 1)
     return fail(h, CPX_ERR_INVALID, "filter params: capacities must be positive");
-  CPX_ENTER(h);
-  cpx::Schedule sc;
-  cpx::SchedLayout sl;
-  int rc = build_schedule(h, clip_offsets, meta, B, &sc);
-  if (rc != CPX_OK) return rc;
-  rc = upload_schedule(h, sc, B, &sl);
-  if (rc != CPX_OK) return rc;
+  return CPX_OK;
+}
+
+static int final_args(cpx_handle* h, const cpx_filter_params* params, const cpx_schedule* s, cpx::FinalArgs* a) {
+  if (int prc = filter_params_check(h, params)) return prc;
+  CPX_ENTER(h);
+  const int B = s->B;
   a->B = B;
   a->params = *params;
   a->max_frames = h->cfg.max_frames;
-  cpx::schedule_point(*a, h->sched.as<int>(), sl);
+  cpx::schedule_point(*a, s->mem.dev, s->l);
   const size_t doubles = (size_t)B * h->cfg.max_frames * 2 * sizeof(double);
-  rc = h->ws_assoc.grow(h, doubles + (size_t)B * h->cfg.max_frames * sizeof(float) + 512, "finalize workspace hipMalloc");
+  const int rc = h->ws_assoc.grow(h, doubles + (size_t)B * h->cfg.max_frames * sizeof(float) + 512, "finalize workspace hipMalloc");
   if (rc != CPX_OK) return rc;
   a->scratch_d = h->ws_assoc.as<double>();
   a->scratch_f = (float*)(h->ws_assoc.as<char>() + align_up(doubles, 256));
@@ -703,8 +874,21 @@
   if (!params || !clip_offsets || !meta || B <= 0 || !pool_dev || !tracks_dev || !n_tracks_dev || !summaries_dev ||
       !counts_dev)
     return fail(h, CPX_ERR_INVALID, "cpx_finalize_tracks: null argument");
+  if (int prc = filter_params_check(h, params)) return prc;
+  const cpx_schedule* s = nullptr;
+  if (int rc = legacy_schedule(h, clip_offsets, meta, B, &s)) return rc;
+  return cpx_finalize_tracks_sched(h, params, s, B, pool_dev, tracks_dev, n_tracks_dev, summaries_dev, counts_dev);
+}
+
+int cpx_finalize_tracks_sched(cpx_handle* h, const cpx_filter_params* params, const cpx_schedule* s, int B,
+                              const cpx_region* pool_dev, const cpx_track_record* tracks_dev,
+                              const int32_t* n_tracks_dev, cpx_track_summary* summaries_dev, int32_t* counts_dev) {
+  if (!h) return CPX_ERR_INVALID;
+  if (!params || !s || B <= 0 || !pool_dev || !tracks_dev || !n_tracks_dev || !summaries_dev || !counts_dev)
+    return fail(h, CPX_ERR_INVALID, "cpx_finalize_tracks: null argument");
+  if (int crc = check_schedule(h, s, B)) return crc;
   cpx::FinalArgs a{};
-  const int rc = final_args(h, params, clip_offsets, meta, B, &a);
+  const int rc = final_args(h, params, s, &a);
   if (rc != CPX_OK) return rc;
   a.square_width = 5;
   a.pool = pool_dev;
@@ -728,8 +912,26 @@
       !refs_dev || !track_offsets_dev || !reqs_dev || !sample_track_dev || !track_clip_dev)
     return fail(h, CPX_ERR_INVALID, "cpx_plan_segments: null argument");
   if (square_width != 5) return fail(h, CPX_ERR_UNSUPPORTED, "cpx_plan_segments: square_width must be 5");
+  if (int prc = filter_params_check(h, params)) return prc;
+  const cpx_schedule* s = nullptr;
+  if (int rc = legacy_schedule(h, clip_offsets, meta, B, &s)) return rc;
+  return cpx_plan_segments_sched(h, params, s, B, pool_dev, summaries_dev, n_tracks_dev, prefix_dev, square_width, refs_dev,
+                                 track_offsets_dev, reqs_dev, sample_track_dev, track_clip_dev);
+}
+
+int cpx_plan_segments_sched(cpx_handle* h, const cpx_filter_params* params, const cpx_schedule* s, int B,
+                            const cpx_region* pool_dev, const cpx_track_summary* summaries_dev,
+                            const int32_t* n_tracks_dev, const int32_t* prefix_dev, int square_width,
+                            cpx_region_ref* refs_dev, int32_t* track_offsets_dev, cpx_crop_req* reqs_dev,
+                            int32_t* sample_track_dev, int32_t* track_clip_dev) {
+  if (!h) return CPX_ERR_INVALID;
+  if (!params || !s || B <= 0 || !pool_dev || !summaries_dev || !n_tracks_dev || !prefix_dev || !refs_dev ||
+      !track_offsets_dev || !reqs_dev || !sample_track_dev || !track_clip_dev)
+    return fail(h, CPX_ERR_INVALID, "cpx_plan_segments: null argument");
+  if (square_width != 5) return fail(h, CPX_ERR_UNSUPPORTED, "cpx_plan_segments: square_width must be 5");
+  if (int crc = check_schedule(h, s, B)) return crc;
   cpx::FinalArgs a{};
-  const int rc = final_args(h, params, clip_offsets, meta, B, &a);
+  const int rc = final_args(h, params, s, &a);
   if (rc != CPX_OK) return rc;
   a.square_width = square_width;
   a.pool = pool_dev;
diff --git a/classifier-pipeline_amd/csrc/cpx_internal.h b/classifier-pipeline_amd/csrc/cpx_internal.h
--- a/classifier-pipeline_amd/csrc/cpx_internal.h
+++ b/classifier-pipeline_amd/csrc/cpx_internal.h
@@ -41,7 +41,10 @@
   int wtab_len = 0;
   std::vector<double> wtab_host;
   DeviceBuffer nlm_lut_dev;
-  DeviceBuffer sched;
+  std::vector<struct cpx_schedule*> schedules, retired;
+  struct SchedMem { int* host; int* dev; size_t ints; };
+  std::vector<SchedMem> sched_spare;
+  unsigned median_seq = 0, median_joined = 0;
   struct ConvEv { int key; double flops; hipEvent_t e0, e1; };
   std::vector<ConvEv> conv_events;
   bool conv_timing = false;
diff --git a/classifier-pipeline_amd/csrc/cpx_schedule_core.h b/classifier-pipeline_amd/csrc/cpx_schedule_core.h
--- a/classifier-pipeline_amd/csrc/cpx_schedule_core.h
+++ b/classifier-pipeline_amd/csrc/cpx_schedule_core.h
@@ -73,6 +73,53 @@
   return flat;
 }
 
+struct SchedTotals {
+  int total = 0, max_proc = 0, nproc = 0;
+};
+
+inline SchedError schedule_measure(const int32_t* clip_offsets, const cpx_frame_meta* meta, int B, int max_frames,
+                                   SchedTotals* t) {
+  *t = SchedTotals{};
+  t->total = clip_offsets[B];
+  for (int b = 0; b < B; ++b) {
+    const int f0 = clip_offsets[b], f1 = clip_offsets[b + 1];
+    if (f1 <= f0) return SchedError::EmptyClip;
+    int np = 0;
+    for (int f = f0; f < f1; ++f) np += meta[f].background_frame ? 0 : 1;
+    t->nproc += np;
+    if (np > max_frames) return SchedError::TooLong;
+    t->max_proc = std::max(t->max_proc, np);
+  }
+  return SchedError::Ok;
+}
+
+inline void schedule_write(const int32_t* clip_offsets, const cpx_frame_meta* meta, int B, const SchedLayout& l,
+                           int* flat) {
+  int* clip_first = flat + l.clip_first;
+  int* proc_off = flat + l.proc_off;
+  int* proc_idx = flat + l.proc_idx;
+  int* proc_ffc = flat + l.proc_ffc;
+  int* order = flat + l.order;
+  int n = 0;
+  proc_off[0] = 0;
+  for (int b = 0; b < B; ++b) {
+    const int f0 = clip_offsets[b], f1 = clip_offsets[b + 1];
+    clip_first[b] = f0;
+    for (int f = f0; f < f1; ++f) {
+      if (meta[f].background_frame) continue;
+      proc_idx[n] = f;
+      proc_ffc[n] = (meta[f].has_times && (meta[f].time_on_ms - meta[f].last_ffc_ms) < 9) ? 1 : 0;
+      ++n;
+    }
+    proc_off[b + 1] = n;
+  }
+  if (n == 0) proc_idx[0] = proc_ffc[0] = 0;
+  for (int b = 0; b < B; ++b) order[b] = b;
+  std::stable_sort(order, order + B, [&](int x, int y) {
+    return proc_off[x + 1] - proc_off[x] > proc_off[y + 1] - proc_off[y];
+  });
+}
+
 template <class Args>
 void schedule_point(Args& a, const int* base, const SchedLayout& l) {
   a.clip_first = base + l.clip_first;
diff --git a/include/cpx.h b/include/cpx.h
--- a/include/cpx.h
+++ b/include/cpx.h
@@ -458,6 +458,26 @@
 
 int cpx_last_kernel_timing(cpx_handle* h, float* total_ms, int* launches);
 
+typedef struct cpx_schedule cpx_schedule;
+int cpx_schedule_create(cpx_handle* h, const int32_t* clip_offsets, const cpx_frame_meta* meta, int B,
+                        cpx_schedule** out);
+void cpx_schedule_destroy(cpx_schedule* s);
+int cpx_track_batch_sched(cpx_handle* h, const uint16_t* frames_dev, const cpx_schedule* s, int B,
+                          cpx_component* comps_dev, cpx_frame_info* info_dev, int32_t* labels_dev,
+                          float* filtered_dev, float* background_dev, int flags);
+int cpx_associate_batch_sched(cpx_handle* h, const cpx_track_params* params, const cpx_schedule* s, int B,
+                              const cpx_component* comps_dev, const cpx_frame_info* info_dev, cpx_region* pool_dev,
+                              cpx_track_record* tracks_dev, int32_t* n_tracks_dev, int32_t* status_dev,
+                              cpx_region* regions_dev, int32_t* region_counts_dev);
+int cpx_finalize_tracks_sched(cpx_handle* h, const cpx_filter_params* params, const cpx_schedule* s, int B,
+                              const cpx_region* pool_dev, const cpx_track_record* tracks_dev,
+                              const int32_t* n_tracks_dev, cpx_track_summary* summaries_dev, int32_t* counts_dev);
+int cpx_plan_segments_sched(cpx_handle* h, const cpx_filter_params* params, const cpx_schedule* s, int B,
+                            const cpx_region* pool_dev, const cpx_track_summary* summaries_dev,
+                            const int32_t* n_tracks_dev, const int32_t* prefix_dev, int square_width,
+                            cpx_region_ref* refs_dev, int32_t* track_offsets_dev, cpx_crop_req* reqs_dev,
+                            int32_t* sample_track_dev, int32_t* track_clip_dev);
+
 #ifdef __cplusplus
 }
 #endif
```

Result: no change. 3.200 million, median of 6 (+0.8%).
